# iracigt/ceres-raytracer

Measured on AMD Instinct MI355X. Metric: Mrays/sec (primary+shadow) on dragon.obj 1920x1080; 1/2/4/8-GPU scaling, higher is better.
Workload: dtype f32; 1 GPU; dragon_1080: dragon.obj 1920x1080 primary+shadow, 16 copies of the config view per step; views=config, W=1920, H=1080, row_block=1080, parallelism=one GPU, whole frames, float_framebuffer=True, streams=8

## Files before the change

### ceres-raytracer_amd/__init__.py

```python
import ctypes
import os
import sys

import numpy as np

_PKG = os.path.dirname(os.path.abspath(__file__))
LIB_PATH = os.environ.get("CERES_LIB") or os.path.join(_PKG, "libceres_hip.so")
CLI_PATH = os.path.join(_PKG, "render")

if _PKG not in sys.path:
    sys.path.insert(0, _PKG)
import configs

MODE_FULL, MODE_PRIMARY = 0, 1
MODE_ROBUST = 0x10
MODE_QBVH4 = 0x20
MODE_FMA = 0x40
ARITH_EXACT, ARITH_FMA = 0, 1


def cfg_mode(cfg, arith=ARITH_EXACT):
    return ((MODE_PRIMARY if cfg["mode"] == "primary" else MODE_FULL) | (MODE_ROBUST if cfg.get("robust") else 0)
            | (MODE_FMA if arith else 0))
SCENE_STATS = 1
SCENE_FIRST_ORDER = 2

EXPORTED_SYMBOLS = (
    "ceres_obj_load", "ceres_proc_mesh", "ceres_rotate_triangles", "ceres_bvh_build", "ceres_bvh_build_gpu",
    "ceres_bvh_build_device", "ceres_obj_load_gpu", "ceres_obj_parse_device", "ceres_rotate_triangles_device",
    "ceres_device_free", "ceres_camera_basis", "ceres_obj_load_f64", "ceres_proc_mesh_f64", "ceres_rotate_triangles_f64",
    "ceres_bvh_build_f64", "ceres_camera_basis_f64", "ceres_orbit_cameras_f64", "ceres_scene_create_f64",
    "ceres_render_f64", "ceres_render_records_f64", "ceres_obj_load_f64_arith", "ceres_proc_mesh_f64_arith",
    "ceres_rotate_triangles_f64_arith", "ceres_bvh_build_f64_arith", "ceres_camera_basis_f64_arith",
    "ceres_orbit_cameras_f64_arith",
    "ceres_free", "ceres_scene_create", "ceres_scene_create_device", "ceres_scene_destroy", "ceres_scene_info", "ceres_scene_shadow_stacks", "ceres_render_f32",
    "ceres_render_device", "ceres_render_batch_device", "ceres_render_multi_f32", "ceres_device_count", "ceres_assemble_rgb8_packed", "ceres_render_records", "ceres_tiling_local_rows",
    "ceres_scene_set_timing", "ceres_scene_read_timing", "ceres_scene_wave_log", "ceres_fetch_counters",
    "ceres_cpu_scene_create", "ceres_cpu_scene_destroy", "ceres_render_cpu_f32", "ceres_cpu_scene_create_f64",
    "ceres_render_cpu_f64",
    "ceres_orbit_cameras", "ceres_assemble_rgb8",
    "ceres_kernel_names", "ceres_last_error", "ceres_version",
    "ceres_obj_load_arith", "ceres_proc_mesh_arith", "ceres_rotate_triangles_arith", "ceres_bvh_build_arith",
    "ceres_camera_basis_arith", "ceres_orbit_cameras_arith", "ceres_content_hash",
    "ceres_bvh_build_gpu_arith", "ceres_bvh_build_device_arith", "ceres_obj_load_gpu_arith",
    "ceres_obj_parse_device_arith", "ceres_rotate_triangles_device_arith",
    "ceres_trace_rays", "ceres_trace_rays_device", "ceres_trace_rays_cpu",
    "ceres_trace_rays_f64", "ceres_trace_rays_f64_device", "ceres_trace_rays_cpu_f64",
    "ceres_shade_rays", "ceres_shade_rays_device", "ceres_shade_rays_cpu", "ceres_camera_rays",
    "ceres_shade_rays_f64", "ceres_shade_rays_f64_device", "ceres_shade_rays_cpu_f64", "ceres_camera_rays_f64",
    "ceres_scene_refit", "ceres_scene_refit_device", "ceres_scene_refit_f64", "ceres_scene_refit_f64_device",
    "ceres_cpu_scene_refit", "ceres_cpu_scene_refit_f64", "ceres_scene_read_boxes",
)

HIT_DTYPE = np.dtype([("prim", np.int32), ("t", np.float32), ("u", np.float32), ("v", np.float32)])
FLT_MAX = np.float32(np.finfo(np.float32).max)
HIT64_DTYPE = np.dtype([("prim", np.int32), ("pad", np.uint32), ("t", np.float64), ("u", np.float64), ("v", np.float64)])
DBL_MAX = np.float64(np.finfo(np.float64).max)


class CeresError(RuntimeError):
    pass


class _Stats(ctypes.Structure):
    _fields_ = [("rays", ctypes.c_uint64), ("hits", ctypes.c_uint64), ("primary_rays", ctypes.c_uint64),
                ("shadow_rays", ctypes.c_uint64), ("node_pairs", ctypes.c_uint64), ("tri_tests", ctypes.c_uint64),
                ("ms", ctypes.c_double)]


class Tiling(ctypes.Structure):
    _fields_ = [("row_block", ctypes.c_uint32), ("rank", ctypes.c_uint32), ("world", ctypes.c_uint32),
                ("bands", ctypes.c_uint32)]


_lib = None
_fp = ctypes.POINTER(ctypes.c_float)
_dp = ctypes.POINTER(ctypes.c_double)
_u32p = ctypes.POINTER(ctypes.c_uint32)
_u64p = ctypes.POINTER(ctypes.c_uint64)
_sz = ctypes.c_size_t
_vp = ctypes.c_void_p


def build(verbose=False):
    import subprocess
    r = subprocess.run(["make", "-C", os.path.join(_PKG, "csrc"), "-j4", "all"], capture_output=True, text=True)
    if verbose or r.returncode:
        sys.stdout.write(r.stdout)
        sys.stderr.write(r.stderr)
    if r.returncode:
        raise CeresError("build of libceres_hip.so failed")


def lib():
    global _lib
    if _lib is not None:
        return _lib
    if not os.path.exists(LIB_PATH):
        raise CeresError(f"{LIB_PATH} is missing: run __graft_entry__.build() (no CPU fallback exists)")
    if "torch" not in sys.modules:
        try:
            import torch
        except ImportError:
            pass
    L = ctypes.CDLL(LIB_PATH)
    L.ceres_last_error.restype = ctypes.c_char_p
    L.ceres_version.restype = ctypes.c_char_p
    L.ceres_kernel_names.restype = ctypes.c_char_p
    L.ceres_obj_load.argtypes = [ctypes.c_char_p, ctypes.POINTER(_fp), ctypes.POINTER(_fp), ctypes.POINTER(_sz)]
    L.ceres_proc_mesh.argtypes = [ctypes.c_int, ctypes.POINTER(_fp), ctypes.POINTER(_fp), ctypes.POINTER(_sz)]
    L.ceres_rotate_triangles.argtypes = [_fp, _sz, ctypes.c_int, ctypes.c_float]
    L.ceres_bvh_build.argtypes = [_fp, _sz, ctypes.POINTER(_u32p), ctypes.POINTER(_sz), ctypes.POINTER(_u64p)]
    L.ceres_bvh_build_gpu.argtypes = [_fp, _sz, ctypes.POINTER(_u32p), ctypes.POINTER(_sz), ctypes.POINTER(_u64p),
                                      ctypes.c_int]
    L.ceres_bvh_build_device.argtypes = [_vp, _sz, _vp, _vp, ctypes.POINTER(_sz), _vp]
    L.ceres_obj_load_gpu.argtypes = [ctypes.c_char_p, ctypes.POINTER(_fp), ctypes.POINTER(_fp), ctypes.POINTER(_sz),
                                     ctypes.c_int]
    L.ceres_obj_parse_device.argtypes = [_vp, _sz, ctypes.POINTER(_vp), ctypes.POINTER(_vp), ctypes.POINTER(_sz), _vp]
    L.ceres_rotate_triangles_device.argtypes = [_vp, _sz, ctypes.c_int, ctypes.c_float, _vp]
    L.ceres_device_free.argtypes = [_vp]
    L.ceres_device_free.restype = None
    L.ceres_camera_basis.argtypes = [_fp, _fp, _fp, ctypes.c_float, _sz, _sz, _fp]
    L.ceres_obj_load_f64.argtypes = [ctypes.c_char_p, ctypes.POINTER(_dp), ctypes.POINTER(_dp), ctypes.POINTER(_sz)]
    L.ceres_proc_mesh_f64.argtypes = [ctypes.c_int, ctypes.POINTER(_dp), ctypes.POINTER(_dp), ctypes.POINTER(_sz)]
    L.ceres_rotate_triangles_f64.argtypes = [_dp, _sz, ctypes.c_int, ctypes.c_double]
    L.ceres_bvh_build_f64.argtypes = [_dp, _sz, ctypes.POINTER(_u64p), ctypes.POINTER(_sz), ctypes.POINTER(_u64p)]
    L.ceres_camera_basis_f64.argtypes = [_dp, _dp, _dp, ctypes.c_double, _sz, _sz, _dp]
    L.ceres_orbit_cameras_f64.argtypes = [_dp, _dp, _dp, _dp, ctypes.c_double, _sz, _sz, _dp, ctypes.c_double,
                                          ctypes.c_uint32, ctypes.c_int, _dp, _dp, _dp]
    L.ceres_obj_load_f64_arith.argtypes = [ctypes.c_char_p, ctypes.POINTER(_dp), ctypes.POINTER(_dp), ctypes.POINTER(_sz),
                                           ctypes.c_int]
    L.ceres_proc_mesh_f64_arith.argtypes = [ctypes.c_int, ctypes.POINTER(_dp), ctypes.POINTER(_dp), ctypes.POINTER(_sz),
                                            ctypes.c_int]
    L.ceres_rotate_triangles_f64_arith.argtypes = [_dp, _sz, ctypes.c_int, ctypes.c_double, ctypes.c_int]
    L.ceres_bvh_build_f64_arith.argtypes = [_dp, _sz, ctypes.POINTER(_u64p), ctypes.POINTER(_sz), ctypes.POINTER(_u64p),
                                            ctypes.c_int]
    L.ceres_camera_basis_f64_arith.argtypes = [_dp, _dp, _dp, ctypes.c_double, _sz, _sz, _dp, ctypes.c_int]
    L.ceres_orbit_cameras_f64_arith.argtypes = [_dp, _dp, _dp, _dp, ctypes.c_double, _sz, _sz, _dp, ctypes.c_double,
                                                ctypes.c_uint32, ctypes.c_int, _dp, _dp, _dp, ctypes.c_int]
    L.ceres_scene_create_f64.argtypes = [_dp, _sz, _dp, _vp, _sz, _u64p, ctypes.c_int, ctypes.c_uint32]
    L.ceres_scene_create_f64.restype = _vp
    L.ceres_render_f64.argtypes = [_vp, _dp, _dp, ctypes.c_int, _dp, ctypes.POINTER(ctypes.c_uint8), _sz, _sz,
                                   ctypes.POINTER(_Stats)]
    L.ceres_render_records_f64.argtypes = [_vp, _dp, _dp, ctypes.c_int, _sz, _sz, ctypes.POINTER(ctypes.c_int32), _dp,
                                           ctypes.POINTER(ctypes.c_int8), ctypes.POINTER(_Stats)]
    L.ceres_orbit_cameras.argtypes = [_fp, _fp, _fp, _fp, ctypes.c_float, _sz, _sz, _fp, ctypes.c_float,
                                      ctypes.c_uint32, ctypes.c_int, _fp, _fp, _fp]
    L.ceres_free.argtypes = [_vp]
    L.ceres_free.restype = None
    L.ceres_scene_create.argtypes = [_fp, _sz, _fp, _vp, _sz, _u64p, ctypes.c_int, ctypes.c_uint32]
    L.ceres_scene_create.restype = _vp
    L.ceres_scene_create_device.argtypes = [_vp, _sz, _vp, _vp, _sz, _vp, ctypes.c_int, ctypes.c_uint32, _vp]
    L.ceres_scene_create_device.restype = _vp
    L.ceres_scene_destroy.argtypes = [_vp]
    L.ceres_scene_destroy.restype = None
    L.ceres_scene_info.argtypes = [_vp, _u32p, _u32p, ctypes.POINTER(_sz), ctypes.POINTER(_sz)]
    L.ceres_scene_shadow_stacks.argtypes = [_vp, _u32p, _u32p]
    L.ceres_render_f32.argtypes = [_vp, _fp, _fp, ctypes.c_int, _fp, ctypes.POINTER(ctypes.c_uint8), _sz, _sz,
                                   ctypes.POINTER(_Stats)]
    L.ceres_render_device.argtypes = [_vp, _fp, _fp, ctypes.c_int, _sz, _sz, ctypes.POINTER(Tiling), _vp, _vp, _vp, _vp]
    L.ceres_render_batch_device.argtypes = [_vp, ctypes.c_uint32, _fp, _fp, ctypes.c_int, _sz, _sz,
                                            ctypes.POINTER(Tiling), _vp, _vp, _vp, _vp]
    L.ceres_render_multi_f32.argtypes = [ctypes.POINTER(_vp), ctypes.c_uint32, ctypes.c_uint32, _fp, _fp, ctypes.c_int, _fp,
                                         ctypes.POINTER(ctypes.c_uint8), _sz, _sz, ctypes.POINTER(_Stats)]
    L.ceres_assemble_rgb8_packed.argtypes = [_vp, _vp, ctypes.c_uint32, _sz, _sz, ctypes.c_uint32, ctypes.c_uint32, _vp]
    L.ceres_assemble_rgb8.argtypes = [_vp, _sz, _vp, ctypes.c_uint32, _sz, _sz, ctypes.c_uint32, ctypes.c_uint32, _vp]
    L.ceres_render_records.argtypes = [_vp, _fp, _fp, ctypes.c_int, _sz, _sz, ctypes.POINTER(ctypes.c_int32), _fp,
                                       ctypes.POINTER(ctypes.c_int8), ctypes.POINTER(_Stats)]
    L.ceres_tiling_local_rows.argtypes = [_sz, ctypes.POINTER(Tiling)]
    L.ceres_tiling_local_rows.restype = _sz
    L.ceres_scene_set_timing.argtypes = [_vp, ctypes.c_int]
    L.ceres_scene_read_timing.argtypes = [_vp, ctypes.POINTER(ctypes.c_double), ctypes.POINTER(ctypes.c_double),
                                          _u64p]
    L.ceres_scene_wave_log.argtypes = [_vp, _u64p, _sz, ctypes.POINTER(_sz)]
    L.ceres_fetch_counters.argtypes = [ctypes.c_int, _u64p, ctypes.c_int]
    L.ceres_cpu_scene_create.argtypes = [_fp, _sz, _fp, _vp, _sz, _u64p]
    L.ceres_cpu_scene_create.restype = _vp
    L.ceres_cpu_scene_destroy.argtypes = [_vp]
    L.ceres_cpu_scene_destroy.restype = None
    L.ceres_render_cpu_f32.argtypes = [_vp, _fp, _fp, ctypes.c_int, _fp, ctypes.POINTER(ctypes.c_uint8), _sz, _sz,
                                       ctypes.POINTER(_Stats), ctypes.c_int]
    L.ceres_cpu_scene_create_f64.argtypes = [_dp, _sz, _dp, _vp, _sz, _u64p]
    L.ceres_cpu_scene_create_f64.restype = _vp
    L.ceres_render_cpu_f64.argtypes = [_vp, _dp, _dp, ctypes.c_int, _dp, ctypes.POINTER(ctypes.c_uint8), _sz, _sz,
                                       ctypes.POINTER(_Stats), ctypes.c_int]
    L.ceres_trace_rays.argtypes = [_vp, _vp, _sz, ctypes.c_int, _vp, _vp, ctypes.POINTER(_Stats)]
    L.ceres_trace_rays_device.argtypes = [_vp, _vp, _sz, ctypes.c_int, _vp, _vp, _vp, _vp]
    L.ceres_trace_rays_cpu.argtypes = [_vp, _vp, _sz, ctypes.c_int, _vp, _vp, ctypes.POINTER(_Stats), ctypes.c_int]
    L.ceres_trace_rays_f64.argtypes = L.ceres_trace_rays.argtypes
    L.ceres_trace_rays_f64_device.argtypes = L.ceres_trace_rays_device.argtypes
    L.ceres_trace_rays_cpu_f64.argtypes = L.ceres_trace_rays_cpu.argtypes
    L.ceres_shade_rays.argtypes = [_vp, _vp, _sz, _fp, ctypes.c_int, _vp, _vp, _vp, _vp, ctypes.POINTER(_Stats)]
    L.ceres_shade_rays_device.argtypes = [_vp, _vp, _sz, _fp, ctypes.c_int, _vp, _vp, _vp, _vp, _vp, _vp]
    L.ceres_shade_rays_cpu.argtypes = L.ceres_shade_rays.argtypes + [ctypes.c_int]
    L.ceres_camera_rays.argtypes = [_fp, _sz, _sz, ctypes.c_int, _vp]
    L.ceres_shade_rays_f64.argtypes = [_vp, _vp, _sz, _dp, ctypes.c_int, _vp, _vp, _vp, _vp, ctypes.POINTER(_Stats)]
    L.ceres_shade_rays_f64_device.argtypes = [_vp, _vp, _sz, _dp, ctypes.c_int, _vp, _vp, _vp, _vp, _vp, _vp]
    L.ceres_shade_rays_cpu_f64.argtypes = L.ceres_shade_rays_f64.argtypes + [ctypes.c_int]
    L.ceres_camera_rays_f64.argtypes = [_dp, _sz, _sz, ctypes.c_int, _vp]
    L.ceres_scene_refit.argtypes = [_vp, _fp, _sz, _fp]
    L.ceres_scene_refit_f64.argtypes = [_vp, _dp, _sz, _dp]
    L.ceres_scene_refit_device.argtypes = [_vp, _vp, _sz, _vp, _vp]
    L.ceres_scene_refit_f64_device.argtypes = [_vp, _vp, _sz, _vp, _vp]
    L.ceres_cpu_scene_refit.argtypes = [_vp, _fp, _sz, _fp]
    L.ceres_cpu_scene_refit_f64.argtypes = [_vp, _dp, _sz, _dp]
    L.ceres_scene_read_boxes.argtypes = [_vp, _vp, ctypes.POINTER(_sz), _fp, ctypes.POINTER(_sz)]
    L.ceres_content_hash.argtypes = [_vp, _sz]
    L.ceres_content_hash.restype = ctypes.c_uint64
    L.ceres_obj_load_arith.argtypes = L.ceres_obj_load.argtypes + [ctypes.c_int]
    L.ceres_proc_mesh_arith.argtypes = L.ceres_proc_mesh.argtypes + [ctypes.c_int]
    L.ceres_rotate_triangles_arith.argtypes = L.ceres_rotate_triangles.argtypes + [ctypes.c_int]
    L.ceres_bvh_build_arith.argtypes = L.ceres_bvh_build.argtypes + [ctypes.c_int]
    L.ceres_camera_basis_arith.argtypes = L.ceres_camera_basis.argtypes + [ctypes.c_int]
    L.ceres_orbit_cameras_arith.argtypes = L.ceres_orbit_cameras.argtypes + [ctypes.c_int]
    L.ceres_bvh_build_gpu_arith.argtypes = L.ceres_bvh_build_gpu.argtypes + [ctypes.c_int]
    L.ceres_bvh_build_device_arith.argtypes = L.ceres_bvh_build_device.argtypes + [ctypes.c_int]
    L.ceres_obj_load_gpu_arith.argtypes = L.ceres_obj_load_gpu.argtypes + [ctypes.c_int]
    L.ceres_obj_parse_device_arith.argtypes = L.ceres_obj_parse_device.argtypes + [ctypes.c_int]
    L.ceres_rotate_triangles_device_arith.argtypes = L.ceres_rotate_triangles_device.argtypes + [ctypes.c_int]
    _lib = L
    return L


def _check(rc):
    if rc != 0:
        raise CeresError(f"ceres error {rc}: {lib().ceres_last_error().decode()}")


def _p(a, t):
    return None if a is None else a.ctypes.data_as(ctypes.POINTER(t))


def _take(ptr, count, dtype):
    if count == 0:
        lib().ceres_free(ctypes.cast(ptr, _vp))
        return np.zeros(0, dtype)
    a = np.ctypeslib.as_array(ptr, shape=(count,)).copy().view(dtype)
    lib().ceres_free(ctypes.cast(ptr, _vp))
    return a


class Camera:

    def __init__(self, eye, dir, up, fov, dtype=np.float32, arith=ARITH_EXACT):
        self.dtype = np.dtype(dtype)
        self.eye = np.asarray(eye, self.dtype)
        self.dir = np.asarray(dir, self.dtype)
        self.up = np.asarray(up, self.dtype)
        self.fov = float(fov)
        self.arith = int(arith)

    def basis(self, W, H):
        if self.dtype == np.float64:
            out = np.zeros(9, np.float64)
            _check(lib().ceres_camera_basis_f64_arith(_p(self.eye, ctypes.c_double), _p(self.dir, ctypes.c_double),
                                                      _p(self.up, ctypes.c_double), self.fov, W, H,
                                                      _p(out, ctypes.c_double), self.arith))
            return np.concatenate([self.eye, out])
        out = np.zeros(9, np.float32)
        _check(lib().ceres_camera_basis_arith(_p(self.eye, ctypes.c_float), _p(self.dir, ctypes.c_float),
                                              _p(self.up, ctypes.c_float), self.fov, W, H, _p(out, ctypes.c_float),
                                              self.arith))
        return np.concatenate([self.eye, out]).astype(np.float32)


class Mesh:

    def __init__(self, tri, norm):
        dt = np.float64 if np.asarray(tri).dtype == np.float64 else np.float32
        self.tri = np.ascontiguousarray(tri, dt).reshape(-1, 12)
        self.norm = np.ascontiguousarray(norm, dt).reshape(-1, 9)

    @property
    def f64(self):
        return self.tri.dtype == np.float64

    def __len__(self):
        return self.tri.shape[0]


class Bvh:

    def __init__(self, nodes, prim):
        dt = np.uint64 if np.asarray(nodes).dtype == np.uint64 else np.uint32
        self.nodes = np.ascontiguousarray(nodes, dt).reshape(-1, 8)
        self.prim = np.ascontiguousarray(prim, np.uint64)


def load_obj(path, arith=ARITH_EXACT):
    t, n, cnt = _fp(), _fp(), _sz()
    _check(lib().ceres_obj_load_arith(os.fsencode(path), ctypes.byref(t), ctypes.byref(n), ctypes.byref(cnt), int(arith)))
    c = cnt.value
    return Mesh(_take(t, c * 12, np.float32).reshape(c, 12), _take(n, c * 9, np.float32).reshape(c, 9))


def load_obj_f64(path, arith=ARITH_EXACT):
    t, n, cnt = _dp(), _dp(), _sz()
    _check(lib().ceres_obj_load_f64_arith(os.fsencode(path), ctypes.byref(t), ctypes.byref(n), ctypes.byref(cnt),
                                          int(arith)))
    c = cnt.value
    return Mesh(_take(t, c * 12, np.float64).reshape(c, 12), _take(n, c * 9, np.float64).reshape(c, 9))


def proc_mesh_f64(n, arith=ARITH_EXACT):
    t, nn, cnt = _dp(), _dp(), _sz()
    _check(lib().ceres_proc_mesh_f64_arith(int(n), ctypes.byref(t), ctypes.byref(nn), ctypes.byref(cnt), int(arith)))
    c = cnt.value
    return Mesh(_take(t, c * 12, np.float64).reshape(c, 12), _take(nn, c * 9, np.float64).reshape(c, 9))


def load_obj_gpu(path, device=0, arith=ARITH_EXACT):
    t, n, cnt = _fp(), _fp(), _sz()
    _check(lib().ceres_obj_load_gpu_arith(os.fsencode(path), ctypes.byref(t), ctypes.byref(n), ctypes.byref(cnt),
                                          int(device), int(arith)))
    c = cnt.value
    return Mesh(_take(t, c * 12, np.float32).reshape(c, 12), _take(n, c * 9, np.float32).reshape(c, 9))


def parse_obj_device(d_text, length, stream=0, arith=ARITH_EXACT):
    t, n, cnt = _vp(), _vp(), _sz()
    _check(lib().ceres_obj_parse_device_arith(d_text, length, ctypes.byref(t), ctypes.byref(n), ctypes.byref(cnt),
                                              stream or None, int(arith)))
    return t.value or 0, n.value or 0, cnt.value


def rotate_triangles_device(d_tri48, n_tri, axis, degrees, stream=0, arith=ARITH_EXACT):
    ax = {"x": 0, "y": 1, "z": 2}[axis] if isinstance(axis, str) else int(axis)
    _check(lib().ceres_rotate_triangles_device_arith(d_tri48, n_tri, ax, float(degrees), stream or None, int(arith)))
# ... 242 lines not shown

    def shade(self, rays, sun, mode=0, pixels=True, rgb8=False, hits=False, status=False, threads=0):
        fn = lib().ceres_shade_rays_cpu_f64 if self.f64 else lib().ceres_shade_rays_cpu
        return _shade_host(lambda r, n, s, m, px, q, h, stt, st: fn(self._h, r, n, s, m, px, q, h, stt, st, int(threads)),
                           rays, sun, mode, pixels, rgb8, hits, status, self.f64)


class Scene:

    def __init__(self, mesh, bvh, device=0, stats=False, first_order=False, _handle=None):
        L = lib()
        if _handle is not None:
            self._h, self.device, self.n_tri = _handle
            self.f64 = False
            return
        self.f64 = mesh.f64
        flags = (SCENE_STATS if stats else 0) | (SCENE_FIRST_ORDER if first_order else 0)
        if self.f64:
            self._h = L.ceres_scene_create_f64(_p(mesh.tri, ctypes.c_double), len(mesh), _p(mesh.norm, ctypes.c_double),
                                               bvh.nodes.ctypes.data_as(_vp), bvh.nodes.shape[0],
                                               _p(bvh.prim, ctypes.c_uint64), int(device), flags)
        else:
            self._h = L.ceres_scene_create(_p(mesh.tri, ctypes.c_float), len(mesh), _p(mesh.norm, ctypes.c_float),
                                           bvh.nodes.ctypes.data_as(_vp), bvh.nodes.shape[0],
                                           _p(bvh.prim, ctypes.c_uint64), int(device), flags)
        if not self._h:
            raise CeresError("ceres_scene_create: " + L.ceres_last_error().decode())
        self.device = device
        self.n_tri = len(mesh)

    @classmethod
    def from_device(cls, d_tri48, n_tri, d_norm36, d_nodes32, n_nodes, d_prim32, device=0, stats=False, stream=0):
        L = lib()
        h = L.ceres_scene_create_device(d_tri48, n_tri, d_norm36, d_nodes32, n_nodes, d_prim32, int(device),
                                        SCENE_STATS if stats else 0, stream or None)
        if not h:
            raise CeresError("ceres_scene_create_device: " + L.ceres_last_error().decode())
        return cls(None, None, _handle=(h, device, n_tri))

    def info(self):
        d, s, n, b = ctypes.c_uint32(), ctypes.c_uint32(), _sz(), _sz()
        _check(lib().ceres_scene_info(self._h, ctypes.byref(d), ctypes.byref(s), ctypes.byref(n), ctypes.byref(b)))
        near, first = ctypes.c_uint32(), ctypes.c_uint32()
        _check(lib().ceres_scene_shadow_stacks(self._h, ctypes.byref(near), ctypes.byref(first)))
        return dict(depth=d.value, stack_entries=s.value, n_pairs=n.value, device_bytes=b.value,
                    shadow_stack_nearest=near.value, shadow_stack_first=first.value)

    def refit(self, mesh):
        if mesh.f64 != self.f64:
            raise CeresError("refit: a %s mesh for a %s scene" % (("float", "double")[mesh.f64], ("float", "double")[self.f64]))
        fn, ct = (lib().ceres_scene_refit_f64, ctypes.c_double) if self.f64 else (lib().ceres_scene_refit, ctypes.c_float)
        _check(fn(self._h, _p(mesh.tri, ct), len(mesh), _p(mesh.norm, ct)))

    def refit_device(self, d_tri, d_norm=0, stream=0, n_tri=None):
        fn = lib().ceres_scene_refit_f64_device if self.f64 else lib().ceres_scene_refit_device
        _check(fn(self._h, d_tri or None, int(self.n_tri if n_tri is None else n_tri), d_norm or None, stream or None))

    def read_boxes(self):
        n, m = _sz(), _sz()
        _check(lib().ceres_scene_read_boxes(self._h, None, ctypes.byref(n), None, ctypes.byref(m)))
        pairs = np.zeros((n.value, 12), np.float64 if self.f64 else np.float32)
        nodes4 = np.zeros((m.value, 24), np.float32) if m.value else None
        _check(lib().ceres_scene_read_boxes(self._h, pairs.ctypes.data_as(_vp), ctypes.byref(n),
                                            _p(nodes4, ctypes.c_float), ctypes.byref(m)))
        return pairs, nodes4

    def close(self):
        if getattr(self, "_h", None):
            lib().ceres_scene_destroy(self._h)
            self._h = None

    def __del__(self):
        try:
            self.close()
        except Exception:
            pass

    def render(self, basis12, sun, W, H, mode=MODE_FULL, want_pixels=True, want_rgb8=True):
        dt, ct = (np.float64, ctypes.c_double) if self.f64 else (np.float32, ctypes.c_float)
        b = np.ascontiguousarray(basis12, dt)
        s = np.ascontiguousarray(sun, dt)
        px = np.empty(3 * W * H, dt) if want_pixels else None
        rgb = np.empty(3 * W * H, np.uint8) if want_rgb8 else None
        st = _Stats()
        fn = lib().ceres_render_f64 if self.f64 else lib().ceres_render_f32
        _check(fn(self._h, _p(b, ct), _p(s, ct), int(mode), _p(px, ct), _p(rgb, ctypes.c_uint8), W, H, ctypes.byref(st)))
        return px, rgb, dict(rays=st.rays, hits=st.hits, primary_rays=st.primary_rays, shadow_rays=st.shadow_rays,
                             node_pairs=st.node_pairs, tri_tests=st.tri_tests, ms=st.ms)

    def records(self, basis12, sun, W, H, mode=MODE_FULL):
        dt, ct = (np.float64, ctypes.c_double) if self.f64 else (np.float32, ctypes.c_float)
        b = np.ascontiguousarray(basis12, dt)
        s = np.ascontiguousarray(sun, dt)
        prim = np.empty(W * H, np.int32)
        tuv = np.empty(3 * W * H, dt)
        sh = np.empty(W * H, np.int8)
        st = _Stats()
        fn = lib().ceres_render_records_f64 if self.f64 else lib().ceres_render_records
        _check(fn(self._h, _p(b, ct), _p(s, ct), int(mode), W, H, _p(prim, ctypes.c_int32), _p(tuv, ct),
                  _p(sh, ctypes.c_int8), ctypes.byref(st)))
        return prim, tuv.reshape(-1, 3), sh, dict(rays=st.rays, hits=st.hits, node_pairs=st.node_pairs,
                                                  tri_tests=st.tri_tests)

    def render_device(self, basis12, sun, W, H, mode=MODE_FULL, tiling=None, d_pixels=0, d_rgb8=0, d_counters=0,
                      stream=0):
        b = np.ascontiguousarray(basis12, np.float32)
        s = np.ascontiguousarray(sun, np.float32)
        t = ctypes.byref(tiling) if tiling is not None else None
        _check(lib().ceres_render_device(self._h, _p(b, ctypes.c_float), _p(s, ctypes.c_float), int(mode), W, H, t,
                                         d_pixels or None, d_rgb8 or None, d_counters or None, stream or None))

    def render_batch_device(self, basis12, sun3, W, H, mode=MODE_FULL, tiling=None, d_pixels=0, d_rgb8=0,
                            d_counters=0, stream=0):
        b = np.ascontiguousarray(basis12, np.float32).reshape(-1, 12)
        s = np.ascontiguousarray(sun3, np.float32).reshape(-1, 3)
        if b.shape[0] != s.shape[0]:
            raise CeresError("render_batch_device: %d cameras but %d suns" % (b.shape[0], s.shape[0]))
        t = ctypes.byref(tiling) if tiling is not None else None
        _check(lib().ceres_render_batch_device(self._h, b.shape[0], _p(b, ctypes.c_float), _p(s, ctypes.c_float),
                                               int(mode), W, H, t, d_pixels or None, d_rgb8 or None,
                                               d_counters or None, stream or None))

    def trace(self, rays, mode=0, closest=True, occluded=False):
        fn = lib().ceres_trace_rays_f64 if self.f64 else lib().ceres_trace_rays
        return _trace_host(lambda r, n, m, h, o, st: fn(self._h, r, n, m, h, o, st), rays, mode, closest, occluded, self.f64)

    def trace_device(self, d_rays32, n_rays, mode=0, d_hits16=0, d_occluded=0, d_counters=0, stream=0):
        fn = lib().ceres_trace_rays_f64_device if self.f64 else lib().ceres_trace_rays_device
        _check(fn(self._h, d_rays32 or None, int(n_rays), int(mode), d_hits16 or None, d_occluded or None,
                  d_counters or None, stream or None))

    def shade(self, rays, sun, mode=0, pixels=True, rgb8=False, hits=False, status=False):
        fn = lib().ceres_shade_rays_f64 if self.f64 else lib().ceres_shade_rays
        return _shade_host(lambda r, n, s, m, px, q, h, stt, st: fn(self._h, r, n, s, m, px, q, h, stt, st),
                           rays, sun, mode, pixels, rgb8, hits, status, self.f64)

    def shade_device(self, d_rays32, n_rays, sun, mode=0, d_pixels=0, d_rgb8=0, d_hits16=0, d_status=0, d_counters=0,
                     stream=0):
        dt, ct = (np.float64, ctypes.c_double) if self.f64 else (np.float32, ctypes.c_float)
        fn = lib().ceres_shade_rays_f64_device if self.f64 else lib().ceres_shade_rays_device
        s = np.ascontiguousarray(sun, dt).reshape(3)
        _check(fn(self._h, d_rays32 or None, int(n_rays), _p(s, ct), int(mode), d_pixels or None, d_rgb8 or None,
                  d_hits16 or None, d_status or None, d_counters or None, stream or None))

    def set_timing(self, on):
        _check(lib().ceres_scene_set_timing(self._h, 1 if on else 0))

    def wave_log(self, max_waves=1 << 16):
        out = np.zeros(8 * max_waves, np.uint64)
        n = _sz()
        _check(lib().ceres_scene_wave_log(self._h, _p(out, ctypes.c_uint64), max_waves, ctypes.byref(n)))
        return out[: 8 * n.value].reshape(-1, 8)

    def read_timing(self):
        p, q, n = ctypes.c_double(), ctypes.c_double(), ctypes.c_uint64()
        _check(lib().ceres_scene_read_timing(self._h, ctypes.byref(p), ctypes.byref(q), ctypes.byref(n)))
        return p.value, q.value, n.value


def source_sha16(repo=None):
    import glob
    import hashlib
    repo = repo or os.path.dirname(_PKG)
    inc = sorted(glob.glob(os.path.join(repo, "include", "*.h")) + glob.glob(os.path.join(repo, "include", "ceres", "*.hpp")))
    csrc = os.path.join(_PKG, "csrc")
    names = sorted(n for n in os.listdir(csrc) if n.endswith((".cpp", ".hip", ".hpp")))
    h = hashlib.sha256()
    for f in inc + [os.path.join(csrc, n) for n in names]:
        with open(f, "rb") as fh:
            h.update(fh.read())
    return h.hexdigest()[:16]


def native_provenance():
    import hashlib
    v = lib().ceres_version().decode()
    built = v.rsplit(" src ", 1)[1] if " src " in v else None
    with open(LIB_PATH, "rb") as fh:
        so_sha = hashlib.sha256(fh.read()).hexdigest()
    now = source_sha16()
    return {"lib": os.path.relpath(LIB_PATH, os.path.dirname(_PKG)), "version": v, "so_sha256": so_sha,
            "built_from_sources_sha16": built, "tree_sources_sha16": now, "built_from_this_tree": built == now}


FETCH_KINDS = ("bvh2_vector", "bvh4_vector", "bvh4_scalar", "tri_vector", "tri_scalar", "shade_vector",
               "store_vector", "order_scalar")
COUNT_LIB_PATH = os.path.join(_PKG, "variants", "libceres_hip_count.so")


def fetch_counters(device=0, reset=True):
    out = np.zeros(8, np.uint64)
    _check(lib().ceres_fetch_counters(int(device), _p(out, ctypes.c_uint64), 1 if reset else 0))
    return {k: int(v) for k, v in zip(FETCH_KINDS, out)}


def render_multi(scenes, basis12, sun, W, H, row_block=8, mode=MODE_FULL, want_pixels=True, want_rgb8=True):
    b = np.ascontiguousarray(basis12, np.float32)
    s = np.ascontiguousarray(sun, np.float32)
    px = np.empty(3 * W * H, np.float32) if want_pixels else None
    rgb = np.empty(3 * W * H, np.uint8) if want_rgb8 else None
    hs = (_vp * len(scenes))(*[sc._h for sc in scenes])
    st = _Stats()
    _check(lib().ceres_render_multi_f32(hs, len(scenes), int(row_block), _p(b, ctypes.c_float), _p(s, ctypes.c_float),
                                        int(mode), _p(px, ctypes.c_float), _p(rgb, ctypes.c_uint8), W, H,
                                        ctypes.byref(st)))
    return px, rgb, dict(rays=st.rays, hits=st.hits, primary_rays=st.primary_rays, shadow_rays=st.shadow_rays,
                         node_pairs=st.node_pairs, tri_tests=st.tri_tests, ms=st.ms)


def orbit_cameras(camera, sun, W, H, n_frames, axis=(0, 1, 0), step_deg=None, rotate_first=True, want_dirs=False):
    n = int(n_frames)
    step = np.float32(360.0) / np.float32(n) if step_deg is None else np.float32(step_deg)
    b = np.zeros((n, 12), np.float32)
    s3 = np.zeros((n, 3), np.float32)
    d3 = np.zeros((n, 3), np.float32)
    ax = np.asarray(axis, np.float32)
    sn = np.asarray(sun, np.float32)
    _check(lib().ceres_orbit_cameras_arith(_p(camera.eye, ctypes.c_float), _p(camera.dir, ctypes.c_float),
                                           _p(camera.up, ctypes.c_float), _p(sn, ctypes.c_float), camera.fov, W, H,
                                           _p(ax, ctypes.c_float), float(step), n, 1 if rotate_first else 0,
                                           _p(b, ctypes.c_float), _p(s3, ctypes.c_float), _p(d3, ctypes.c_float),
                                           camera.arith))
    return (b, s3, d3) if want_dirs else (b, s3)


def bench_views(camera, sun, W, H, F, basis0=None):
    F = int(F)
    b12 = np.zeros((F, 12), np.float32)
    s3 = np.zeros((F, 3), np.float32)
    steps = np.asarray([configs.orbit_step(f, F) for f in range(F)], np.float32)
    b12[0] = camera.basis(W, H) if basis0 is None else np.asarray(basis0, np.float32)
    s3[0] = np.asarray(sun, np.float32)
    for f in range(1, F):
        b, s = orbit_cameras(camera, sun, W, H, 2, axis=configs.BENCH_AXIS, step_deg=float(steps[f]),
                             rotate_first=False)
        b12[f], s3[f] = b[1], s[1]
    return b12, s3, steps


def pose(cfg, frame=0, arith=ARITH_EXACT):
    cam = Camera(cfg["eye"], cfg["dir"], cfg["up"], cfg["fov"], arith=arith)
    axis, step = (cfg["orbit"][0], cfg["orbit"][1]) if cfg.get("orbit") else configs.BENCH_ORBIT
    n = (cfg["orbit"][2] if cfg.get("orbit") else 0) + int(frame)
    if n == 0:
        return cam, np.asarray(cfg["sun"], np.float32)
    b, s3, d3 = orbit_cameras(cam, cfg["sun"], cfg["W"], cfg["H"], n + 1, axis=axis, step_deg=step,
                              rotate_first=False, want_dirs=True)
    return Camera(b[n, :3], d3[n], cfg["up"], cfg["fov"], arith=arith), s3[n].copy()


def pose_f64(cfg, arith=ARITH_EXACT):
    cam = Camera(cfg["eye"], cfg["dir"], cfg["up"], cfg["fov"], dtype=np.float64, arith=arith)
    sun = np.asarray(cfg["sun"], np.float64)
    if not cfg.get("orbit"):
        return cam, sun
    (axis, step, n) = cfg["orbit"]
    b = np.zeros((n + 1, 12), np.float64)
    s3 = np.zeros((n + 1, 3), np.float64)
    d3 = np.zeros((n + 1, 3), np.float64)
    ax = np.asarray(axis, np.float64)
    _check(lib().ceres_orbit_cameras_f64_arith(_p(cam.eye, ctypes.c_double), _p(cam.dir, ctypes.c_double),
                                               _p(cam.up, ctypes.c_double), _p(sun, ctypes.c_double), cam.fov, cfg["W"],
                                               cfg["H"], _p(ax, ctypes.c_double), float(step), n + 1, 0,
                                               _p(b, ctypes.c_double), _p(s3, ctypes.c_double), _p(d3, ctypes.c_double),
                                               int(arith)))
    return Camera(b[n, :3], d3[n], cfg["up"], cfg["fov"], dtype=np.float64, arith=arith), s3[n].copy()


def assemble_rgb8(d_gathered, rank_stride, d_out, frames, W, H, row_block, world, stream=0):
    _check(lib().ceres_assemble_rgb8(d_gathered, rank_stride, d_out, int(frames), W, H, int(row_block), int(world),
                                     stream or None))


def assemble_rgb8_packed(d_gathered, d_out, frames, W, H, row_block, world, stream=0):
    _check(lib().ceres_assemble_rgb8_packed(d_gathered, d_out, int(frames), W, H, int(row_block), int(world),
                                            stream or None))


def local_rows(H, tiling):
    return lib().ceres_tiling_local_rows(H, ctypes.byref(tiling))


def row_map(H, row_block, world):
    out = []
    nb = (H + row_block - 1) // row_block
    for r in range(world):
        rows = []
        for b in range(r, nb, world):
            rows.extend(range(b * row_block, min(H, (b + 1) * row_block)))
        out.append(np.asarray(rows, np.int64))
    return out


def prepare(cfg, f64=False, arith=ARITH_EXACT):
    if f64:
        mesh = proc_mesh_f64(cfg["proc"], arith) if cfg.get("proc") else load_obj_f64(configs.obj_path(cfg), arith)
        if len(mesh) == 0:
            raise CeresError("The given scene is empty or cannot be loaded")
        if cfg.get("rotate"):
            rotate_triangles(mesh, cfg["rotate"][0], cfg["rotate"][1], arith)
        return mesh, build_bvh(mesh, arith), pose_f64(cfg, arith)[0]
    mesh = proc_mesh(cfg["proc"], arith) if cfg.get("proc") else load_obj(configs.obj_path(cfg), arith)
    if len(mesh) == 0:
        raise CeresError("The given scene is empty or cannot be loaded")
    if cfg.get("rotate"):
        rotate_triangles(mesh, cfg["rotate"][0], cfg["rotate"][1], arith)
    bvh = build_bvh(mesh, arith)
    cam, _ = pose(cfg, arith=arith)
    return mesh, bvh, cam


def render(camera, sun, scene, W, H, mode=MODE_FULL):
    px, _, st = scene.render(camera.basis(W, H), sun, W, H, mode=mode, want_rgb8=False)
    return px, st["rays"], st["hits"]


def ppm(W, H, rgb8):
    return b"P6 %d %d 255\n" % (W, H) + np.asarray(rgb8, np.uint8).tobytes()
```

### ceres-raytracer_amd/csrc/ceres_types.hpp

```cpp
#pragma once
#include <cstddef>
#include <cstdint>
#include <vector>

namespace ceres {

struct Tri48 {
    float p0[3], e1[3], e2[3], n[3];
};
static_assert(sizeof(Tri48) == 48, "Tri48");

struct RefNode {
    float bounds[6];
    uint32_t primitive_count;
    uint32_t first_child_or_primitive;
};
static_assert(sizeof(RefNode) == 32, "RefNode");

struct alignas(16) SiblingPair {
    float lb[6];
    float rb[6];
    uint32_t lcount, lfirst;
    uint32_t rcount, rfirst;
};
static_assert(sizeof(SiblingPair) == 64, "SiblingPair");

struct RefNode64 {
    double bounds[6];
    uint64_t primitive_count;
    uint64_t first_child_or_primitive;
};
static_assert(sizeof(RefNode64) == 64, "RefNode64");
struct Tri96 { double p0[3], e1[3], e2[3], n[3]; };
static_assert(sizeof(Tri96) == 96, "Tri96");
struct alignas(16) SiblingPair64 {
    double lb[6], rb[6];
    uint32_t lcount, lfirst, rcount, rfirst;
};
static_assert(sizeof(SiblingPair64) == 112, "SiblingPair64");

constexpr uint32_t kNode4Empty = 0xffffffffu;
constexpr uint32_t kNode4CountBits = 5;
constexpr uint32_t kNode4MaxCount = (1u << kNode4CountBits) - 1;
constexpr uint32_t kNode4MaxFirst = (1u << (32 - kNode4CountBits)) - 2;
struct alignas(128) Node4 {
    float lo_x[4], hi_x[4], lo_y[4], hi_y[4], lo_z[4], hi_z[4];
    uint32_t child[4];
    uint32_t nleaf;
    uint32_t unused[3];
};
static_assert(sizeof(Node4) == 128, "Node4");
#if defined(__HIPCC__)
__host__ __device__
#endif
inline uint32_t node4_child(uint32_t count, uint32_t first) { return first << kNode4CountBits | count; }

constexpr uint32_t kNode4NoSource = 0xffffffffu;

#if defined(__HIPCC__)
__host__ __device__
#endif
inline void node4_leaves_first(Node4& r, uint32_t* src = nullptr) {
    Node4 t;
    uint32_t k = 0, nl = 0, ts[4] = {0, 0, 0, 0};
    for (int pass = 0; pass < 3; ++pass)
        for (int c = 0; c < 4; ++c) {
            const uint32_t w = r.child[c];
            const int group = w == kNode4Empty ? 2 : (w & kNode4MaxCount) ? 0 : 1;
            if (group != pass) continue;
            t.lo_x[k] = r.lo_x[c]; t.hi_x[k] = r.hi_x[c];
            t.lo_y[k] = r.lo_y[c]; t.hi_y[k] = r.hi_y[c];
            t.lo_z[k] = r.lo_z[c]; t.hi_z[k] = r.hi_z[c];
            t.child[k] = w;
            if (src) ts[k] = src[c];
            nl += group == 0;
            ++k;
        }
    t.nleaf = nl;
    t.unused[0] = t.unused[1] = t.unused[2] = 0;
    r = t;
    if (src) for (int c = 0; c < 4; ++c) src[c] = ts[c];
}

struct alignas(64) QNode4 {
    float ox, oy, oz, sx;
    float sy, sz;
    uint32_t qlx, qhx;
    uint32_t qly, qhy, qlz, qhz;
    uint32_t child[4];
};
static_assert(sizeof(QNode4) == 64, "QNode4");

constexpr int kShards = 32;
struct alignas(128) Shard {
    uint32_t queued;
    uint32_t error;
    unsigned long long hits;
    unsigned long long pairs;
    unsigned long long tests;
    uint32_t pad[24];
};
static_assert(sizeof(Shard) == 128, "Shard");

constexpr int kMaxFrames = 64;
constexpr int kFramesPerLaunch = 56;
struct FrameCam {
    float eye[3], dir[3], iu[3], iv[3], sun[3];
};

constexpr uint32_t kTileXBits = 13, kTileYBits = 13;
constexpr uint32_t pack_tile(uint32_t f, uint32_t y, uint32_t x) { return (f << (kTileXBits + kTileYBits)) | (y << kTileXBits) | x; }

struct CullRect { uint16_t i0, i1, j0, j1; };

struct KParams {
    FrameCam cam[kFramesPerLaunch];
    CullRect cull_rect[kFramesPerLaunch];
    uint32_t frames;
    uint32_t W, H;
    uint32_t row_block, rank, world, local_rows;
    uint32_t bands;
    uint32_t band_magic;
    uint32_t row_blocks_per_frame;
    uint32_t stack_entries;
    uint32_t root_leaf_count, root_leaf_first;
    float root_box[6];
    uint32_t root_box_ok;
    uint32_t cull;
    uint32_t shadow_stack_entries;
    uint32_t steal_first;
    uint32_t packets;
    uint32_t tiles_x;
    uint32_t lds_entries;
    uint32_t tile_packed;
    const uint32_t* tile_order;
    const SiblingPair* pairs;
    const Node4* nodes4;
    const QNode4* qnodes4;
    const Tri48* tris;
    const uint32_t* orig;
    const float* norms;
    float* pixels;
    uint8_t* rgb8;
    Shard* shards;
    int32_t* rec_prim;
    float* rec_tuv;
    int8_t* rec_shadow;
    unsigned long long* wave_log;
    uint32_t fill_stride, fill_magic;
};
static_assert(sizeof(KParams) <= 4096, "KParams must fit the 4 KB kernel-argument limit");

struct DeviceLayout {
    float root_box[6] = {0, 0, 0, 0, 0, 0};
    SiblingPair* pairs = nullptr;
    Node4* nodes4 = nullptr;
    Tri48* tris = nullptr;
    uint32_t* orig = nullptr;
    size_t n_pairs = 0, n_nodes4 = 0;
    uint32_t depth = 0, stack4 = 0, root_leaf_count = 0, root_leaf_first = 0;
    uint32_t* src4 = nullptr;
};
#ifdef __HIPCC__
int relayout_device(const Tri48* d_tris, uint32_t n_tri, const RefNode* d_nodes, uint32_t n_nodes, const uint32_t* d_prim,
                    hipStream_t stream, DeviceLayout& out);
#endif

int relayout_bvh(const RefNode* nodes, size_t n_nodes, const uint64_t* prim, size_t n_tri, const Tri48* tris,
                 std::vector<SiblingPair>& pairs, std::vector<Tri48>& leaf_tris, std::vector<uint32_t>& orig,
                 uint32_t& depth, uint32_t& root_leaf_count, uint32_t& root_leaf_first);
int build_shadow_bvh4(const std::vector<SiblingPair>& pairs, std::vector<Node4>& out, uint32_t& stack_bound,
                      uint32_t& not_collapsed, std::vector<uint32_t>* src4 = nullptr);
int order_shadow_bvh4(std::vector<Node4>& nodes, uint32_t& first_bound, std::vector<uint32_t>* src4 = nullptr);
int relayout_bvh64(const RefNode64* nodes, size_t n_nodes, const uint64_t* prim, size_t n_tri, const Tri96* tris,
                   std::vector<SiblingPair64>& pairs, std::vector<Tri96>& leaf_tris, std::vector<uint32_t>& orig,
                   uint32_t& depth, uint32_t& root_leaf_count, uint32_t& root_leaf_first);

}
```

### ceres-raytracer_amd/csrc/render_hip.hip

```cpp
#include <hip/hip_runtime.h>

#include <algorithm>
#include <chrono>
#include <cfloat>
#include <cmath>
#include <cstdint>
#include <cstdlib>
#include <cstring>
#include <new>
#include <string>
#include <type_traits>
#include <vector>

#include "ceres_render.h"
#include "ceres_types.hpp"
#include "host_common.hpp"
#include "pow24.hpp"

#pragma clang fp contract(off)

#ifndef CERES_COUNTING
#define CERES_COUNTING 0
#endif
#ifndef CERES_TILES_PER_WAVE
#define CERES_TILES_PER_WAVE 4
#endif
#ifndef CERES_TPW_BY_SIZE
#define CERES_TPW_BY_SIZE 1
#endif
#ifndef CERES_FRAME_MAJOR_PIXELS
#define CERES_FRAME_MAJOR_PIXELS (1u << 20)
#endif
#ifndef CERES_SPLIT_UNIFORM
#define CERES_SPLIT_UNIFORM 1
#endif
#ifndef CERES_ROOT_TEST
#define CERES_ROOT_TEST 1
#endif
#ifndef CERES_OCTANT_SLAB
#define CERES_OCTANT_SLAB 3
#endif
#ifndef CERES_SHADOW_PACKET
#define CERES_SHADOW_PACKET 1
#endif
#ifndef CERES_TRUST_STACK_BOUND
#define CERES_TRUST_STACK_BOUND 1
#endif
#ifndef CERES_PAIR_STORES
#define CERES_PAIR_STORES 1
#endif
#ifndef CERES_STACK_GUARD
#define CERES_STACK_GUARD CERES_COUNTING
#endif
#ifndef CERES_ASSEMBLE_NT
#define CERES_ASSEMBLE_NT 0
#endif
#ifndef CERES_LOCAL_ORDER
#define CERES_LOCAL_ORDER 1
#endif
#ifndef CERES_LOCAL_CHUNK_BATCH
#define CERES_LOCAL_CHUNK_BATCH 128
#endif
#ifndef CERES_XCD_GROUP_TILES
#define CERES_XCD_GROUP_TILES 16
#endif
#ifndef CERES_LOCAL_CHUNK_SOLO
#define CERES_LOCAL_CHUNK_SOLO 16
#endif
#ifndef CERES_RCP_UNIFORM
#define CERES_RCP_UNIFORM 2
#endif
#ifndef CERES_RCP_IFTHEN
#define CERES_RCP_IFTHEN 1
#endif
#ifndef CERES_PK_PACKET
#define CERES_PK_PACKET 1
#endif
#ifndef CERES_LOAD_ALWAYS
#define CERES_LOAD_ALWAYS 1
#endif
#ifndef CERES_CULL
#define CERES_CULL 1
#endif
#ifndef CERES_TRI_SELECT
#define CERES_TRI_SELECT 1
#endif

namespace ceres {

char* error_buffer() {
    static thread_local char buf[kErrorBufferSize] = "";
    return buf;
}

namespace dev {

constexpr int kBlock = 256;

struct F3 { float x, y, z; };
__device__ __forceinline__ F3 operator+(F3 a, F3 b) { return {a.x + b.x, a.y + b.y, a.z + b.z}; }
__device__ __forceinline__ F3 operator-(F3 a, F3 b) { return {a.x - b.x, a.y - b.y, a.z - b.z}; }
__device__ __forceinline__ F3 operator*(F3 a, float s) { return {a.x * s, a.y * s, a.z * s}; }
__device__ __forceinline__ float dot(F3 a, F3 b) { float s = a.x * b.x; s += a.y * b.y; s += a.z * b.z; return s; }
__device__ __forceinline__ F3 cross(F3 a, F3 b) { return {a.y * b.z - a.z * b.y, a.z * b.x - a.x * b.z, a.x * b.y - a.y * b.x}; }
template <bool kU = false>
__device__ __forceinline__ float rcp_exact(float x) {
    const uint32_t m = __float_as_uint(x) & 0x7fffffffu;
    if (kU) {
        const bool slow = m - 0x00800000u >= 0x7e000000u - 0x00800000u;
        if (__builtin_expect(__ballot(slow) != 0, 0)) {
            const float q = 1.0f / x;
            const float r0 = __builtin_amdgcn_rcpf(x);
            return slow ? q : __builtin_fmaf(__builtin_fmaf(-x, r0, 1.0f), r0, r0);
        }
        const float r0 = __builtin_amdgcn_rcpf(x);
        return __builtin_fmaf(__builtin_fmaf(-x, r0, 1.0f), r0, r0);
    }
    if constexpr (CERES_RCP_IFTHEN) {
        const float r0 = __builtin_amdgcn_rcpf(x);
        float r = __builtin_fmaf(__builtin_fmaf(-x, r0, 1.0f), r0, r0);
        if (__builtin_expect(m - 0x00800000u >= 0x7e000000u - 0x00800000u, 0)) r = 1.0f / x;
        return r;
    }
    if (__builtin_expect(m - 0x00800000u >= 0x7e000000u - 0x00800000u, 0)) return 1.0f / x;
    const float r0 = __builtin_amdgcn_rcpf(x);
    return __builtin_fmaf(__builtin_fmaf(-x, r0, 1.0f), r0, r0);
}

__device__ __forceinline__ float rcp_fast(float x) {
    const float r0 = __builtin_amdgcn_rcpf(x);
    return __builtin_fmaf(__builtin_fmaf(-x, r0, 1.0f), r0, r0);
}
__device__ __forceinline__ F3 normalize(F3 v) { float inv = 1.0f / sqrtf(dot(v, v)); return v * inv; }
__device__ __forceinline__ F3 f3(const float* p) { return {p[0], p[1], p[2]}; }

template <bool kG> __device__ __forceinline__ float dotA(F3 a, F3 b) {
    if constexpr (kG) return __builtin_fmaf(a.z, b.z, __builtin_fmaf(a.x, b.x, a.y * b.y));
    else return dot(a, b);
}
template <bool kG> __device__ __forceinline__ float dotB(F3 a, F3 b) {
    if constexpr (kG) return __builtin_fmaf(a.z, b.z, __builtin_fmaf(a.y, b.y, a.x * b.x));
    else return dot(a, b);
}
template <bool kG> __device__ __forceinline__ F3 crossG(F3 a, F3 b) {
    if constexpr (kG)
        return {__builtin_fmaf(a.y, b.z, -(a.z * b.y)), __builtin_fmaf(a.z, b.x, -(a.x * b.z)),
                __builtin_fmaf(a.x, b.y, -(a.y * b.x))};
    else return cross(a, b);
}
template <bool kG> __device__ __forceinline__ F3 normalizeG(F3 v) { float inv = 1.0f / sqrtf(dotA<kG>(v, v)); return v * inv; }

__device__ __forceinline__ bool uniform_id(uint32_t id, uint32_t& r) {
    r = __builtin_amdgcn_readfirstlane(id);
    return __ballot(id != r) == 0;
}
enum FetchKind : int {
    kFBvh2V = 0,
    kFBvh4V,
    kFBvh4S,
    kFTriV,
    kFTriS,
    kFShadeV,
    kFStoreV,
    kFOrderS,
    kFKinds
};
#if CERES_COUNTING
constexpr int kFetchShards = 16;
__device__ unsigned long long g_fetch[kFetchShards][kFKinds];
__device__ __forceinline__ void count_fetch(int k, uint32_t bytes, bool per_lane) {
    const uint64_t m = __ballot(1);
    if ((threadIdx.x & 63u) == uint32_t(__builtin_ctzll(m)))
        atomicAdd(&g_fetch[blockIdx.x % kFetchShards][k], (unsigned long long)(per_lane ? __popcll(m) : 1) * bytes);
}
#define CERES_COUNT_V(k, b) ::ceres::dev::count_fetch((k), (b), true)
#define CERES_COUNT_S(k, b) ::ceres::dev::count_fetch((k), (b), false)
#else
#define CERES_COUNT_V(k, b) ((void)0)
#define CERES_COUNT_S(k, b) ((void)0)
#endif

typedef float F4v __attribute__((ext_vector_type(4)));
typedef uint32_t U4v __attribute__((ext_vector_type(4)));
__device__ __forceinline__ float4 sload_f4(const void* p, int i) {
    const F4v v = ((const __attribute__((address_space(4))) F4v*)(p))[i];
    return make_float4(v.x, v.y, v.z, v.w);
}
__device__ __forceinline__ uint32_t sload_u32(const void* p) {
    return *((const __attribute__((address_space(4))) uint32_t*)(p));
}
__device__ __forceinline__ uint4 sload_u4(const void* p, int i) {
    const U4v v = ((const __attribute__((address_space(4))) U4v*)(p))[i];
    return make_uint4(v.x, v.y, v.z, v.w);
}

struct TriV { F3 p0, e1, e2, n; };
__device__ __forceinline__ TriV load_tri(const Tri48* t) {
    const float4* q = reinterpret_cast<const float4*>(t);
    const float4 a = q[0], b = q[1], c = q[2];
    return {{a.x, a.y, a.z}, {a.w, b.x, b.y}, {b.z, b.w, c.x}, {c.y, c.z, c.w}};
}
__device__ __forceinline__ TriV load_tri_s(const Tri48* t) {
    const float4 a = sload_f4(t, 0), b = sload_f4(t, 1), c = sload_f4(t, 2);
    return {{a.x, a.y, a.z}, {a.w, b.x, b.y}, {b.z, b.w, c.x}, {c.y, c.z, c.w}};
}
__device__ __forceinline__ TriV load_tri_u(const Tri48* tris, uint32_t idx) {
    uint32_t r;
    if (uniform_id(idx, r)) { CERES_COUNT_S(kFTriS, 48); return load_tri_s(tris + r); }
    CERES_COUNT_V(kFTriV, 48);
    return load_tri(tris + idx);
}

struct Stk24 {
    uint16_t* lo;
    uint8_t* hi;
    struct Ref {
        uint16_t* lo; uint8_t* hi;
        __device__ __forceinline__ operator uint32_t() const { return uint32_t(*lo) | (uint32_t(*hi) << 16); }
        __device__ __forceinline__ Ref& operator=(uint32_t v) { *lo = uint16_t(v); *hi = uint8_t(v >> 16); return *this; }
    };
    __device__ __forceinline__ Ref operator[](uint32_t i) const { return {lo + i, hi + i}; }
};

template <typename StkT> __device__ __forceinline__ constexpr uint32_t stack_guard() {
    return std::is_same<StkT, uint16_t*>::value ? 0xffffu : std::is_same<StkT, Stk24>::value ? 0xffffffu : 0xffffffffu;
}

struct Hit { uint32_t slot; float t, u, v; };
constexpr uint32_t kNoSlot = 0xffffffffu;

struct CamRay {
    constexpr float tmin() const { return 0.0f; }
    constexpr float tmax() const { return FLT_MAX; }
    static constexpr bool kNanFail = false;
    static constexpr bool kUnitDir = true;
// ... 853 lines not shown
        }
        const unsigned long long idle = __ballot(!active);
        const unsigned long long donors = __ballot(active && cnt > 0);
        if (idle && donors) {
            const uint32_t n_idle = __popcll(idle), n_don = __popcll(donors);
            if (active && cnt > 0) {
                const uint32_t r = __popcll(donors & lt_mask);
                if (r < n_idle) {
                    L.mail[wbase + r] = stk[bot * kS];
                    L.from[wbase + r] = lane;
                    bot = bot + 1 == cap ? 0 : bot + 1;
                    --cnt;
                }
            }
            __builtin_amdgcn_wave_barrier();
            uint32_t mail = 0, donor = 0;
            const uint32_t r = __popcll(idle & lt_mask);
            const bool thief = !active && r < n_don;
            if (thief) { mail = L.mail[wbase + r]; donor = L.from[wbase + r]; }
            const float ox = __shfl(w.o.x, donor, 64), oy = __shfl(w.o.y, donor, 64), oz = __shfl(w.o.z, donor, 64);
            const float dx = __shfl(w.d.x, donor, 64), dy = __shfl(w.d.y, donor, 64), dz = __shfl(w.d.z, donor, 64);
            const float jx = __shfl(w.ix, donor, 64), jy = __shfl(w.iy, donor, 64), jz = __shfl(w.iz, donor, 64);
            const float tx = __shfl(w.sx, donor, 64), ty = __shfl(w.sy, donor, 64), tz = __shfl(w.sz, donor, 64);
            const uint32_t down = __shfl(owner, donor, 64);
            if (thief) {
                w.o = F3{ox, oy, oz}; w.d = F3{dx, dy, dz};
                w.ix = jx; w.iy = jy; w.iz = jz; w.sx = tx; w.sy = ty; w.sz = tz;
                owner = down;
                cur = mail;
                top = bot = cnt = 0;
                active = true;
            }
            __builtin_amdgcn_wave_barrier();
        }
    }
    __builtin_amdgcn_wave_barrier();
}

template <bool kRobust = false, bool kG = false>
__device__ __forceinline__ RayWork make_shadow_ray(F3 o, F3 sun) {
    RayWork w;
    w.o = o;
    w.d = normalizeG<kG>(sun - o);
    const Slab<kRobust> sl = make_slab<kRobust>(o, w.d);
    w.ix = sl.ix; w.iy = sl.iy; w.iz = sl.iz; w.sx = sl.sx; w.sy = sl.sy; w.sz = sl.sz;
    return w;
}

template <typename StkT, bool kRobust, bool kQ, bool kG>
__device__ __forceinline__ bool shadow_packet(const KParams& P, bool hit, const RayWork& w, uint32_t lane, bool& blocked) {
    if constexpr (!kRobust && !kQ && CERES_SHADOW_PACKET && std::is_same<StkT, uint16_t*>::value) {
        const uint64_t act = __ballot(hit);
        if (!act) { blocked = false; return true; }
        const uint32_t oct = (__float_as_uint(w.ix) >> 31) | (__float_as_uint(w.iy) >> 31) << 1 |
                             (__float_as_uint(w.iz) >> 31) << 2;
        const int first = __builtin_ctzll(act);
        const uint32_t oct0 = uint32_t(__builtin_amdgcn_readlane(int(oct), first));
        const bool finite = isfinite(w.ix) && isfinite(w.iy) && isfinite(w.iz) && isfinite(w.sx) && isfinite(w.sy) &&
                            isfinite(w.sz);
        if (!P.packets || P.shadow_stack_entries > 64 || P.root_leaf_count || __ballot(hit && (oct != oct0 || !finite)))
            return false;
        auto bc = [&](float x) { return hit ? x : __int_as_float(__builtin_amdgcn_readlane(__float_as_int(x), first)); };
        const F3 o{bc(w.o.x), bc(w.o.y), bc(w.o.z)}, d{bc(w.d.x), bc(w.d.y), bc(w.d.z)};
        const Slab<false> sl{bc(w.ix), bc(w.iy), bc(w.iz), bc(w.sx), bc(w.sy), bc(w.sz), o};
        uint64_t occ = 0;
        switch (oct0) {
            case 0: occ = packet_any4<0, kG>(P, sl, o, d, act, lane); break;
            case 1: occ = packet_any4<1, kG>(P, sl, o, d, act, lane); break;
            case 2: occ = packet_any4<2, kG>(P, sl, o, d, act, lane); break;
            case 3: occ = packet_any4<3, kG>(P, sl, o, d, act, lane); break;
            case 4: occ = packet_any4<4, kG>(P, sl, o, d, act, lane); break;
            case 5: occ = packet_any4<5, kG>(P, sl, o, d, act, lane); break;
            case 6: occ = packet_any4<6, kG>(P, sl, o, d, act, lane); break;
            default: occ = packet_any4<7, kG>(P, sl, o, d, act, lane); break;
        }
        blocked = (occ >> lane) & 1u;
        return true;
    }
    return false;
}

template <bool kG, bool kBands = false>
__device__ __forceinline__ void shade_pixel(const KParams& P, uint32_t f, uint32_t lr, uint32_t i, uint32_t pix,
                                            bool blocked, F3 sun_line, uint32_t slot, float hu, float hv,
                                            uint32_t& occluded, float c[3]) {
    if (P.rec_shadow) P.rec_shadow[pix] = blocked ? 1 : 0;
    c[0] = c[1] = c[2] = 0.f;
    if (blocked) {
        ++occluded;
    } else {
        const F3 view = primary_dir<kG>(P, f, i, global_row<kBands>(P, f, lr));
        CERES_COUNT_V(kFShadeV, 40);
        shade<kG>(sun_line, P.norms + 9 * size_t(P.orig[slot]), view, hu, hv, c);
    }
}

constexpr int kFusedB = 64;
constexpr size_t kLdsPerCu = 160 * 1024;
template <bool kStats, typename StkT, int kMinW, bool kRobust, bool kSteal, bool kQ, bool kG, int kTPWo = 0, bool kBands = false>
__global__ __launch_bounds__(kFusedB) __attribute__((amdgpu_waves_per_eu(kMinW))) void ceres_fused(const KParams P) {
    constexpr int kB = kFusedB;
    constexpr bool kPacketsCompiled = !kStats && !kSteal && !kRobust && !kQ && CERES_SHADOW_PACKET && std::is_same<StkT, uint16_t*>::value;
    extern __shared__ __attribute__((aligned(16))) uint32_t lds[];
    __shared__ StealLdsT<kB> L;
    const uint32_t lane = threadIdx.x, tid = lane;
    constexpr uint32_t kTPWp = (kStats || kSteal) ? 1 : kTPWo ? uint32_t(kTPWo) : uint32_t(CERES_TILES_PER_WAVE);
    constexpr bool kPair = CERES_PAIR_STORES && !kStats && !kSteal && kTPWp >= 2 && std::is_same<StkT, uint16_t*>::value;
    __shared__ typename std::conditional<kPair, PairStash, NoStash>::type S;
    auto tile_pixel = [&](uint32_t t, uint32_t& f_, uint32_t& lr_, uint32_t& i_) {
        uint32_t by_, bx_;
        if (P.tile_packed) {
            bx_ = t & ((1u << kTileXBits) - 1u);
            by_ = (t >> kTileXBits) & ((1u << kTileYBits) - 1u);
            f_ = t >> (kTileXBits + kTileYBits);
        } else {
            const uint32_t per_frame_ = P.tiles_x * P.row_blocks_per_frame;
            f_ = t / per_frame_;
            const uint32_t rem = t - f_ * per_frame_;
            by_ = rem / P.tiles_x; bx_ = rem - by_ * P.tiles_x;
        }
        const uint32_t lx = (lane & 1) | ((lane >> 1) & 2) | ((lane >> 2) & 4), ly = ((lane >> 1) & 1) | ((lane >> 2) & 2) | ((lane >> 3) & 4);
        i_ = bx_ * 8u + lx;
        lr_ = by_ * 8u + ly;
        return i_ < P.W && lr_ < P.local_rows && (!kBands || global_row<true>(P, f_, lr_) < P.H);
    };
    bool stashed = false;
    auto flush = [&](uint32_t t_prev) {
        if constexpr (kPair) {
            uint32_t pf, plr, pi;
            if (tile_pixel(t_prev, pf, plr, pi)) store_pixel(P, pf, plr, pi, S.c[0][lane], S.c[1][lane], S.c[2][lane]);
        }
        stashed = false;
    };
    auto emit = [&](uint32_t q, bool last, uint32_t t_prev, bool act, uint32_t f_, uint32_t lr_, uint32_t i_, float c0, float c1,
                    float c2) {
        if constexpr (kPair) {
            if (!(q & 1u) && !last) {
                S.c[0][lane] = c0; S.c[1][lane] = c1; S.c[2][lane] = c2;
                stashed = true;
                return;
            }
            if (stashed) flush(t_prev);
        }
        if (act) store_pixel(P, f_, lr_, i_, c0, c1, c2);
    };
    StkT stk;
    if constexpr (std::is_same<StkT, Stk24>::value)
        stk = Stk24{reinterpret_cast<uint16_t*>(lds) + tid,
                    reinterpret_cast<uint8_t*>(lds) + size_t(P.lds_entries) * kB * 2 + tid};
    else
        stk = reinterpret_cast<StkT>(lds) + tid;
    constexpr uint32_t kTile = 8;
    constexpr uint32_t kTPW = (kStats || kSteal) ? 1 : kTPWo ? uint32_t(kTPWo) : uint32_t(CERES_TILES_PER_WAVE);
    const uint32_t per_frame = P.tiles_x * P.row_blocks_per_frame;
    const uint32_t n_tiles = per_frame * P.frames;
    uint32_t group = blockIdx.x;
    if constexpr (!kStats) {
        const uint32_t tile_groups = (n_tiles + kTPW - 1) / kTPW;
        if (P.fill_stride) {
            const uint32_t oct = blockIdx.x >> 3, x = blockIdx.x & 7u, nfo = (gridDim.x >> 3) - (tile_groups + 7u) / 8u;
            const uint32_t q = __umulhi(oct, P.fill_magic), r = oct - q * P.fill_stride;
            if (r == P.fill_stride - 1 && q < nfo) {
                fill_culled_rows<kBands>(P, q * 8u + x, lane);
                return;
            }
            group = (oct - (q < nfo ? q : nfo)) * 8u + x;
            if (group >= tile_groups) return;
        } else if (blockIdx.x >= tile_groups) {
            fill_culled_rows<kBands>(P, blockIdx.x - tile_groups, lane);
            return;
        }
    }
    uint32_t n_shadow = 0, occluded = 0, n_pairs = 0, n_tests = 0;
    bool overflow = false;
    static_assert(kTPW == 1 || kTPW == 2 || kTPW == 4 || kTPW == 8, "CERES_TILES_PER_WAVE must be 1, 2, 4 or 8");
    uint4 tiles4 = make_uint4(0, 0, 0, 0), tiles4b = make_uint4(0, 0, 0, 0);
    if constexpr (kTPW == 8) {
        tiles4 = sload_u4(P.tile_order + 8 * size_t(group), 0);
        tiles4b = sload_u4(P.tile_order + 8 * size_t(group), 1);
    } else if constexpr (kTPW == 4) {
        tiles4 = sload_u4(P.tile_order + 4 * size_t(group), 0);
    } else if constexpr (kTPW == 2) {
        tiles4.x = sload_u32(P.tile_order + 2 * size_t(group));
        tiles4.y = sload_u32(P.tile_order + 2 * size_t(group) + 1);
    } else {
        tiles4.x = sload_u32(P.tile_order + group);
    }
    CERES_COUNT_S(kFOrderS, 4 * kTPW);
    const uint32_t n_here = kTPW == 1 || n_tiles - group * kTPW >= kTPW ? kTPW : n_tiles - group * kTPW;
    for (uint32_t q = 0; q < n_here; ++q) {
    const uint4 tq = q < 4 ? tiles4 : tiles4b;
    const uint32_t qq = q & 3;
    const uint32_t t = kTPW == 1 ? tiles4.x : qq == 0 ? tq.x : qq == 1 ? tq.y : qq == 2 ? tq.z : tq.w;
    const uint32_t qp = (q - 1) & 3;
    const uint4 tp = q - 1 < 4 ? tiles4 : tiles4b;
    const uint32_t t_prev = qp == 0 ? tp.x : qp == 1 ? tp.y : qp == 2 ? tp.z : tp.w;
    uint32_t f, lr, i;
    bool active = tile_pixel(t, f, lr, i);
    uint32_t px = (f * P.local_rows + lr) * P.W + i;
    auto redecode = [&]() {
        if constexpr (CERES_LEAN_WRITES) {
            uint32_t tr = t;
            asm volatile("" : "+s"(tr));
            active = tile_pixel(tr, f, lr, i);
            px = (f * P.local_rows + lr) * P.W + i;
        }
    };
    bool hit = false;
    Hit h{0, 0.f, 0.f, 0.f};
    RayWork w{};
    uint64_t t_start = 0;
    if (kStats && P.wave_log) t_start = __builtin_amdgcn_s_memrealtime();
    const bool last_q = q + 1 == n_here;
    if (!kStats && P.cull && tile_misses_root(P, f, i >> 3, tile_rows_hit<kBands>(P, f, lr))) {
        if (stashed) flush(t_prev);
        continue;
    }
    if (active) {
        const F3 view = primary_dir<kG>(P, f, i, global_row<kBands>(P, f, lr));
        constexpr int kOctMode = (!kSteal || (CERES_OCTANT_SLAB & 4)) ? -1 : -2;
        hit = guarded_trace<kStats, kB, StkT, kRobust, kOctMode, kG>(P, f3(P.cam[f].eye), view, stk, h, n_pairs,
                                                                   n_tests, overflow);
        if (P.rec_prim) {
            redecode();
            P.rec_prim[px] = hit ? int32_t(P.orig[h.slot]) : -1;
            P.rec_tuv[3 * size_t(px)] = hit ? h.t : 0.f;
            P.rec_tuv[3 * size_t(px) + 1] = hit ? h.u : 0.f;
            P.rec_tuv[3 * size_t(px) + 2] = hit ? h.v : 0.f;
            P.rec_shadow[px] = -1;
        }
        if (hit) {
            CERES_COUNT_V(kFShadeV, 48);
            const TriV tr = load_tri(P.tris + h.slot);
            const F3 normal = normalizeG<kG>(tr.n);
            w = make_shadow_ray<kRobust, kG>(hit_point<kG>(tr, normal, h.u, h.v), f3(P.cam[f].sun));
        }
    }
    const uint32_t n_shadow_t = __popcll(__ballot(hit));
    n_shadow += n_shadow_t;
    uint64_t t_primary = 0;
    uint32_t prim_pairs = n_pairs, shadow_iters = 0;
    if (kStats && P.wave_log) t_primary = __builtin_amdgcn_s_memrealtime();
    bool pk_blocked = false;
    const bool pk = !kStats && !kSteal && shadow_packet<StkT, kRobust, kQ, kG>(P, hit, w, lane, pk_blocked);
    if (pk)
        L.blocked[tid] = pk_blocked ? 1u : 0u;
    else if constexpr (kSteal)
        steal_traverse<kStats, kB, StkT, kRobust, kQ, kG>(P, hit, w, stk, L, tid, lane, n_pairs, n_tests, overflow, &shadow_iters);
    else
        L.blocked[tid] = hit && trace_any4<kStats, kB, StkT, kRobust, kQ, kPacketsCompiled ? -2 : -1, kG>(
                                    P, w.o, w.d, stk, n_pairs, n_tests, overflow) ? 1u : 0u;
    redecode();
    float col[3] = {0.f, 0.f, 0.f};
    if (hit) shade_pixel<kG, kBands>(P, f, lr, i, px, L.blocked[tid] != 0, w.d, h.slot, h.u, h.v, occluded, col);
    emit(q, last_q, t_prev, active, f, lr, i, col[0], col[1], col[2]);
    if (kStats && P.wave_log) {
        const uint64_t t_end = __builtin_amdgcn_s_memrealtime();
        uint32_t mx = prim_pairs;
        for (int off = 32; off > 0; off >>= 1) mx = max(mx, uint32_t(__shfl_xor(int(mx), off, 64)));
        const uint32_t sp = wave_sum(prim_pairs), ss = wave_sum(n_pairs - prim_pairs);
        if (lane == 0) {
            unsigned long long* wl = P.wave_log + 8 * size_t(blockIdx.x);
            wl[0] = t_start; wl[1] = t_primary; wl[2] = t_end; wl[3] = mx; wl[4] = shadow_iters;
            wl[5] = n_shadow_t; wl[6] = sp; wl[7] = ss;
        }
    }
    }
    const uint32_t wo = wave_sum(occluded);
    const uint32_t shard = blockIdx.x % kShards;
    if (lane == 0 && n_shadow) {
        atomicAdd(&P.shards[shard].queued, n_shadow);
        atomicAdd(&P.shards[shard].hits, (unsigned long long)(n_shadow + wo));
    }
    if (kStats) {
        const uint32_t wp = wave_sum(n_pairs), wt = wave_sum(n_tests);
        if (lane == 0) {
            atomicAdd(&P.shards[shard].pairs, (unsigned long long)wp);
            atomicAdd(&P.shards[shard].tests, (unsigned long long)wt);
        }
    }
    if (overflow) atomicOr(&P.shards[shard].error, 1u);
}

__global__ __launch_bounds__(256) void ceres_compact_lit(const float* __restrict__ px, uint32_t n_pix,
                                                         uint4* __restrict__ out, uint32_t* __restrict__ n,
                                                         uint32_t cap) {
    const uint32_t p = blockIdx.x * 256 + threadIdx.x, lane = threadIdx.x & 63;
    uint32_t r = 0, g = 0, b = 0;
    if (p < n_pix) {
        const float* q = px + 3 * size_t(p);
        r = __float_as_uint(q[0]); g = __float_as_uint(q[1]); b = __float_as_uint(q[2]);
    }
    const bool lit = (r | g | b) != 0;
    const uint64_t m = __ballot(lit);
    if (!m) return;
    uint32_t base = 0;
    if (lane == 0) base = atomicAdd(n, uint32_t(__popcll(m)));
    base = uint32_t(__shfl(int(base), 0, 64));
    const uint32_t k = base + uint32_t(__popcll(m & ((1ull << lane) - 1ull)));
    if (lit && k < cap) out[k] = make_uint4(p, r, g, b);
}

__global__ void ceres_finalize(Shard* shards, uint64_t primary_rays, uint64_t* out) {
    if (threadIdx.x != 0) return;
    unsigned long long q = 0, h = 0, p = 0, t = 0;
    uint32_t err = 0;
    for (int s = 0; s < kShards; ++s) { q += shards[s].queued; h += shards[s].hits; p += shards[s].pairs; t += shards[s].tests; err |= shards[s].error; }
    for (int s = 0; s < kShards; ++s) { shards[s].queued = 0; shards[s].hits = 0; shards[s].pairs = 0; shards[s].tests = 0; shards[s].error = 0; }
    out[0] = primary_rays + q; out[1] = h; out[2] = primary_rays; out[3] = q;
    out[4] = p; out[5] = t; out[6] = err; out[7] = 0;
}

struct RayParams {
    const float4* rays;
    uint4* hits;
    uint8_t* occluded;
    unsigned long long* counters;
    const SiblingPair* pairs;
    const Node4* nodes4;
    const Tri48* tris;
    const uint32_t* orig;
    uint32_t n_rays;
    uint32_t stack_entries, shadow_stack_entries, lds_entries;
    uint32_t root_leaf_count, root_leaf_first;
    uint32_t root_box_ok;
    float root_box[6];
};

template <bool kStats, typename StkT, bool kRobust, bool kG>
__global__ __launch_bounds__(kFusedB) void ceres_trace_rays_k(const RayParams P) {
    constexpr int kB = kFusedB;
    constexpr int kOctMode = kStats ? -2 : -1;
    extern __shared__ __attribute__((aligned(16))) uint32_t lds[];
    const uint32_t lane = threadIdx.x;
    StkT stk;
    if constexpr (std::is_same<StkT, Stk24>::value)
        stk = Stk24{reinterpret_cast<uint16_t*>(lds) + lane,
                    reinterpret_cast<uint8_t*>(lds) + size_t(P.lds_entries) * kB * 2 + lane};
    else
        stk = reinterpret_cast<StkT>(lds) + lane;
    const uint32_t r = blockIdx.x * uint32_t(kB) + lane;
    bool hit = false, occ = false, overflow = false;
    uint32_t n_pairs = 0, n_tests = 0;
    if (r < P.n_rays) {
        const float4 a = P.rays[2 * size_t(r)], b = P.rays[2 * size_t(r) + 1];
        const F3 o{a.x, a.y, a.z}, d{a.w, b.x, b.y};
        const CallerRay rk{b.z, b.w};
        if (P.hits) {
            Hit h{kNoSlot, 0.f, 0.f, 0.f};
            hit = trace<false, kStats, kB, StkT, kRobust, kOctMode, kG>(P, o, d, stk, h, n_pairs, n_tests, overflow, rk);
            uint4 rec = make_uint4(0xffffffffu, 0u, 0u, 0u);
            if (hit) rec = make_uint4(P.orig[h.slot], __float_as_uint(h.t), __float_as_uint(h.u), __float_as_uint(h.v));
            P.hits[r] = rec;
        }
        if (P.occluded) {
            occ = trace_any4<false, kB, StkT, kRobust, false, kOctMode, kG>(P, o, d, stk, n_pairs, n_tests, overflow, rk);
            P.occluded[r] = occ ? 1 : 0;
        }
    }
    if (P.counters) {
        const uint32_t nh = __popcll(__ballot(P.hits ? hit : occ));
        if (lane == 0 && nh) atomicAdd(&P.counters[1], (unsigned long long)nh);
        if (kStats) {
            const uint32_t wp = wave_sum(n_pairs), wt = wave_sum(n_tests);
            if (lane == 0) {
                atomicAdd(&P.counters[4], (unsigned long long)wp);
                atomicAdd(&P.counters[5], (unsigned long long)wt);
            }
        }
        if (blockIdx.x == 0 && lane == 0) {
            atomicAdd(&P.counters[0], (unsigned long long)P.n_rays);
            atomicAdd(&P.counters[2], (unsigned long long)P.n_rays);
        }
        if (overflow) atomicOr(&P.counters[6], 1ull);
    }
}

struct ShadeParams {
    const float4* rays;
    float* pixels;
    uint8_t* rgb8;
    uint4* hits;
    uint8_t* status;
    unsigned long long* counters;
    const SiblingPair* pairs;
    const Node4* nodes4;
    const Tri48* tris;
    const uint32_t* orig;
    const float* norms;
    uint32_t n_rays;
    uint32_t stack_entries, shadow_stack_entries, lds_entries;
    uint32_t root_leaf_count, root_leaf_first;
    uint32_t root_box_ok;
    float root_box[6];
    float sun[3];
};

template <typename StkT, bool kRobust, bool kG>
__global__ __launch_bounds__(kFusedB) void ceres_shade_rays_k(const ShadeParams P) {
    constexpr int kB = kFusedB;
    extern __shared__ __attribute__((aligned(16))) uint32_t lds[];
    const uint32_t lane = threadIdx.x;
    StkT stk;
    if constexpr (std::is_same<StkT, Stk24>::value)
        stk = Stk24{reinterpret_cast<uint16_t*>(lds) + lane,
                    reinterpret_cast<uint8_t*>(lds) + size_t(P.lds_entries) * kB * 2 + lane};
    else
        stk = reinterpret_cast<StkT>(lds) + lane;
    const uint32_t r = blockIdx.x * uint32_t(kB) + lane;
    bool hit = false, blocked = false, overflow = false;
    uint32_t n_pairs = 0, n_tests = 0;
    if (r < P.n_rays) {
        Hit h{kNoSlot, 0.f, 0.f, 0.f};
        {
            const float4 a = P.rays[2 * size_t(r)], b = P.rays[2 * size_t(r) + 1];
            const CallerRay rk{b.z, b.w};
            hit = trace<false, false, kB, StkT, kRobust, -1, kG>(P, F3{a.x, a.y, a.z}, F3{a.w, b.x, b.y}, stk, h, n_pairs, n_tests,
                                                                 overflow, rk);
        }
        if (P.hits) {
            uint4 rec = make_uint4(0xffffffffu, 0u, 0u, 0u);
            if (hit) rec = make_uint4(P.orig[h.slot], __float_as_uint(h.t), __float_as_uint(h.u), __float_as_uint(h.v));
            P.hits[r] = rec;
        }
        float col[3] = {0.f, 0.f, 0.f};
        if (hit) {
            CERES_COUNT_V(kFShadeV, 48);
            const TriV tr = load_tri(P.tris + h.slot);
            const F3 normal = normalizeG<kG>(tr.n);
            const RayWork w = make_shadow_ray<kRobust, kG>(hit_point<kG>(tr, normal, h.u, h.v), f3(P.sun));
            blocked = trace_any4<false, kB, StkT, kRobust, false, -1, kG>(P, w.o, w.d, stk, n_pairs, n_tests, overflow);
            if (!blocked) {
                const float4 a = P.rays[2 * size_t(r)], b = P.rays[2 * size_t(r) + 1];
                CERES_COUNT_V(kFShadeV, 40);
                shade<kG>(w.d, P.norms + 9 * size_t(P.orig[h.slot]), F3{a.w, b.x, b.y}, h.u, h.v, col);
            }
        }
        CERES_COUNT_V(kFStoreV, (P.pixels ? 12u : 0u) + (P.rgb8 ? 3u : 0u));
        if (P.pixels) {
            float* q = P.pixels + 3 * size_t(r);
            q[0] = col[0]; q[1] = col[1]; q[2] = col[2];
        }
        if (P.rgb8) {
            uint8_t* q = P.rgb8 + 3 * size_t(r);
            q[0] = quantize(col[0]); q[1] = quantize(col[1]); q[2] = quantize(col[2]);
        }
        if (P.status) P.status[r] = hit ? (blocked ? 2 : 1) : 0;
    }
    if (P.counters) {
        const uint32_t nh = __popcll(__ballot(hit)), nb = __popcll(__ballot(blocked));
        if (lane == 0 && nh) {
            atomicAdd(&P.counters[0], (unsigned long long)nh);
            atomicAdd(&P.counters[1], (unsigned long long)(nh + nb));
            atomicAdd(&P.counters[3], (unsigned long long)nh);
        }
        if (blockIdx.x == 0 && lane == 0) {
            atomicAdd(&P.counters[0], (unsigned long long)P.n_rays);
            atomicAdd(&P.counters[2], (unsigned long long)P.n_rays);
        }
        if (overflow) atomicOr(&P.counters[6], 1ull);
    }
}

__device__ __forceinline__ uint32_t rank_rows(uint32_t H, uint32_t rb, uint32_t r, uint32_t world) {
    const uint32_t nb = (H + rb - 1) / rb;
    if (r >= nb) return 0;
    const uint32_t mine = (nb - 1 - r) / world + 1;
    const bool has_last = (nb - 1) % world == r;
    return mine * rb - (has_last ? nb * rb - H : 0);
}

template <bool kVec, bool kPacked = false>
__global__ __launch_bounds__(256) void ceres_assemble(const uint8_t* __restrict__ src, size_t rank_stride,
                                                      uint8_t* __restrict__ dst, uint32_t frames, uint32_t H,
                                                      uint32_t row_bytes, uint32_t rb, uint32_t world) {
    const uint32_t units = kVec ? row_bytes / 16 : row_bytes;
    for (uint32_t oy = blockIdx.y; oy < frames * H; oy += gridDim.y) {
        const uint32_t f = oy / H, y = oy - f * H;
        const uint32_t j = H - 1 - y;
        const uint32_t b = j / rb, r = b % world;
        const uint32_t k = (b / world) * rb + j % rb;
        const uint32_t n = rank_rows(H, rb, r, world);
        size_t base = size_t(r) * rank_stride;
        if (kPacked) {
            base = 0;
            for (uint32_t p = 0; p < r; ++p) base += size_t(frames) * rank_rows(H, rb, p, world) * row_bytes;
        }
        const uint8_t* s = src + base + (size_t(f) * n + (n - 1 - k)) * row_bytes;
        uint8_t* d = dst + size_t(oy) * row_bytes;
        for (uint32_t u = blockIdx.x * blockDim.x + threadIdx.x; u < units; u += gridDim.x * blockDim.x) {
            if (kVec) {
#if CERES_ASSEMBLE_NT
                const U4v x = __builtin_nontemporal_load(reinterpret_cast<const U4v*>(s) + u);
                __builtin_nontemporal_store(x, reinterpret_cast<U4v*>(d) + u);
#else
                reinterpret_cast<uint4*>(d)[u] = reinterpret_cast<const uint4*>(s)[u];
#endif
            }
            else d[u] = s[u];
        }
    }
}

}
}

using namespace ceres;

#include "scene_internal.hpp"

namespace {

#define HIP_TRY(expr)                                                                         \
    do {                                                                                      \
        hipError_t e_ = (expr);                                                               \
        if (e_ != hipSuccess) return set_error(CERES_EHIP, "%s: %s", #expr, hipGetErrorString(e_)); \
    } while (0)

template <typename T>
void dfree(T*& p) { if (p) { (void)hipFree(p); p = nullptr; } }

}

void ceres::scene_release(ceres_scene* s) {
    if (!s) return;
    (void)hipSetDevice(s->device);
    dfree(s->d_pairs64); dfree(s->d_tris64); dfree(s->d_norms64);
    dfree(s->d_src4); dfree(s->d_refit_levels); dfree(s->d_refit_root);
    if (s->d_refit_stage) { (void)hipFree(s->d_refit_stage); s->d_refit_stage = nullptr; }
    for (auto& o : s->orders) dfree(o.d);
    for (auto& d : s->retired) dfree(d);
    s->orders.clear(); s->retired.clear(); s->retired_bytes = 0;
    dfree(s->d_pairs); dfree(s->d_nodes4); dfree(s->d_qnodes4); dfree(s->d_tris); dfree(s->d_orig); dfree(s->d_norms);
    dfree(s->d_shards); dfree(s->d_counters); dfree(s->d_wave_log); dfree(s->d_pixels); dfree(s->d_rgb8);
    for (auto e : s->ev_pool) (void)hipEventDestroy(e);
    for (auto e : s->ev_used) (void)hipEventDestroy(e);
    s->ev_pool.clear(); s->ev_used.clear();
    for (auto e : s->band_events) (void)hipEventDestroy(e);
    s->band_events.clear();
    dfree(s->d_band_counters);
    dfree(s->d_lit); dfree(s->d_lit_count);
    if (s->h_lit_pinned) (void)hipHostFree(s->h_lit_pinned);
    s->h_lit_pinned = nullptr;
    if (s->h_small) (void)hipHostFree(s->h_small);
    s->h_small = nullptr;
    if (s->ev_count) (void)hipEventDestroy(s->ev_count);
    s->ev_count = nullptr;
    if (s->copy_stream) (void)hipStreamDestroy(s->copy_stream);
    s->copy_stream = nullptr;
    if (s->stream) (void)hipStreamDestroy(s->stream);
    s->stream = nullptr;
}

namespace {

size_t local_rows_of(size_t H, uint32_t rb, uint32_t rank, uint32_t world);
size_t local_rows_of(size_t H, const ceres_tiling& t) {
    if (t.bands && t.world > 1) return t.row_block;
    return local_rows_of(H, t.row_block, t.rank, t.world);
}
size_t local_rows_of(size_t H, uint32_t rb, uint32_t rank, uint32_t world) {
    const size_t nblocks = (H + rb - 1) / rb;
    size_t rows = 0;
    for (size_t b = rank; b < nblocks; b += world) rows += std::min<size_t>(rb, H - b * rb);
    return rows;
}

int ensure_workspace(ceres_scene* s, size_t px, bool want_px, bool want_rgb) {
    if ((want_px || want_rgb) && px > s->px_cap) {
        dfree(s->d_pixels); dfree(s->d_rgb8);
        HIP_TRY(hipMalloc(&s->d_pixels, px * 3 * sizeof(float)));
        HIP_TRY(hipMalloc(&s->d_rgb8, px * 3));
        s->px_cap = px;
    }
    return CERES_OK;
}

int upload_tile_order(ceres_scene* s, size_t W, size_t H, const ceres_tiling& t, uint32_t frames, uint32_t tile,
                      std::vector<uint32_t>& order, hipStream_t stream, const uint32_t** out, bool packed,
                      uint32_t bx, uint32_t by) {
    const size_t n = order.size();
    if (packed) {
        const uint32_t per_frame = bx * by;
        for (auto& id : order) {
            const uint32_t f = id / per_frame, rem = id - f * per_frame, y = rem / bx;
            id = pack_tile(f, y, rem - y * bx);
        }
    }
    ceres_scene::TileOrder o;
    if (s->orders.size() >= ceres::kMaxTileOrders) {
        auto lru = std::min_element(s->orders.begin(), s->orders.end(),
                                    [](const auto& a, const auto& b) { return a.used < b.used; });
        s->retired.push_back(lru->d);
        s->retired_bytes += (lru->cap * sizeof(uint32_t) + kAllocGranule - 1) / kAllocGranule * kAllocGranule;
        s->orders.erase(lru);
        if (s->retired_bytes > ceres::kRetiredBytes || s->retired.size() >= ceres::kMaxRetired) {
            HIP_TRY(hipDeviceSynchronize());
            for (auto& d : s->retired) dfree(d);
            s->retired.clear();
            s->retired_bytes = 0;
        }
    }
    o.W = W; o.H = H; o.row_block = t.row_block; o.rank = t.rank; o.world = t.world; o.frames = frames; o.tile = tile;
    o.bands = t.bands;
    o.packed = packed;
    const size_t padded = (n + 7) / 8 * 8;
    if (!o.d) {
        HIP_TRY(hipMalloc(&o.d, padded * sizeof(uint32_t)));
        o.cap = padded;
    }
    if ((padded > n && hipMemsetAsync(o.d + n, 0, (padded - n) * sizeof(uint32_t), stream) != hipSuccess) ||
        hipMemcpyAsync(o.d, order.data(), n * sizeof(uint32_t), hipMemcpyHostToDevice, stream) != hipSuccess ||
        hipStreamSynchronize(stream) != hipSuccess) {
        dfree(o.d);
        return set_error(CERES_EHIP, "tile order upload failed");
    }
    o.used = ++s->order_clock;
    s->orders.push_back(o);
    *out = o.d;
    return CERES_OK;
}

static void xcd_group_rows(std::vector<uint32_t>& order, uint32_t bx, uint32_t per_frame, uint32_t tpw) {
    std::vector<uint32_t> q[8];
    for (auto& v : q) v.reserve(order.size() / 8 + 1);
    for (const uint32_t id : order) {
        const uint32_t f = id / per_frame, rem = id - f * per_frame, y = rem / bx, x = rem - y * bx;
        uint64_t h = (uint64_t(f) << 42) ^ (uint64_t(y) << 21) ^ uint64_t(x / CERES_XCD_GROUP_TILES);
        h *= 0x9e3779b97f4a7c15ull;
        h ^= h >> 29;
        h *= 0xbf58476d1ce4e5b9ull;
        q[(h >> 32) & 7].push_back(id);
    }
    size_t head[8] = {0, 0, 0, 0, 0, 0, 0, 0};
    for (size_t p = 0; p < order.size(); ++p) {
        uint32_t x = uint32_t((p / tpw) % 8);
        if (head[x] == q[x].size()) {
            size_t best = 0;
            for (uint32_t k = 0; k < 8; ++k)
                if (q[k].size() - head[k] > best) { best = q[k].size() - head[k]; x = k; }
        }
        order[p] = q[x][head[x]++];
    }
}

int ensure_tile_order(ceres_scene* s, size_t W, size_t H, const ceres_tiling& t, size_t rows, uint32_t frames,
                      uint32_t bx, uint32_t by, uint32_t tile, hipStream_t stream, const uint32_t** out, bool packed,
                      uint32_t tpw) {
    const uint32_t tile_key = tile | tpw << 16;
    for (auto& o : s->orders)
        if (o.W == W && o.H == H && o.row_block == t.row_block && o.rank == t.rank && o.world == t.world && o.bands == t.bands &&
            o.frames == frames && o.tile == tile_key && o.packed == packed) {
            o.used = ++s->order_clock;
            *out = o.d;
            return CERES_OK;
        }
    const size_t n = size_t(bx) * by * frames;
    const double cx = 0.5 * double(W), cy = 0.5 * double(H);
    std::vector<std::pair<double, uint32_t>> k(n);
    const uint64_t fm_pixels = CERES_FRAME_MAJOR_PIXELS;
    const bool frame_major = fm_pixels != 0 && uint64_t(W) * rows >= fm_pixels;
    for (uint32_t f = 0; f < frames; ++f)
        for (uint32_t y = 0; y < by; ++y) {
            const size_t lr = std::min<size_t>(size_t(y) * tile + tile / 2, rows - 1);
            const size_t j = (t.bands && t.world > 1) ? ((t.rank + f) % t.world) * t.row_block + lr
                                                      : ((lr / t.row_block) * t.world + t.rank) * t.row_block + lr % t.row_block;
            for (uint32_t x = 0; x < bx; ++x) {
                const double dx = double(x) * tile + tile / 2 - cx, dy = double(j) - cy;
                const uint32_t id = (f * by + y) * bx + x;
                k[id] = {dx * dx + dy * dy, id};
            }
        }
    const uint32_t per_frame = bx * by;
    std::stable_sort(k.begin(), k.end(), [frame_major, per_frame](const auto& a, const auto& b) {
        if (frame_major && a.second / per_frame != b.second / per_frame) return a.second < b.second;
        return a.first < b.first;
    });
    std::vector<uint32_t> order(n);
    for (size_t q = 0; q < n; ++q) order[q] = k[q].second;
    const size_t scene_bytes = s->n_pairs * sizeof(SiblingPair) + s->n_nodes4 * sizeof(Node4) +
                               s->n_tri * (sizeof(Tri48) + 4 + 36);
    const size_t lchunk = !CERES_LOCAL_ORDER || !frame_major ? 0
                          : frames > 1 ? size_t(CERES_LOCAL_CHUNK_BATCH)
                          : scene_bytes >= kDramSceneBytes ? size_t(CERES_LOCAL_CHUNK_SOLO) : 0;
    if (lchunk) {
        auto morton = [](uint32_t x, uint32_t y) {
            uint64_t m = 0;
            for (int b = 0; b < 16; ++b) m |= (uint64_t((x >> b) & 1) << (2 * b)) | (uint64_t((y >> b) & 1) << (2 * b + 1));
            return m;
        };
        std::vector<std::pair<uint64_t, uint32_t>> mk(n);
        for (uint32_t id = 0; id < n; ++id) {
            const uint32_t f = id / per_frame, rem = id - f * per_frame, y = rem / bx, x = rem - y * bx;
            mk[id] = {(uint64_t(f) << 40) | morton(x, y), id};
        }
        std::sort(mk.begin(), mk.end());
        const size_t c = std::max<size_t>(tpw, lchunk / tpw * tpw), cw = c / tpw, grp = 8 * c;
        const size_t full = n / grp * grp;
        for (size_t p = 0; p < n; ++p) {
            size_t src = p;
            if (p < full) {
                const size_t w = p / tpw, i = p % tpw, g = w / (8 * cw), wl = w % (8 * cw);
                src = g * grp + (wl % 8) * c + (wl / 8) * tpw + i;
            }
            order[p] = mk[src].second;
        }
        return upload_tile_order(s, W, H, t, frames, tile_key, order, stream, out, packed, bx, by);
    }
    uint64_t st = 0x9e3779b97f4a7c15ull;
    for (size_t b0 = 0; b0 < n; b0 += dev::kTileShuffleWindow) {
        const size_t len = std::min<size_t>(dev::kTileShuffleWindow, n - b0);
        for (size_t q = len - 1; q > 0; --q) {
            st = st * 6364136223846793005ull + 1442695040888963407ull;
            std::swap(order[b0 + q], order[b0 + size_t((st >> 33) % (q + 1))]);
        }
    }
    if (CERES_XCD_GROUP_TILES && frames > 1) xcd_group_rows(order, bx, per_frame, tpw);
    return upload_tile_order(s, W, H, t, frames, tile_key, order, stream, out, packed, bx, by);
}

int quantize_nodes4(const std::vector<Node4>& in, std::vector<QNode4>& out) {
    out.assign(in.size(), QNode4{});
    for (size_t k = 0; k < in.size(); ++k) {
        const Node4& n = in[k];
        QNode4& q = out[k];
        const float* lo[3] = {n.lo_x, n.lo_y, n.lo_z};
        const float* hi[3] = {n.hi_x, n.hi_y, n.hi_z};
        float org[3], scl[3];
        uint32_t ql[3] = {0, 0, 0}, qh[3] = {0, 0, 0};
        for (int a = 0; a < 3; ++a) {
            float mn = INFINITY, mx = -INFINITY;
            for (int c = 0; c < 4; ++c)
                if (n.child[c] != kNode4Empty) { mn = std::min(mn, lo[a][c]); mx = std::max(mx, hi[a][c]); }
            if (mn > mx) { mn = 0.f; mx = 0.f; }
            if (!std::isfinite(mn) || !std::isfinite(mx))
                return set_error(CERES_EUNSUPPORTED, "CERES_MODE_QBVH4: non-finite BVH bounds");
            const double ext = double(mx) - double(mn);
            int e = ext > 0 ? int(std::ceil(std::log2(ext / 250.0))) : -126;
            e = std::max(e, -126);
            float sc = std::ldexp(1.0f, e);
            org[a] = mn;
            for (int c = 0; c < 4; ++c) {
                uint32_t bl = 255, bh = 0;
                if (n.child[c] != kNode4Empty) {
                    double fl = std::floor((double(lo[a][c]) - double(mn)) / double(sc));
                    double fh = std::ceil((double(hi[a][c]) - double(mn)) / double(sc));
                    int il = int(std::max(0.0, std::min(255.0, fl))), ih = int(std::max(0.0, std::min(255.0, fh)));
                    while (il > 0 && std::fma(float(il), sc, mn) > lo[a][c]) --il;
                    while (ih < 255 && std::fma(float(ih), sc, mn) < hi[a][c]) ++ih;
                    if (std::fma(float(il), sc, mn) > lo[a][c] || std::fma(float(ih), sc, mn) < hi[a][c])
                        return set_error(CERES_EUNSUPPORTED, "CERES_MODE_QBVH4: bound not representable");
                    bl = uint32_t(il); bh = uint32_t(ih);
                }
                ql[a] |= bl << (8 * c);
                qh[a] |= bh << (8 * c);
            }
            scl[a] = sc;
        }
        q.ox = org[0]; q.oy = org[1]; q.oz = org[2];
        q.sx = scl[0]; q.sy = scl[1]; q.sz = scl[2];
        q.qlx = ql[0]; q.qhx = qh[0]; q.qly = ql[1]; q.qhy = qh[1]; q.qlz = ql[2]; q.qhz = qh[2];
        for (int c = 0; c < 4; ++c) q.child[c] = n.child[c];
    }
    return CERES_OK;
}

int build_qnodes4(ceres_scene* s) {
    if (!s->n_nodes4 || !s->d_nodes4) return CERES_OK;
    std::vector<Node4> n4(s->n_nodes4);
    HIP_TRY(hipMemcpy(n4.data(), s->d_nodes4, n4.size() * sizeof(Node4), hipMemcpyDeviceToHost));
    std::vector<QNode4> q;
    if (int rc = quantize_nodes4(n4, q)) return rc;
    HIP_TRY(hipMalloc(&s->d_qnodes4, q.size() * sizeof(QNode4)));
    HIP_TRY(hipMemcpy(s->d_qnodes4, q.data(), q.size() * sizeof(QNode4), hipMemcpyHostToDevice));
    return CERES_OK;
}

void set_root_box(ceres_scene* s, const float root[6], const SiblingPair& p0) {
    for (int k = 0; k < 6; ++k) s->root_box[k] = root[k];
    auto inside = [&](const float* c) {
        return c[0] >= root[0] && c[1] <= root[1] && c[2] >= root[2] && c[3] <= root[3] && c[4] >= root[4] && c[5] <= root[5];
    };
    s->root_box_ok = (!s->root_leaf_count && inside(p0.lb) && inside(p0.rb)) ? 1u : 0u;
}

static CullRect cull_rect(const FrameCam& c, const float root[6], uint32_t W, uint32_t H) {
    const CullRect keep{0u, 0xffffu, 0u, 0xffffu};
    if (W > 0xffffu || H > 0xffffu) return keep;
    double e[3], iu[3], iv[3], d[3];
    for (int k = 0; k < 3; ++k) { e[k] = c.eye[k]; iu[k] = c.iu[k]; iv[k] = c.iv[k]; d[k] = c.dir[k]; }
    double sc = 0;
    for (int k = 0; k < 3; ++k) sc = std::max(sc, std::fabs(e[k]));
    for (int k = 0; k < 6; ++k) sc = std::max(sc, std::fabs(double(root[k])));
    const double pad = 1e-4 * sc;
    auto cr = [](const double* a, const double* b, double* o) {
        o[0] = a[1] * b[2] - a[2] * b[1]; o[1] = a[2] * b[0] - a[0] * b[2]; o[2] = a[0] * b[1] - a[1] * b[0]; };
    double c0[3], c1[3], c2[3];
    cr(iv, d, c0); cr(d, iu, c1); cr(iu, iv, c2);
    const double det = iu[0] * c0[0] + iu[1] * c0[1] + iu[2] * c0[2];
    double u0 = HUGE_VAL, u1 = -HUGE_VAL, v0 = HUGE_VAL, v1 = -HUGE_VAL;
    for (int k = 0; k < 8; ++k) {
        const double X[3] = {(k & 1) ? root[1] + pad : root[0] - pad, (k & 2) ? root[3] + pad : root[2] - pad,
                             (k & 4) ? root[5] + pad : root[4] - pad};
        const double r[3] = {X[0] - e[0], X[1] - e[1], X[2] - e[2]};
        const double pw = r[0] * c0[0] + r[1] * c0[1] + r[2] * c0[2], qw = r[0] * c1[0] + r[1] * c1[1] + r[2] * c1[2];
        const double ww = r[0] * c2[0] + r[1] * c2[1] + r[2] * c2[2];
        if (!(ww / det > 0.01 * std::sqrt(r[0] * r[0] + r[1] * r[1] + r[2] * r[2]))) return keep;
        u0 = std::min(u0, pw / ww); u1 = std::max(u1, pw / ww); v0 = std::min(v0, qw / ww); v1 = std::max(v1, qw / ww);
    }
    const double m = 2e-3 * (1 + std::max(std::max(std::fabs(u0), std::fabs(u1)), std::max(std::fabs(v0), std::fabs(v1))));
    auto lo = [](double x, uint32_t n) { return x <= 0 ? 0u : x >= n ? n : uint32_t(std::floor(x)); };
    const double a0 = (u0 - m + 1) * W / 2 - 0.5 - 1, a1 = (u1 + m + 1) * W / 2 - 0.5 + 1;
    const double b0 = (v0 - m + 1) * H / 2 - 0.5 - 1, b1 = (v1 + m + 1) * H / 2 - 0.5 + 1;
    if (!(a0 == a0 && a1 == a1 && b0 == b0 && b1 == b1)) return keep;
    if (a1 < 0 || b1 < 0) return CullRect{1u, 0u, 1u, 0u};
    return CullRect{uint16_t(lo(a0, W)), uint16_t(std::min<double>(std::ceil(a1), 0xffff)),
                    uint16_t(lo(b0, H)), uint16_t(std::min<double>(std::ceil(b1), 0xffff))};
}

static bool launch_culls_a_tile(const KParams& P) {
    const uint32_t tiles_x = (P.W + 7u) / 8u;
    for (uint32_t f = 0; f < P.frames; ++f) {
        const CullRect& r = P.cull_rect[f];
        const bool all_cols = dev::cull_cols_hit(r, P.W, 0) && dev::cull_cols_hit(r, P.W, tiles_x - 1);
        for (uint32_t lr0 = 0; lr0 < P.local_rows; lr0 += 8) {
            bool exists = false, hit = false;
            for (uint32_t lr = lr0; lr < lr0 + 8 && lr < P.local_rows; ++lr) {
                const uint32_t j = P.world == 1 ? lr
                                   : P.bands    ? ((P.rank + f) % P.world) * P.row_block + lr
                                                : ((lr / P.row_block) * P.world + P.rank) * P.row_block + lr % P.row_block;
                if (P.bands && P.world > 1 && j >= P.H) continue;
                exists = true;
                hit = hit || (j >= r.j0 && j <= r.j1);
            }
            if (exists && !(hit && all_cols)) return true;
        }
    }
    return false;
}

static int stack_width(size_t n_pairs, size_t n_nodes4) {
    const size_t nmax = std::max(n_pairs, n_nodes4);
    return CERES_STACK16 && nmax < (1u << 16) ? 2 : CERES_STACK24 && nmax < (1u << 24) ? 3 : 4;
}
static uint32_t batch_tiles_per_wave(size_t frame_pixels, int stw, bool qbvh) {
    if (!CERES_TPW_BY_SIZE || stw != 2 || qbvh) return CERES_TILES_PER_WAVE;
    return frame_pixels >= (size_t(1) << 20) && frame_pixels < (size_t(1) << 22) ? 2u : uint32_t(CERES_TILES_PER_WAVE);
}

static size_t fused_lds_bytes(uint32_t entries, int stw) {
    return size_t(entries) * dev::kFusedB * stw + sizeof(dev::StealLdsT<dev::kFusedB>);
}
static bool lds_limits_waves(uint32_t entries, int stw) { return fused_lds_bytes(entries, stw) > dev::kLdsPerCu / 28; }

static int check_fused_lds(const ceres_scene* s, const KParams& P, int stw, size_t dyn_bytes) {
    const size_t need = size_t(P.lds_entries) * dev::kFusedB * size_t(stw);
    const size_t total = dyn_bytes + sizeof(dev::StealLdsT<dev::kFusedB>);
    if (stw != 2 && stw != 3 && stw != 4)
        return set_error(CERES_EINVAL, "render: bad LDS stack entry width %d", stw);
    if (P.lds_entries < P.stack_entries + 1 || P.lds_entries < P.shadow_stack_entries || dyn_bytes < need)
        return set_error(CERES_EINVAL, "render: LDS stack of %u slots (%zu B) cannot hold the BVH2 stack (%u + 1) and the BVH4 "
                         "stack (%u)", P.lds_entries, dyn_bytes, P.stack_entries, P.shadow_stack_entries);
    if (total > s->max_lds_per_block)
        return set_error(CERES_EINVAL, "render: fused kernel needs %zu B of LDS per workgroup (%zu available)", total,
                         s->max_lds_per_block);
    return CERES_OK;
}

int launch_chunk(ceres_scene* s, uint32_t frames, const float* basis12, const float* sun, int mode, size_t W, size_t H,
                 const ceres_tiling* tiling, float* d_pixels, uint8_t* d_rgb8, uint64_t* d_counters, hipStream_t stream,
                 int32_t* d_rec_prim, float* d_rec_tuv, int8_t* d_rec_shadow, bool first, bool last,
                 uint64_t batch_primary) {
    if (!s || !basis12 || !sun) return set_error(CERES_EINVAL, "render: null argument");
    if (s->f64) return set_error(CERES_EINVAL, "scene is double precision: use ceres_render_f64");
    if (frames == 0 || frames > uint32_t(kFramesPerLaunch))
        return set_error(CERES_EINVAL, "render: %u frames per launch (1..%d)", frames, kFramesPerLaunch);
    const bool robust = (mode & CERES_MODE_ROBUST) != 0;
    const bool qbvh = (mode & CERES_MODE_QBVH4) != 0;
    const bool gfma = (mode & CERES_MODE_FMA) != 0;
    mode &= ~(CERES_MODE_ROBUST | CERES_MODE_QBVH4 | CERES_MODE_FMA);
    if (mode != CERES_MODE_FULL && mode != CERES_MODE_PRIMARY) return set_error(CERES_EINVAL, "render: bad mode %d", mode);
    if (W == 0 || H == 0 || W > 65535u * 16u || H > 0xffffffu) return set_error(CERES_EINVAL, "render: bad size %zux%zu", W, H);
    ceres_tiling t{uint32_t(H), 0, 1};
    if (tiling) t = *tiling;
    if (t.world == 0 || t.rank >= t.world || t.row_block == 0) return set_error(CERES_EINVAL, "render: bad tiling");
    if (t.world == 1) t.bands = 0;
    if (t.bands && (t.bands != 1 || t.world > 65535u || size_t(t.row_block) * t.world < H))
        return set_error(CERES_EINVAL, "render: bands of %u rows x %u ranks do not cover %zu rows", t.row_block, t.world, H);
    const size_t rows = local_rows_of(H, t);
    if (size_t(frames) * W * rows > 0xffffffffull) return set_error(CERES_EINVAL, "render: more than 2^32 pixels per batch");
    const uint32_t bx = uint32_t((W + 15) / 16), by = uint32_t((rows + 15) / 16);
    if (size_t(by) * frames > 65535u) return set_error(CERES_EINVAL, "render: frames x row blocks exceeds the grid limit");
    if ((d_rec_prim != nullptr) != (d_rec_tuv != nullptr) || (d_rec_prim != nullptr) != (d_rec_shadow != nullptr))
        return set_error(CERES_EINVAL, "render: hit records need all three arrays");
    if (qbvh && (robust || (s->flags & CERES_SCENE_STATS)))
        return set_error(CERES_EUNSUPPORTED, "render: CERES_MODE_QBVH4 takes neither CERES_MODE_ROBUST nor a stats scene");
    if (t.bands && (mode != CERES_MODE_FULL || robust || qbvh || (s->flags & CERES_SCENE_STATS) || d_rec_prim))
        return set_error(CERES_EUNSUPPORTED, "render: ceres_tiling.bands takes the full mode of a non-stats scene "
                                             "(not ROBUST, QBVH4, PRIMARY or hit records)");
    HIP_TRY(hipSetDevice(s->device));
    if (qbvh && mode == CERES_MODE_FULL && !s->d_qnodes4)
        if (int rc = build_qnodes4(s)) return rc;

    KParams P{};
    for (uint32_t f = 0; f < frames; ++f) {
        FrameCam& c = P.cam[f];
        std::memcpy(c.eye, basis12 + 12 * f, 12); std::memcpy(c.dir, basis12 + 12 * f + 3, 12);
        std::memcpy(c.iu, basis12 + 12 * f + 6, 12); std::memcpy(c.iv, basis12 + 12 * f + 9, 12);
        std::memcpy(c.sun, sun + 3 * f, 12);
    }
    P.frames = frames;
    P.W = uint32_t(W); P.H = uint32_t(H);
    P.row_block = t.row_block; P.rank = t.rank; P.world = t.world; P.local_rows = uint32_t(rows);
    P.bands = t.bands;
    P.band_magic = t.bands ? uint32_t(((uint64_t(1) << 32) + t.world - 1) / t.world) : 0u;
    P.row_blocks_per_frame = by;
    P.stack_entries = s->stack_entries;
    P.shadow_stack_entries = s->shadow_stack_entries;
    P.packets = (s->n_pairs * sizeof(SiblingPair) + s->n_nodes4 * sizeof(Node4) + s->n_tri * sizeof(Tri48)) <
                kDramSceneBytes ? 1u : 0u;
    P.root_leaf_count = s->root_leaf_count; P.root_leaf_first = s->root_leaf_first;
    for (int k = 0; k < 6; ++k) P.root_box[k] = s->root_box[k];
    P.root_box_ok = CERES_ROOT_TEST ? s->root_box_ok : 0u;
    P.cull = (CERES_CULL && P.root_box_ok && !(s->flags & CERES_SCENE_STATS) && !d_rec_prim && W <= 0xffffu && H <= 0xffffu) ? 1u : 0u;
    uint32_t fill_tasks = 0;
    if (P.cull) {
        for (uint32_t f = 0; f < frames; ++f) P.cull_rect[f] = cull_rect(P.cam[f], P.root_box, P.W, P.H);
        if (rows && launch_culls_a_tile(P)) fill_tasks = frames * uint32_t((rows + 7) / 8);
        else P.cull = 0u;
    }
    P.pairs = s->d_pairs; P.nodes4 = s->d_nodes4; P.tris = s->d_tris; P.orig = s->d_orig; P.norms = s->d_norms;
    P.qnodes4 = s->d_qnodes4;
    P.pixels = d_pixels; P.rgb8 = d_rgb8; P.shards = s->d_shards;
    P.rec_prim = d_rec_prim; P.rec_tuv = d_rec_tuv; P.rec_shadow = d_rec_shadow;

    const bool stats = (s->flags & CERES_SCENE_STATS) != 0;
    const bool full = mode == CERES_MODE_FULL;
    hipEvent_t e0 = nullptr, e1 = nullptr;
    if (s->timing && rows) {
        while (s->ev_pool.size() < 2) { hipEvent_t e; HIP_TRY(hipEventCreate(&e)); s->ev_pool.push_back(e); }
        e0 = s->ev_pool.back(); s->ev_pool.pop_back();
        e1 = s->ev_pool.back(); s->ev_pool.pop_back();
        s->ev_used.push_back(e0); s->ev_used.push_back(e1);
    }
    constexpr uint32_t ftile = 8;
    const uint32_t fbx = uint32_t((W + ftile - 1) / ftile), fby = uint32_t((rows + ftile - 1) / ftile);
    const uint32_t* tile_order = nullptr;
    const bool packed = frames <= (1u << (32 - kTileXBits - kTileYBits)) &&
                        fbx <= (1u << kTileXBits) && fby <= (1u << kTileYBits);
    const uint32_t tpw = (!stats && (frames > 1 || t.bands)) ? batch_tiles_per_wave(size_t(W) * rows, stack_width(s->n_pairs, s->n_nodes4), qbvh)
                                                : 1u;
    if (full && rows)
        if (int rc = ensure_tile_order(s, W, H, t, rows, frames, fbx, fby, ftile, stream, &tile_order, packed, tpw)) return rc;
    const bool need_clean = d_counters || !full;
    if (first && need_clean && s->shards_dirty) HIP_TRY(hipMemsetAsync(s->d_shards, 0, sizeof(Shard) * kShards, stream));
    s->shards_dirty = true;
    if (rows) {
        if (e0) HIP_TRY(hipEventRecord(e0, stream));
        if (full) {
            const int stw = stack_width(s->n_pairs, s->n_nodes4);
            const bool st16 = stw == 2;
            const bool steal = frames == 1 && !t.bands;
            P.steal_first = steal && !stats && ((s->flags & CERES_SCENE_FIRST_ORDER) ||
                                                lds_limits_waves(std::max(s->stack_entries + 1, s->shadow_stack_entries), stw))
                                ? 1u : 0u;
            P.shadow_stack_entries = (!steal || P.steal_first) ? s->shadow_stack_first : s->shadow_stack_entries;
            P.lds_entries = uint32_t(std::max(s->stack_entries + 1, P.shadow_stack_entries));
            const size_t flds = size_t(P.lds_entries) * dev::kFusedB * stw;
            if (int rc = check_fused_lds(s, P, stw, flds)) return rc;
            if (!stats)
                if (const char* g = std::getenv("CERES_DEBUG_GUARD_SLOT")) {
                    const long k = std::strtol(g, nullptr, 10);
                    if (k > 0 && uint32_t(k) < P.stack_entries) P.stack_entries = uint32_t(k);
                }
            P.tile_order = tile_order;
            P.tile_packed = packed ? 1u : 0u;
            P.tiles_x = fbx;
            P.row_blocks_per_frame = fby;
            const uint32_t n_tiles = fbx * fby * frames;
            const uint32_t tile_groups = (n_tiles + tpw - 1) / tpw;
            dim3 fgrid(tile_groups + fill_tasks), fblock(dev::kFusedB);
            if (CERES_FILL_SPREAD > (steal ? 1 : 0) && fill_tasks) {
                const uint64_t nto = (tile_groups + 7) / 8, nfo = (fill_tasks + 7) / 8, stride = (nto + nfo) / nfo;
                if (stride >= 2 && (nto + nfo) * stride < (uint64_t(1) << 32)) {
                    fgrid.x = uint32_t((nto + nfo) * 8);
                    P.fill_stride = uint32_t(stride);
                    P.fill_magic = uint32_t(((uint64_t(1) << 32) + stride - 1) / stride);
                }
            }
            if (stats) {
                const size_t waves = size_t(fbx) * fby * frames;
                if (s->wave_log_waves < waves) {
                    dfree(s->d_wave_log);
                    HIP_TRY(hipMalloc(&s->d_wave_log, waves * 64));
                    s->wave_log_waves = waves;
                }
                HIP_TRY(hipMemsetAsync(s->d_wave_log, 0, waves * 64, stream));
                P.wave_log = s->d_wave_log;
                s->last_grid_waves = waves;
            }
            constexpr int w32 = CERES_FUSED_MINW32;
            auto fused = [&](auto rt, auto st, auto gt) {
                constexpr bool R = decltype(rt)::value, T = decltype(st)::value, G = decltype(gt)::value;
                constexpr int w16 = T ? CERES_FUSED_MINW16_SOLO : CERES_FUSED_MINW16;
                if constexpr (!R) {
                    if (qbvh) {
                        if (st16) hipLaunchKernelGGL((dev::ceres_fused<false, uint16_t*, w16, false, T, true, G>), fgrid, fblock, flds, stream, P);
                        else if (stw == 3) hipLaunchKernelGGL((dev::ceres_fused<false, dev::Stk24, w32, false, T, true, G>), fgrid, fblock, flds, stream, P);
                        else hipLaunchKernelGGL((dev::ceres_fused<false, uint32_t*, w32, false, T, true, G>), fgrid, fblock, flds, stream, P);
                        return;
                    }
                }
                if (stats && st16) hipLaunchKernelGGL((dev::ceres_fused<true, uint16_t*, 1, R, T, false, G>), fgrid, fblock, flds, stream, P);
                else if (stats && stw == 3) hipLaunchKernelGGL((dev::ceres_fused<true, dev::Stk24, w32, R, T, false, G>), fgrid, fblock, flds, stream, P);
                else if (stats) hipLaunchKernelGGL((dev::ceres_fused<true, uint32_t*, w32, R, T, false, G>), fgrid, fblock, flds, stream, P);
                else if (st16) {
                    if constexpr (!T) {
                        if (tpw == 2) { hipLaunchKernelGGL((dev::ceres_fused<false, uint16_t*, w16, R, T, false, G, 2>), fgrid, fblock, flds, stream, P); return; }
                    }
                    constexpr int w16b = T ? CERES_FUSED_MINW16_SOLO : CERES_FUSED_MINW16_TPW4;
                    hipLaunchKernelGGL((dev::ceres_fused<false, uint16_t*, w16b, R, T, false, G>), fgrid, fblock, flds, stream, P);
                }
                else if (stw == 3) hipLaunchKernelGGL((dev::ceres_fused<false, dev::Stk24, w32, R, T, false, G>), fgrid, fblock, flds, stream, P);
                else hipLaunchKernelGGL((dev::ceres_fused<false, uint32_t*, w32, R, T, false, G>), fgrid, fblock, flds, stream, P);
            };
            auto fused_g = [&](auto rt, auto st) {
                if (gfma) fused(rt, st, std::true_type{});
                else fused(rt, st, std::false_type{});
            };
            auto fused_s = [&](auto rt) {
                if (steal) fused_g(rt, std::true_type{});
                else fused_g(rt, std::false_type{});
            };
            auto fused_bands = [&](auto gt) {
                constexpr bool G = decltype(gt)::value;
                if (st16) {
                    if (tpw == 2) hipLaunchKernelGGL((dev::ceres_fused<false, uint16_t*, CERES_FUSED_MINW16, false, false, false, G, 2, true>), fgrid, fblock, flds, stream, P);
                    else hipLaunchKernelGGL((dev::ceres_fused<false, uint16_t*, CERES_FUSED_MINW16_TPW4, false, false, false, G, 0, true>), fgrid, fblock, flds, stream, P);
                } else if (stw == 3) hipLaunchKernelGGL((dev::ceres_fused<false, dev::Stk24, w32, false, false, false, G, 0, true>), fgrid, fblock, flds, stream, P);
                else hipLaunchKernelGGL((dev::ceres_fused<false, uint32_t*, w32, false, false, false, G, 0, true>), fgrid, fblock, flds, stream, P);
            };
            if (t.bands) {
                if (gfma) fused_bands(std::true_type{});
                else fused_bands(std::false_type{});
            } else if (robust) fused_s(std::true_type{});
            else fused_s(std::false_type{});
        } else {
            const size_t lds = size_t(s->stack_entries + 1) * dev::kBlock * 4;
            if (lds > s->max_lds_per_block)
                return set_error(CERES_EINVAL, "render: primary-only traversal stack needs %zu B of LDS per workgroup (%zu available)",
                                 lds, s->max_lds_per_block);
            uint32_t fill_y = (((fill_tasks + dev::kBlock / 64 - 1) / (dev::kBlock / 64)) + bx - 1) / bx;
            if (size_t(by) * frames + fill_y > 65535u) { P.cull = 0u; fill_y = 0; }
            const dim3 grid(bx, by * frames + fill_y), block(dev::kBlock);
            auto primary = [&](auto rt, auto gt) {
                constexpr bool R = decltype(rt)::value, G = decltype(gt)::value;
                if (stats) hipLaunchKernelGGL((dev::ceres_primary<true, R, G>), grid, block, lds, stream, P);
                else hipLaunchKernelGGL((dev::ceres_primary<false, R, G>), grid, block, lds, stream, P);
            };
            auto primary_g = [&](auto rt) {
                if (gfma) primary(rt, std::true_type{});
                else primary(rt, std::false_type{});
            };
            if (robust) primary_g(std::true_type{});
            else primary_g(std::false_type{});
        }
        HIP_TRY(hipGetLastError());
        if (e1) HIP_TRY(hipEventRecord(e1, stream));
    }
    if (d_counters && last) {
        hipLaunchKernelGGL(dev::ceres_finalize, dim3(1), dim3(64), 0, stream, s->d_shards,
                           batch_primary, d_counters);
        HIP_TRY(hipGetLastError());
        s->shards_dirty = false;
    }
    return CERES_OK;
}

int launch(ceres_scene* s, uint32_t frames, const float* basis12, const float* sun, int mode, size_t W, size_t H,
           const ceres_tiling* tiling, float* d_pixels, uint8_t* d_rgb8, uint64_t* d_counters, hipStream_t stream,
           int32_t* d_rec_prim = nullptr, float* d_rec_tuv = nullptr, int8_t* d_rec_shadow = nullptr) {
    if (frames == 0 || frames > uint32_t(kMaxFrames))
        return set_error(CERES_EINVAL, "render: %u frames per batch (1..%d)", frames, kMaxFrames);
    if (!basis12 || !sun) return set_error(CERES_EINVAL, "render: null argument");
    ceres_tiling t{uint32_t(H), 0, 1};
    if (tiling) t = *tiling;
    if (t.world == 0 || t.rank >= t.world || t.row_block == 0) return set_error(CERES_EINVAL, "render: bad tiling");
    uint64_t primary = uint64_t(frames) * W * local_rows_of(H, t);
    if (t.bands && t.world > 1) {
        primary = 0;
        for (uint32_t f = 0; f < frames; ++f) {
            const size_t b = (t.rank + f) % t.world, top = b * size_t(t.row_block);
            primary += uint64_t(W) * (top < H ? std::min<size_t>(t.row_block, H - top) : 0);
        }
    }
    if (frames <= uint32_t(kFramesPerLaunch))
        return launch_chunk(s, frames, basis12, sun, mode, W, H, tiling, d_pixels, d_rgb8, d_counters, stream, d_rec_prim,
                            d_rec_tuv, d_rec_shadow, true, true, primary);
    const size_t fp = W * local_rows_of(H, t);
    const uint32_t n_launch = (frames + kFramesPerLaunch - 1) / kFramesPerLaunch;
    for (uint32_t c = 0, f0 = 0; c < n_launch; ++c) {
        const uint32_t n = frames / n_launch + (c < frames % n_launch ? 1u : 0u);
        const size_t o = size_t(f0) * fp;
        ceres_tiling tc = t;
        if (t.bands) tc.rank = (t.rank + f0) % t.world;
        if (int rc = launch_chunk(s, n, basis12 + 12 * size_t(f0), sun + 3 * size_t(f0), mode, W, H, &tc,
                                  d_pixels ? d_pixels + 3 * o : nullptr, d_rgb8 ? d_rgb8 + 3 * o : nullptr, d_counters,
                                  stream, d_rec_prim ? d_rec_prim + o : nullptr, d_rec_tuv ? d_rec_tuv + 3 * o : nullptr,
                                  d_rec_shadow ? d_rec_shadow + o : nullptr, f0 == 0, f0 + n >= frames, primary))
            return rc;
        f0 += n;
    }
    return CERES_OK;
}

void fill_stats(ceres_stats* st, const uint64_t c[8], double ms) {
    if (!st) return;
    st->rays = c[0]; st->hits = c[1]; st->primary_rays = c[2]; st->shadow_rays = c[3];
    st->node_pairs = c[4]; st->tri_tests = c[5]; st->ms = ms;
}

}

namespace ceres {
int scene_after_refit(ceres_scene* s, const float root[6], const SiblingPair& p0) {
    set_root_box(s, root, p0);
    dfree(s->d_qnodes4);
    return CERES_OK;
}
int frame_tile_order(ceres_scene* s, size_t W, size_t H, uint32_t tile, hipStream_t stream, const uint32_t** out) {
    const ceres_tiling t{uint32_t(H), 0, 1};
    return ensure_tile_order(s, W, H, t, H, 1, uint32_t((W + tile - 1) / tile), uint32_t((H + tile - 1) / tile), tile,
                             stream, out, false, 1u);
}
}

extern "C" {

const char* ceres_last_error(void) { return error_buffer(); }
extern const char ceres_src_sha[];
const char* ceres_version(void) {
    static const std::string v = std::string("ceres-mi355x 0.4 (gfx950) src ") + ceres_src_sha;
    return v.c_str();
}
int ceres_device_count(void) {
    int n = 0;
    if (hipGetDeviceCount(&n) != hipSuccess) return set_error(CERES_EHIP, "hipGetDeviceCount failed");
    return n;
}
const char* ceres_kernel_names(void) {
    return "ceres_fused,ceres_primary,ceres_finalize,ceres_assemble,ceres_trace_rays_k,ceres_trace_rays64_k,ceres_shade_rays_k,ceres_shade_rays64_k";
}

size_t ceres_tiling_local_rows(size_t height, const ceres_tiling* t) {
    if (!t) return height;
    if (t->world == 0 || t->row_block == 0 || t->rank >= t->world) return 0;
    return local_rows_of(height, *t);
}

ceres_scene* ceres_scene_create(const float* tri48, size_t n_tri, const float* norm36, const void* nodes32,
                                size_t n_nodes, const uint64_t* prim64, int device, uint32_t flags) {
    if (!tri48 || !norm36 || !nodes32 || !prim64 || n_tri == 0 || n_nodes == 0) {
        set_error(CERES_EINVAL, "ceres_scene_create: empty scene or null argument");
        return nullptr;
    }
    if (n_tri > 0xffffffffull || n_nodes > 0xffffffffull) { set_error(CERES_EUNSUPPORTED, "scene too large"); return nullptr; }
    std::vector<SiblingPair> pairs;
    std::vector<Tri48> leaf_tris;
    std::vector<uint32_t> orig;
    uint32_t depth = 0, rlc = 0, rlf = 0;
    if (relayout_bvh(static_cast<const RefNode*>(nodes32), n_nodes, prim64, n_tri, reinterpret_cast<const Tri48*>(tri48),
                     pairs, leaf_tris, orig, depth, rlc, rlf))
        return nullptr;
    std::vector<Node4> nodes4;
    std::vector<uint32_t> src4;
    uint32_t stack4 = 0, not_collapsed = 0;
    if (!rlc && build_shadow_bvh4(pairs, nodes4, stack4, not_collapsed, &src4)) return nullptr;

    uint32_t stack4_first = stack4;
    if (!rlc && ((flags & CERES_SCENE_FIRST_ORDER) ||
                 lds_limits_waves(std::max(depth + 1, stack4), stack_width(pairs.size(), nodes4.size()))) &&
        order_shadow_bvh4(nodes4, stack4_first, &src4))
        return nullptr;
    if (nodes4.empty()) nodes4.emplace_back();
    src4.resize(nodes4.size() * 4, kNode4NoSource);
    auto* s = new (std::nothrow) ceres_scene;
    if (!s) { set_error(CERES_ENOMEM, "out of host memory"); return nullptr; }
    s->n_nodes4 = nodes4.size();
    s->shadow_stack_entries = std::max<uint32_t>(1, stack4);
    s->shadow_stack_first = std::max<uint32_t>(1, std::min(stack4, stack4_first));
    s->device = device; s->flags = flags; s->n_tri = n_tri; s->n_pairs = pairs.size();
    s->depth = depth; s->root_leaf_count = rlc; s->root_leaf_first = rlf;
    s->stack_entries = std::max<uint32_t>(1, depth);
    set_root_box(s, static_cast<const RefNode*>(nodes32)[0].bounds, pairs[0]);
    auto fail = [&]() -> ceres_scene* { scene_release(s); delete s; return nullptr; };
    int ndev = 0;
    if (hipGetDeviceCount(&ndev) != hipSuccess || ndev == 0) { set_error(CERES_EHIP, "no HIP device available"); return fail(); }
    if (device < 0 || device >= ndev) { set_error(CERES_EINVAL, "device %d out of range (%d devices)", device, ndev); return fail(); }
    auto body = [&]() -> int {
        HIP_TRY(hipSetDevice(device));
        hipDeviceProp_t prop;
        HIP_TRY(hipGetDeviceProperties(&prop, device));
        if (std::strncmp(prop.gcnArchName, "gfx950", 6) != 0)
            return set_error(CERES_EHIP, "device %d is %s, this build targets gfx950 only", device, prop.gcnArchName);
        s->num_cus = prop.multiProcessorCount;
        s->max_lds_per_block = prop.sharedMemPerBlock;
        HIP_TRY(hipStreamCreateWithFlags(&s->stream, hipStreamNonBlocking));
        HIP_TRY(hipMalloc(&s->d_pairs, pairs.size() * sizeof(SiblingPair)));
        HIP_TRY(hipMalloc(&s->d_nodes4, nodes4.size() * sizeof(Node4)));
        HIP_TRY(hipMemcpy(s->d_nodes4, nodes4.data(), nodes4.size() * sizeof(Node4), hipMemcpyHostToDevice));
        HIP_TRY(hipMalloc(&s->d_src4, src4.size() * sizeof(uint32_t)));
        HIP_TRY(hipMemcpy(s->d_src4, src4.data(), src4.size() * sizeof(uint32_t), hipMemcpyHostToDevice));
        HIP_TRY(hipMalloc(&s->d_tris, n_tri * sizeof(Tri48)));
        HIP_TRY(hipMalloc(&s->d_orig, n_tri * sizeof(uint32_t)));
        HIP_TRY(hipMalloc(&s->d_norms, n_tri * 36));
        HIP_TRY(hipMalloc(&s->d_shards, sizeof(Shard) * kShards));
        HIP_TRY(hipMalloc(&s->d_counters, 8 * sizeof(uint64_t)));
        HIP_TRY(hipMemcpy(s->d_pairs, pairs.data(), pairs.size() * sizeof(SiblingPair), hipMemcpyHostToDevice));
        HIP_TRY(hipMemcpy(s->d_tris, leaf_tris.data(), n_tri * sizeof(Tri48), hipMemcpyHostToDevice));
        HIP_TRY(hipMemcpy(s->d_orig, orig.data(), n_tri * sizeof(uint32_t), hipMemcpyHostToDevice));
        HIP_TRY(hipMemcpy(s->d_norms, norm36, n_tri * 36, hipMemcpyHostToDevice));
        return CERES_OK;
    };
    if (body()) return fail();
    return s;
}

ceres_scene* ceres_scene_create_device(const float* d_tri48, size_t n_tri, const float* d_norm36, const uint32_t* d_nodes32,
                                       size_t n_nodes, const uint32_t* d_prim32, int device, uint32_t flags, void* stream) {
    if (!d_tri48 || !d_norm36 || !d_nodes32 || !d_prim32 || n_tri == 0 || n_nodes == 0) {
        set_error(CERES_EINVAL, "ceres_scene_create_device: empty scene or null argument");
        return nullptr;
    }
    if (n_tri > 0xffffffffull || n_nodes > 0xffffffffull) { set_error(CERES_EUNSUPPORTED, "scene too large"); return nullptr; }
    auto* s = new (std::nothrow) ceres_scene;
    if (!s) { set_error(CERES_ENOMEM, "out of host memory"); return nullptr; }
    DeviceLayout L;
    auto fail = [&]() -> ceres_scene* {
        if (L.pairs) (void)hipFree(L.pairs);
        if (L.nodes4) (void)hipFree(L.nodes4);
        if (L.tris) (void)hipFree(L.tris);
        if (L.orig) (void)hipFree(L.orig);
        if (L.src4) (void)hipFree(L.src4);
        scene_release(s); delete s; return nullptr;
    };
    int ndev = 0;
    if (hipGetDeviceCount(&ndev) != hipSuccess || ndev == 0) { set_error(CERES_EHIP, "no HIP device available"); return fail(); }
    if (device < 0 || device >= ndev) { set_error(CERES_EINVAL, "device %d out of range (%d devices)", device, ndev); return fail(); }
    s->device = device; s->flags = flags; s->n_tri = n_tri;
    auto body = [&]() -> int {
        HIP_TRY(hipSetDevice(device));
        hipDeviceProp_t prop;
        HIP_TRY(hipGetDeviceProperties(&prop, device));
        if (std::strncmp(prop.gcnArchName, "gfx950", 6) != 0)
            return set_error(CERES_EHIP, "device %d is %s, this build targets gfx950 only", device, prop.gcnArchName);
        s->num_cus = prop.multiProcessorCount;
        s->max_lds_per_block = prop.sharedMemPerBlock;
        HIP_TRY(hipStreamCreateWithFlags(&s->stream, hipStreamNonBlocking));
        hipStream_t st = stream ? static_cast<hipStream_t>(stream) : s->stream;
        if (int rc = relayout_device(reinterpret_cast<const Tri48*>(d_tri48), uint32_t(n_tri),
                                     reinterpret_cast<const RefNode*>(d_nodes32), uint32_t(n_nodes), d_prim32, st, L))
            return rc;
        s->d_pairs = L.pairs; s->d_nodes4 = L.nodes4; s->d_tris = L.tris; s->d_orig = L.orig;
        s->d_src4 = L.src4;
        s->n_pairs = L.n_pairs; s->n_nodes4 = L.n_nodes4;
        s->depth = L.depth; s->root_leaf_count = L.root_leaf_count; s->root_leaf_first = L.root_leaf_first;
        s->stack_entries = std::max<uint32_t>(1, L.depth);
        s->shadow_stack_entries = std::max<uint32_t>(1, L.stack4);
        s->shadow_stack_first = s->shadow_stack_entries;
        if (!L.root_leaf_count) {
            SiblingPair p0;
            HIP_TRY(hipMemcpyAsync(&p0, L.pairs, sizeof p0, hipMemcpyDeviceToHost, st));
            HIP_TRY(hipStreamSynchronize(st));
            set_root_box(s, L.root_box, p0);
        }
        L = DeviceLayout{};
        HIP_TRY(hipMalloc(&s->d_norms, n_tri * 36));
        HIP_TRY(hipMemcpyAsync(s->d_norms, d_norm36, n_tri * 36, hipMemcpyDeviceToDevice, st));
        HIP_TRY(hipMalloc(&s->d_shards, sizeof(Shard) * kShards));
        HIP_TRY(hipMalloc(&s->d_counters, 8 * sizeof(uint64_t)));
        HIP_TRY(hipStreamSynchronize(st));
        return CERES_OK;
    };
    if (body()) return fail();
    return s;
}

void ceres_scene_destroy(ceres_scene* s) {
    if (!s) return;
    scene_release(s);
    delete s;
}

int ceres_scene_info(const ceres_scene* s, uint32_t* depth, uint32_t* stack_entries, size_t* n_pairs, size_t* device_bytes) {
    if (!s) return set_error(CERES_EINVAL, "null scene");
    if (depth) *depth = s->depth;
    if (stack_entries) *stack_entries = s->stack_entries;
    if (n_pairs) *n_pairs = s->n_pairs;
    if (device_bytes)
        *device_bytes = s->n_pairs * sizeof(SiblingPair) + s->n_nodes4 * sizeof(Node4) + s->n_tri * (sizeof(Tri48) + 4 + 36);
    return CERES_OK;
}

int ceres_scene_shadow_stacks(const ceres_scene* s, uint32_t* nearest_first, uint32_t* first_passing) {
// ... 397 lines not shown
        return CERES_OK;
    }
    HIP_TRY(hipSetDevice(s->device));
    void* dr = nullptr; void* dh = nullptr; uint8_t* dc = nullptr;
    hipEvent_t e0 = nullptr, e1 = nullptr;
    auto cleanup = [&] {
        dfree(dr); dfree(dh); dfree(dc);
        if (e0) (void)hipEventDestroy(e0);
        if (e1) (void)hipEventDestroy(e1);
    };
    if (hipMalloc(&dr, n_rays * 32) != hipSuccess || (hits16 && hipMalloc(&dh, n_rays * 16) != hipSuccess) ||
        (occluded && hipMalloc(&dc, n_rays) != hipSuccess)) {
        cleanup();
        return set_error(CERES_ENOMEM, "ceres_trace_rays: device allocation failed");
    }
    float ms = 0.f;
    int rc = CERES_OK;
    if (hipEventCreate(&e0) != hipSuccess || hipEventCreate(&e1) != hipSuccess ||
        hipMemcpyAsync(dr, rays32, n_rays * 32, hipMemcpyHostToDevice, s->stream) != hipSuccess ||
        hipEventRecord(e0, s->stream) != hipSuccess)
        rc = set_error(CERES_EHIP, "ceres_trace_rays: upload failed");
    if (!rc) rc = ceres_trace_rays_device(s, dr, n_rays, mode, dh, dc, s->d_counters, s->stream);
    if (!rc && (hipEventRecord(e1, s->stream) != hipSuccess ||
                hipMemcpyAsync(c, s->d_counters, sizeof c, hipMemcpyDeviceToHost, s->stream) != hipSuccess ||
                (hits16 && hipMemcpyAsync(hits16, dh, n_rays * 16, hipMemcpyDeviceToHost, s->stream) != hipSuccess) ||
                (occluded && hipMemcpyAsync(occluded, dc, n_rays, hipMemcpyDeviceToHost, s->stream) != hipSuccess) ||
                hipStreamSynchronize(s->stream) != hipSuccess || hipEventElapsedTime(&ms, e0, e1) != hipSuccess))
        rc = set_error(CERES_EHIP, "ceres_trace_rays: copy back failed");
    cleanup();
    if (rc) return rc;
    fill_stats(stats, c, double(ms));
    if (c[6]) return set_error(CERES_ESTACK, "traversal stack overflow");
    return CERES_OK;
}

static int check_shade_args(const ceres_scene* s, const void* rays, size_t n_rays, const float* sun, int mode, bool any_output) {
    if (!s) return set_error(CERES_EINVAL, "ceres_shade_rays: null scene");
    if (s->f64) return set_error(CERES_EUNSUPPORTED, "ceres_shade_rays: the scene is double precision (use ceres_shade_rays_f64)");
    if (mode & ~(CERES_MODE_FMA | CERES_MODE_ROBUST))
        return set_error(CERES_EINVAL, "ceres_shade_rays: bad mode %d (0, CERES_MODE_FMA, CERES_MODE_ROBUST or both)", mode);
    if (!any_output) return set_error(CERES_EINVAL, "ceres_shade_rays: none of pixels, rgb8, hits and status asked for");
    if (n_rays >= (size_t(1) << 31)) return set_error(CERES_EUNSUPPORTED, "ceres_shade_rays: %zu rays (below 2^31 per call)", n_rays);
    if (n_rays == 0) return 1;
    if (!rays || !sun) return set_error(CERES_EINVAL, "ceres_shade_rays: null rays or sun");
    return 0;
}

int ceres_shade_rays_device(ceres_scene* s, const void* d_rays32, size_t n_rays, const float sun[3], int mode, float* d_pixels,
                            uint8_t* d_rgb8, void* d_hits16, uint8_t* d_status, uint64_t* d_counters, void* stream_) {
    if (const int chk = check_shade_args(s, d_rays32, n_rays, sun, mode, d_pixels || d_rgb8 || d_hits16 || d_status))
        return chk < 0 ? chk : CERES_OK;
    if ((reinterpret_cast<uintptr_t>(d_rays32) | reinterpret_cast<uintptr_t>(d_hits16)) & 15u)
        return set_error(CERES_EINVAL, "ceres_shade_rays: rays and hits must be 16-byte aligned");
    if (reinterpret_cast<uintptr_t>(d_pixels) & 3u) return set_error(CERES_EINVAL, "ceres_shade_rays: pixels must be 4-byte aligned");
    hipStream_t stream = static_cast<hipStream_t>(stream_);
    HIP_TRY(hipSetDevice(s->device));
    dev::ShadeParams P{};
    P.rays = static_cast<const float4*>(d_rays32);
    P.pixels = d_pixels; P.rgb8 = d_rgb8;
    P.hits = static_cast<uint4*>(d_hits16);
    P.status = d_status;
    P.counters = reinterpret_cast<unsigned long long*>(d_counters);
    P.pairs = s->d_pairs; P.nodes4 = s->d_nodes4; P.tris = s->d_tris; P.orig = s->d_orig; P.norms = s->d_norms;
    P.n_rays = uint32_t(n_rays);
    P.stack_entries = s->stack_entries;
    P.shadow_stack_entries = s->shadow_stack_entries;
    P.lds_entries = std::max(s->stack_entries + 1, s->shadow_stack_entries);
    P.root_leaf_count = s->root_leaf_count; P.root_leaf_first = s->root_leaf_first;
    for (int k = 0; k < 6; ++k) P.root_box[k] = s->root_box[k];
    P.root_box_ok = s->root_box_ok;
    for (int k = 0; k < 3; ++k) P.sun[k] = sun[k];
    const int stw = stack_width(s->n_pairs, s->n_nodes4);
    const size_t lds = size_t(P.lds_entries) * dev::kFusedB * size_t(stw);
    if (P.lds_entries < P.stack_entries + 1 || P.lds_entries < P.shadow_stack_entries)
        return set_error(CERES_EINVAL, "ceres_shade_rays: LDS stack of %u slots cannot hold the BVH2 stack (%u + 1) and the BVH4 "
                         "stack (%u)", P.lds_entries, P.stack_entries, P.shadow_stack_entries);
    if (lds > s->max_lds_per_block)
        return set_error(CERES_EINVAL, "ceres_shade_rays: traversal stacks need %zu B of LDS per workgroup (%zu available)", lds,
                         s->max_lds_per_block);
    if (d_counters) HIP_TRY(hipMemsetAsync(d_counters, 0, 8 * sizeof(uint64_t), stream));
    const dim3 grid(uint32_t((n_rays + dev::kFusedB - 1) / dev::kFusedB)), block(dev::kFusedB);
    const bool robust = (mode & CERES_MODE_ROBUST) != 0, gfma = (mode & CERES_MODE_FMA) != 0;
    auto go = [&](auto rt, auto gt) {
        constexpr bool R = decltype(rt)::value, G = decltype(gt)::value;
        if (stw == 2) hipLaunchKernelGGL((dev::ceres_shade_rays_k<uint16_t*, R, G>), grid, block, lds, stream, P);
        else if (stw == 3) hipLaunchKernelGGL((dev::ceres_shade_rays_k<dev::Stk24, R, G>), grid, block, lds, stream, P);
        else hipLaunchKernelGGL((dev::ceres_shade_rays_k<uint32_t*, R, G>), grid, block, lds, stream, P);
    };
    auto go_g = [&](auto rt) {
        if (gfma) go(rt, std::true_type{});
        else go(rt, std::false_type{});
    };
    if (robust) go_g(std::true_type{});
    else go_g(std::false_type{});
    HIP_TRY(hipGetLastError());
    return CERES_OK;
}

int ceres_shade_rays(ceres_scene* s, const void* rays32, size_t n_rays, const float sun[3], int mode, float* pixels,
                     uint8_t* rgb8, void* hits16, uint8_t* status, ceres_stats* stats) {
    uint64_t c[8] = {0};
    if (const int chk = check_shade_args(s, rays32, n_rays, sun, mode, pixels || rgb8 || hits16 || status)) {
        if (chk < 0) return chk;
        fill_stats(stats, c, 0.0);
        return CERES_OK;
    }
    HIP_TRY(hipSetDevice(s->device));
    void* dr = nullptr; void* dh = nullptr; float* dp = nullptr; uint8_t* dq = nullptr; uint8_t* ds = nullptr;
    hipEvent_t e0 = nullptr, e1 = nullptr;
    auto cleanup = [&] {
        dfree(dr); dfree(dh); dfree(dp); dfree(dq); dfree(ds);
        if (e0) (void)hipEventDestroy(e0);
        if (e1) (void)hipEventDestroy(e1);
    };
    if (hipMalloc(&dr, n_rays * 32) != hipSuccess || (hits16 && hipMalloc(&dh, n_rays * 16) != hipSuccess) ||
        (pixels && hipMalloc(&dp, n_rays * 12) != hipSuccess) || (rgb8 && hipMalloc(&dq, n_rays * 3) != hipSuccess) ||
        (status && hipMalloc(&ds, n_rays) != hipSuccess)) {
        cleanup();
        return set_error(CERES_ENOMEM, "ceres_shade_rays: device allocation failed");
    }
    float ms = 0.f;
    int rc = CERES_OK;
    if (hipEventCreate(&e0) != hipSuccess || hipEventCreate(&e1) != hipSuccess ||
        hipMemcpyAsync(dr, rays32, n_rays * 32, hipMemcpyHostToDevice, s->stream) != hipSuccess ||
        hipEventRecord(e0, s->stream) != hipSuccess)
        rc = set_error(CERES_EHIP, "ceres_shade_rays: upload failed");
    if (!rc) rc = ceres_shade_rays_device(s, dr, n_rays, sun, mode, dp, dq, dh, ds, s->d_counters, s->stream);
    if (!rc && (hipEventRecord(e1, s->stream) != hipSuccess ||
                hipMemcpyAsync(c, s->d_counters, sizeof c, hipMemcpyDeviceToHost, s->stream) != hipSuccess ||
                (pixels && hipMemcpyAsync(pixels, dp, n_rays * 12, hipMemcpyDeviceToHost, s->stream) != hipSuccess) ||
                (rgb8 && hipMemcpyAsync(rgb8, dq, n_rays * 3, hipMemcpyDeviceToHost, s->stream) != hipSuccess) ||
                (hits16 && hipMemcpyAsync(hits16, dh, n_rays * 16, hipMemcpyDeviceToHost, s->stream) != hipSuccess) ||
                (status && hipMemcpyAsync(status, ds, n_rays, hipMemcpyDeviceToHost, s->stream) != hipSuccess) ||
                hipStreamSynchronize(s->stream) != hipSuccess || hipEventElapsedTime(&ms, e0, e1) != hipSuccess))
        rc = set_error(CERES_EHIP, "ceres_shade_rays: copy back failed");
    cleanup();
    if (rc) return rc;
    fill_stats(stats, c, double(ms));
    if (c[6]) return set_error(CERES_ESTACK, "traversal stack overflow");
    return CERES_OK;
}

int ceres_scene_wave_log(ceres_scene* s, uint64_t* out, size_t max_waves, size_t* n_waves) {
    if (!s || !out || !n_waves) return set_error(CERES_EINVAL, "ceres_scene_wave_log: null argument");
    if (!s->d_wave_log) return set_error(CERES_EINVAL, "wave log needs a CERES_SCENE_STATS scene and a full-mode render");
    HIP_TRY(hipSetDevice(s->device));
    HIP_TRY(hipDeviceSynchronize());
    const size_t n = std::min(max_waves, s->last_grid_waves);
    HIP_TRY(hipMemcpy(out, s->d_wave_log, n * 64, hipMemcpyDeviceToHost));
    *n_waves = n;
    return CERES_OK;
}

int ceres_fetch_counters(int device, uint64_t out[8], int reset) {
    if (!out) return set_error(CERES_EINVAL, "ceres_fetch_counters: null argument");
#if CERES_COUNTING
    static_assert(dev::kFKinds == 8, "ceres_fetch_counters reports 8 kinds");
    HIP_TRY(hipSetDevice(device));
    HIP_TRY(hipDeviceSynchronize());
    unsigned long long h[dev::kFetchShards][dev::kFKinds];
    HIP_TRY(hipMemcpyFromSymbol(h, HIP_SYMBOL(dev::g_fetch), sizeof h));
    for (int k = 0; k < dev::kFKinds; ++k) {
        out[k] = 0;
        for (int q = 0; q < dev::kFetchShards; ++q) out[k] += h[q][k];
    }
    if (reset) {
        std::memset(h, 0, sizeof h);
        HIP_TRY(hipMemcpyToSymbol(HIP_SYMBOL(dev::g_fetch), h, sizeof h));
    }
    return CERES_OK;
#else
    (void)device; (void)reset;
    std::memset(out, 0, 8 * sizeof(uint64_t));
    return set_error(CERES_EUNSUPPORTED, "ceres_fetch_counters: only the counting build (make count) tallies fetches");
#endif
}

int ceres_scene_set_timing(ceres_scene* s, int enable) {
    if (!s) return set_error(CERES_EINVAL, "null scene");
    s->timing = enable != 0;
    return CERES_OK;
}

int ceres_scene_read_timing(ceres_scene* s, double* kernel_ms, double* shadow_ms, uint64_t* renders) {
    if (!s) return set_error(CERES_EINVAL, "null scene");
    HIP_TRY(hipSetDevice(s->device));
    double p = 0;
    const size_t n = s->ev_used.size() / 2;
    for (size_t k = 0; k < n; ++k) {
        hipEvent_t e0 = s->ev_used[2 * k], e1 = s->ev_used[2 * k + 1];
        HIP_TRY(hipEventSynchronize(e1));
        float a = 0.f;
        HIP_TRY(hipEventElapsedTime(&a, e0, e1));
        p += a;
    }
    for (auto e : s->ev_used) s->ev_pool.push_back(e);
    s->ev_used.clear();
    if (kernel_ms) *kernel_ms = p;
    if (shadow_ms) *shadow_ms = 0.0;
    if (renders) *renders = n;
    return CERES_OK;
}

}
```

### ceres-raytracer_amd/csrc/scene_internal.hpp

```cpp
#pragma once
#include <hip/hip_runtime.h>

#include <cstdint>
#include <utility>
#include <vector>

#include "ceres_types.hpp"

using ceres::SiblingPair; using ceres::SiblingPair64; using ceres::Node4; using ceres::Tri48; using ceres::Tri96;
using ceres::Shard;

struct ceres_scene {
    int device = 0;
    uint32_t flags = 0;
    size_t n_tri = 0, n_pairs = 0;
    uint32_t depth = 0, stack_entries = 1, root_leaf_count = 0, root_leaf_first = 0;
    float root_box[6] = {0, 0, 0, 0, 0, 0};
    uint32_t root_box_ok = 0;
    uint32_t shadow_stack_entries = 1;
    uint32_t shadow_stack_first = 1;
    size_t n_nodes4 = 0;
    SiblingPair* d_pairs = nullptr;
    Node4* d_nodes4 = nullptr;
    ceres::QNode4* d_qnodes4 = nullptr;
    struct TileOrder {
        size_t W = 0, H = 0;
        uint32_t row_block = 0, rank = 0, world = 0, frames = 0, tile = 0, bands = 0;
        bool packed = false;
        uint32_t* d = nullptr;
        size_t cap = 0;
        uint64_t used = 0;
    };
    std::vector<TileOrder> orders;
    std::vector<uint32_t*> retired;
    size_t retired_bytes = 0;
    uint64_t order_clock = 0;
    Tri48* d_tris = nullptr;
    uint32_t* d_orig = nullptr;
    float* d_norms = nullptr;
    Shard* d_shards = nullptr;
    bool shards_dirty = true;
    uint64_t* d_counters = nullptr;
    float* d_pixels = nullptr;
    uint8_t* d_rgb8 = nullptr;
    size_t px_cap = 0;
    hipStream_t stream = nullptr;
    hipStream_t copy_stream = nullptr;
    uint64_t* d_band_counters = nullptr;
    std::vector<hipEvent_t> band_events;
    uint4* d_lit = nullptr;
    uint32_t* d_lit_count = nullptr;
    size_t lit_cap = 0;
    uint32_t* h_small = nullptr;
    std::vector<uint4> h_lit;
    uint4* h_lit_pinned = nullptr;
    bool lit_zc = false;
    double last_lit_frac = 0.0;
    uint32_t dense_calls = 0;
    hipEvent_t ev_count = nullptr;
    int num_cus = 256;
    size_t max_lds_per_block = 64 * 1024;
    unsigned long long* d_wave_log = nullptr;
    size_t wave_log_waves = 0, last_grid_waves = 0;
    bool timing = false;
    std::vector<hipEvent_t> ev_pool;
    std::vector<hipEvent_t> ev_used;
    bool f64 = false;
    SiblingPair64* d_pairs64 = nullptr;
    Tri96* d_tris64 = nullptr;
    double* d_norms64 = nullptr;
    uint32_t* d_src4 = nullptr;
    uint32_t* d_refit_levels = nullptr;
    std::vector<uint32_t> refit_level_off;
    float* d_refit_root = nullptr;
    void* d_refit_stage = nullptr;
};

namespace ceres {
void host_fill_zero(float* dst, size_t n);
void host_scatter_lit(float* dst, const uint32_t* lit4, size_t n);
void scene_release(ceres_scene* s);
int scene_after_refit(ceres_scene* s, const float root[6], const SiblingPair& p0);
int frame_tile_order(ceres_scene* s, size_t W, size_t H, uint32_t tile, hipStream_t stream, const uint32_t** out);
constexpr size_t kMaxTileOrders = 16;
constexpr size_t kDramSceneBytes = size_t(64) << 20;
#ifndef CERES_RETIRED_BYTES
#define CERES_RETIRED_BYTES (64u << 20)
#endif
constexpr size_t kRetiredBytes = CERES_RETIRED_BYTES;
constexpr size_t kMaxRetired = 64;
constexpr size_t kAllocGranule = 4096;
}
```

### include/ceres_render.h

```cpp
#ifndef CERES_RENDER_H
#define CERES_RENDER_H

#include <stddef.h>
#include <stdint.h>

#ifdef __cplusplus
extern "C" {
#endif

typedef enum {
    CERES_OK = 0,
    CERES_EINVAL = -1,
    CERES_EIO = -2,
    CERES_ENOMEM = -3,
    CERES_EHIP = -4,
    CERES_ESTACK = -5,
    CERES_EUNSUPPORTED = -6
} ceres_status;

typedef enum {
    CERES_MODE_FULL = 0,
    CERES_MODE_PRIMARY = 1,
    CERES_MODE_ROBUST = 0x10,
    CERES_MODE_QBVH4 = 0x20,
// ... 11 lines not shown
    uint64_t primary_rays, shadow_rays;
    uint64_t node_pairs;
    uint64_t tri_tests;
    double   ms;
} ceres_stats;

typedef struct {
    uint32_t row_block, rank, world;
    uint32_t bands;
} ceres_tiling;


int ceres_obj_load(const char* path, float** tri48, float** norm36, size_t* n_tri);
int ceres_proc_mesh(int n, float** tri48, float** norm36, size_t* n_tri);
int ceres_rotate_triangles(float* tri48, size_t n_tri, int axis, float degrees);
int ceres_bvh_build(const float* tri48, size_t n_tri, uint32_t** nodes32, size_t* n_nodes, uint64_t** prim64);
int ceres_bvh_build_gpu(const float* tri48, size_t n_tri, uint32_t** nodes32, size_t* n_nodes, uint64_t** prim64,
                        int device);
int ceres_bvh_build_device(const float* d_tri48, size_t n_tri, uint32_t* d_nodes32, uint32_t* d_prim32,
                           size_t* n_nodes, void* stream);
int ceres_obj_load_gpu(const char* path, float** tri48, float** norm36, size_t* n_tri, int device);
int ceres_obj_parse_device(const char* d_text, size_t len, float** d_tri48, float** d_norm36, size_t* n_tri,
                           void* stream);
int ceres_rotate_triangles_device(float* d_tri48, size_t n_tri, int axis, float degrees, void* stream);
void ceres_device_free(void* d_ptr);
int ceres_bvh_build_gpu_arith(const float* tri48, size_t n_tri, uint32_t** nodes32, size_t* n_nodes, uint64_t** prim64,
                              int device, int arith);
int ceres_bvh_build_device_arith(const float* d_tri48, size_t n_tri, uint32_t* d_nodes32, uint32_t* d_prim32,
                                 size_t* n_nodes, void* stream, int arith);
int ceres_obj_load_gpu_arith(const char* path, float** tri48, float** norm36, size_t* n_tri, int device, int arith);
int ceres_obj_parse_device_arith(const char* d_text, size_t len, float** d_tri48, float** d_norm36, size_t* n_tri,
                                 void* stream, int arith);
int ceres_rotate_triangles_device_arith(float* d_tri48, size_t n_tri, int axis, float degrees, void* stream, int arith);
int ceres_camera_basis(const float eye[3], const float dir[3], const float up[3], float fov_deg,
                       size_t width, size_t height, float out9[9]);
int ceres_orbit_cameras(const float eye[3], const float dir[3], const float up[3], const float sun[3],
                        float fov_deg, size_t width, size_t height, const float axis[3], float step_deg,
                        uint32_t n_frames, int rotate_first, float* basis12, float* sun3, float* dir3);
void ceres_free(void* p);
int ceres_obj_load_arith(const char* path, float** tri48, float** norm36, size_t* n_tri, int arith);
int ceres_proc_mesh_arith(int n, float** tri48, float** norm36, size_t* n_tri, int arith);
int ceres_rotate_triangles_arith(float* tri48, size_t n_tri, int axis, float degrees, int arith);
int ceres_bvh_build_arith(const float* tri48, size_t n_tri, uint32_t** nodes32, size_t* n_nodes, uint64_t** prim64,
                          int arith);
int ceres_camera_basis_arith(const float eye[3], const float dir[3], const float up[3], float fov_deg,
                             size_t width, size_t height, float out9[9], int arith);
int ceres_orbit_cameras_arith(const float eye[3], const float dir[3], const float up[3], const float sun[3],
                              float fov_deg, size_t width, size_t height, const float axis[3], float step_deg,
                              uint32_t n_frames, int rotate_first, float* basis12, float* sun3, float* dir3, int arith);

int ceres_obj_load_f64(const char* path, double** tri96, double** norm72, size_t* n_tri);
int ceres_proc_mesh_f64(int n, double** tri96, double** norm72, size_t* n_tri);
int ceres_rotate_triangles_f64(double* tri96, size_t n_tri, int axis, double degrees);
int ceres_bvh_build_f64(const double* tri96, size_t n_tri, uint64_t** nodes64, size_t* n_nodes, uint64_t** prim64);
int ceres_camera_basis_f64(const double eye[3], const double dir[3], const double up[3], double fov_deg,
                           size_t width, size_t height, double out9[9]);
int ceres_orbit_cameras_f64(const double eye[3], const double dir[3], const double up[3], const double sun[3],
                            double fov_deg, size_t width, size_t height, const double axis[3], double step_deg,
                            uint32_t n_frames, int rotate_first, double* basis12, double* sun3, double* dir3);
int ceres_obj_load_f64_arith(const char* path, double** tri96, double** norm72, size_t* n_tri, int arith);
int ceres_proc_mesh_f64_arith(int n, double** tri96, double** norm72, size_t* n_tri, int arith);
int ceres_rotate_triangles_f64_arith(double* tri96, size_t n_tri, int axis, double degrees, int arith);
int ceres_bvh_build_f64_arith(const double* tri96, size_t n_tri, uint64_t** nodes64, size_t* n_nodes,
                              uint64_t** prim64, int arith);
int ceres_camera_basis_f64_arith(const double eye[3], const double dir[3], const double up[3], double fov_deg,
                                 size_t width, size_t height, double out9[9], int arith);
int ceres_orbit_cameras_f64_arith(const double eye[3], const double dir[3], const double up[3], const double sun[3],
                                  double fov_deg, size_t width, size_t height, const double axis[3], double step_deg,
                                  uint32_t n_frames, int rotate_first, double* basis12, double* sun3, double* dir3,
                                  int arith);


#define CERES_SCENE_STATS 1u
#define CERES_SCENE_FIRST_ORDER 2u

ceres_scene* ceres_scene_create(const float* tri48, size_t n_tri, const float* norm36,
                                const void* nodes32, size_t n_nodes, const uint64_t* prim64,
                                int device, uint32_t flags);
ceres_scene* ceres_scene_create_device(const float* d_tri48, size_t n_tri, const float* d_norm36,
                                       const uint32_t* d_nodes32, size_t n_nodes, const uint32_t* d_prim32,
                                       int device, uint32_t flags, void* stream);
ceres_scene* ceres_scene_create_f64(const double* tri96, size_t n_tri, const double* norm72, const void* nodes64,
                                    size_t n_nodes, const uint64_t* prim64, int device, uint32_t flags);
void ceres_scene_destroy(ceres_scene* scene);
int ceres_scene_info(const ceres_scene* scene, uint32_t* depth, uint32_t* stack_entries,
                     size_t* n_pairs, size_t* device_bytes);
int ceres_scene_shadow_stacks(const ceres_scene* scene, uint32_t* nearest_first, uint32_t* first_passing);

int ceres_scene_refit(ceres_scene* scene, const float* tri48, size_t n_tri, const float* norm36);
int ceres_scene_refit_device(ceres_scene* scene, const float* d_tri48, size_t n_tri, const float* d_norm36, void* stream);
int ceres_scene_refit_f64(ceres_scene* scene, const double* tri96, size_t n_tri, const double* norm72);
int ceres_scene_refit_f64_device(ceres_scene* scene, const double* d_tri96, size_t n_tri, const double* d_norm72,
                                 void* stream);
int ceres_scene_read_boxes(ceres_scene* scene, void* pair_boxes, size_t* n_pairs, float* node4_boxes, size_t* n_nodes4);


int ceres_render_f32(ceres_scene* scene, const float basis12[12], const float sun[3], int mode,
                     float* pixels, uint8_t* rgb8, size_t width, size_t height, ceres_stats* stats);

int ceres_render_device(ceres_scene* scene, const float basis12[12], const float sun[3], int mode,
                        size_t width, size_t height, const ceres_tiling* tiling,
                        float* d_pixels, uint8_t* d_rgb8, uint64_t* d_counters, void* stream);
int ceres_render_batch_device(ceres_scene* scene, uint32_t frames, const float* basis12,
                              const float* sun3, int mode, size_t width, size_t height,
                              const ceres_tiling* tiling, float* d_pixels, uint8_t* d_rgb8,
                              uint64_t* d_counters, void* stream);
int ceres_assemble_rgb8(const uint8_t* d_gathered, size_t rank_stride_bytes, uint8_t* d_out, uint32_t frames,
                        size_t width, size_t height, uint32_t row_block, uint32_t world, void* stream);
int ceres_device_count(void);
int ceres_render_multi_f32(ceres_scene* const* scenes, uint32_t world, uint32_t row_block,
                           const float basis12[12], const float sun[3], int mode, float* pixels,
                           uint8_t* rgb8, size_t width, size_t height, ceres_stats* stats);
int ceres_assemble_rgb8_packed(const uint8_t* d_gathered, uint8_t* d_out, uint32_t frames, size_t width,
                               size_t height, uint32_t row_block, uint32_t world, void* stream);
int ceres_render_records(ceres_scene* scene, const float basis12[12], const float sun[3], int mode,
                         size_t width, size_t height, int32_t* prim, float* tuv, int8_t* shadow,
                         ceres_stats* stats);
size_t ceres_tiling_local_rows(size_t height, const ceres_tiling* tiling);
int ceres_render_f64(ceres_scene* scene, const double basis12[12], const double sun[3], int mode,
                     double* pixels, uint8_t* rgb8, size_t width, size_t height, ceres_stats* stats);
int ceres_render_records_f64(ceres_scene* scene, const double basis12[12], const double sun[3], int mode,
                             size_t width, size_t height, int32_t* prim, double* tuv, int8_t* shadow,
                             ceres_stats* stats);

int ceres_trace_rays_device(ceres_scene* scene, const void* d_rays32, size_t n_rays, int mode, void* d_hits16,
                            uint8_t* d_occluded, uint64_t* d_counters, void* stream);
int ceres_trace_rays(ceres_scene* scene, const void* rays32, size_t n_rays, int mode, void* hits16, uint8_t* occluded,
                     ceres_stats* stats);

int ceres_trace_rays_f64_device(ceres_scene* scene, const void* d_rays64, size_t n_rays, int mode, void* d_hits32,
                                uint8_t* d_occluded, uint64_t* d_counters, void* stream);
int ceres_trace_rays_f64(ceres_scene* scene, const void* rays64, size_t n_rays, int mode, void* hits32, uint8_t* occluded,
                         ceres_stats* stats);

int ceres_shade_rays_device(ceres_scene* scene, const void* d_rays32, size_t n_rays, const float sun[3], int mode,
                            float* d_pixels, uint8_t* d_rgb8, void* d_hits16, uint8_t* d_status, uint64_t* d_counters,
                            void* stream);
int ceres_shade_rays(ceres_scene* scene, const void* rays32, size_t n_rays, const float sun[3], int mode, float* pixels,
                     uint8_t* rgb8, void* hits16, uint8_t* status, ceres_stats* stats);
int ceres_camera_rays(const float basis12[12], size_t width, size_t height, int arith, void* rays32);

int ceres_shade_rays_f64_device(ceres_scene* scene, const void* d_rays64, size_t n_rays, const double sun[3], int mode,
                                double* d_pixels, uint8_t* d_rgb8, void* d_hits32, uint8_t* d_status, uint64_t* d_counters,
                                void* stream);
int ceres_shade_rays_f64(ceres_scene* scene, const void* rays64, size_t n_rays, const double sun[3], int mode, double* pixels,
                         uint8_t* rgb8, void* hits32, uint8_t* status, ceres_stats* stats);
int ceres_camera_rays_f64(const double basis12[12], size_t width, size_t height, int arith, void* rays64);

int ceres_scene_set_timing(ceres_scene* scene, int enable);
int ceres_scene_read_timing(ceres_scene* scene, double* kernel_ms, double* shadow_ms, uint64_t* renders);

int ceres_scene_wave_log(ceres_scene* scene, uint64_t* out, size_t max_waves, size_t* n_waves);

int ceres_fetch_counters(int device, uint64_t out[8], int reset);

typedef struct ceres_cpu_scene ceres_cpu_scene;
ceres_cpu_scene* ceres_cpu_scene_create(const float* tri48, size_t n_tri, const float* norm36, const void* nodes32,
                                        size_t n_nodes, const uint64_t* prim64);
void ceres_cpu_scene_destroy(ceres_cpu_scene* scene);
int ceres_render_cpu_f32(const ceres_cpu_scene* scene, const float basis12[12], const float sun[3], int mode,
                         float* pixels, uint8_t* rgb8, size_t width, size_t height, ceres_stats* stats, int threads);
ceres_cpu_scene* ceres_cpu_scene_create_f64(const double* tri96, size_t n_tri, const double* norm72, const void* nodes64,
                                            size_t n_nodes, const uint64_t* prim64);
int ceres_render_cpu_f64(const ceres_cpu_scene* scene, const double basis12[12], const double sun[3], int mode,
                         double* pixels, uint8_t* rgb8, size_t width, size_t height, ceres_stats* stats, int threads);
int ceres_cpu_scene_refit(ceres_cpu_scene* scene, const float* tri48, size_t n_tri, const float* norm36);
int ceres_cpu_scene_refit_f64(ceres_cpu_scene* scene, const double* tri96, size_t n_tri, const double* norm72);
int ceres_trace_rays_cpu(const ceres_cpu_scene* scene, const void* rays32, size_t n_rays, int mode, void* hits16,
                         uint8_t* occluded, ceres_stats* stats, int threads);
int ceres_trace_rays_cpu_f64(const ceres_cpu_scene* scene, const void* rays64, size_t n_rays, int mode, void* hits32,
                             uint8_t* occluded, ceres_stats* stats, int threads);

int ceres_shade_rays_cpu(const ceres_cpu_scene* scene, const void* rays32, size_t n_rays, const float sun[3], int mode,
                         float* pixels, uint8_t* rgb8, void* hits16, uint8_t* status, ceres_stats* stats, int threads);
int ceres_shade_rays_cpu_f64(const ceres_cpu_scene* scene, const void* rays64, size_t n_rays, const double sun[3], int mode,
                             double* pixels, uint8_t* rgb8, void* hits32, uint8_t* status, ceres_stats* stats, int threads);

uint64_t ceres_content_hash(const void* p, size_t bytes);

const char* ceres_kernel_names(void);

const char* ceres_last_error(void);
const char* ceres_version(void);

#ifdef __cplusplus
}
#endif

#endif
```

Baseline: 50000 Mrays/s.

## Compact tile order on device to drop culled tile groups before fused launch

```diff
diff --git a/ceres-raytracer_amd/__init__.py b/ceres-raytracer_amd/__init__.py
--- a/ceres-raytracer_amd/__init__.py
+++ b/ceres-raytracer_amd/__init__.py
@@ -36,6 +36,7 @@
     "ceres_free", "ceres_scene_create", "ceres_scene_create_device", "ceres_scene_destroy", "ceres_scene_info", "ceres_scene_shadow_stacks", "ceres_render_f32",
     "ceres_render_device", "ceres_render_batch_device", "ceres_render_multi_f32", "ceres_device_count", "ceres_assemble_rgb8_packed", "ceres_render_records", "ceres_tiling_local_rows",
     "ceres_scene_set_timing", "ceres_scene_read_timing", "ceres_scene_wave_log", "ceres_fetch_counters",
+    "ceres_debug_compact_order", "ceres_debug_kept_tiles",
     "ceres_cpu_scene_create", "ceres_cpu_scene_destroy", "ceres_render_cpu_f32", "ceres_cpu_scene_create_f64",
     "ceres_render_cpu_f64",
     "ceres_orbit_cameras", "ceres_assemble_rgb8",
@@ -174,6 +175,10 @@
                                           _u64p]
     L.ceres_scene_wave_log.argtypes = [_vp, _u64p, _sz, ctypes.POINTER(_sz)]
     L.ceres_fetch_counters.argtypes = [ctypes.c_int, _u64p, ctypes.c_int]
+    if hasattr(L, "ceres_debug_compact_order"):
+        L.ceres_debug_compact_order.argtypes = [_vp, _u32p, _u32p, _u32p, _sz]
+        L.ceres_debug_kept_tiles.argtypes = [_sz, _sz, ctypes.c_uint32, ctypes.c_uint32, ctypes.POINTER(ctypes.c_uint16), _u32p,
+                                             _u32p, _sz]
     L.ceres_cpu_scene_create.argtypes = [_fp, _sz, _fp, _vp, _sz, _u64p]
     L.ceres_cpu_scene_create.restype = _vp
     L.ceres_cpu_scene_destroy.argtypes = [_vp]
@@ -722,6 +727,18 @@
         _check(lib().ceres_scene_wave_log(self._h, _p(out, ctypes.c_uint64), max_waves, ctypes.byref(n)))
         return out[: 8 * n.value].reshape(-1, 8)
 
+    def compact_order(self):
+        info = np.zeros(8, np.uint32)
+        _check(lib().ceres_debug_compact_order(self._h, _p(info, ctypes.c_uint32), None, None, 0))
+        if not info[0]:
+            return None
+        cap = int(info[6]) + 16
+        order, source = np.zeros(cap, np.uint32), np.zeros(cap, np.uint32)
+        _check(lib().ceres_debug_compact_order(self._h, _p(info, ctypes.c_uint32), _p(order, ctypes.c_uint32),
+                                               _p(source, ctypes.c_uint32), cap))
+        return {"host_tiles": int(info[1]), "device_tiles": int(info[2]), "groups": int(info[3]), "tpw": int(info[4]),
+                "deal": int(info[5]), "order": order[:(int(info[2]) + 7) // 8 * 8], "source": source[:int(info[6])]}
+
     def read_timing(self):
         p, q, n = ctypes.c_double(), ctypes.c_double(), ctypes.c_uint64()
         _check(lib().ceres_scene_read_timing(self._h, ctypes.byref(p), ctypes.byref(q), ctypes.byref(n)))
@@ -851,6 +868,18 @@
     return lib().ceres_tiling_local_rows(H, ctypes.byref(tiling))
 
 
+def kept_tiles(W, H, frames, tpw, rects):
+    r = np.ascontiguousarray(rects, np.uint16).reshape(frames, 4)
+    info = np.zeros(4, np.uint32)
+    n = ((W + 7) // 8) * ((H + 7) // 8) * frames
+    src = np.zeros(n, np.uint32)
+    _check(lib().ceres_debug_kept_tiles(W, H, frames, tpw, _p(r, ctypes.c_uint16), _p(info, ctypes.c_uint32),
+                                        _p(src, ctypes.c_uint32), n))
+    assert int(info[1]) == n
+    how = "boxes" if info[3] & 4 else "walk" if info[3] & 2 else None
+    return {"tiles": int(info[0]), "deal": int(info[2]), "packed": bool(info[3] & 1), "count": how, "source": src}
+
+
 def row_map(H, row_block, world):
     out = []
     nb = (H + row_block - 1) // row_block
diff --git a/ceres-raytracer_amd/csrc/ceres_types.hpp b/ceres-raytracer_amd/csrc/ceres_types.hpp
--- a/ceres-raytracer_amd/csrc/ceres_types.hpp
+++ b/ceres-raytracer_amd/csrc/ceres_types.hpp
@@ -148,7 +148,17 @@
     int8_t* rec_shadow;
     unsigned long long* wave_log;
     uint32_t fill_stride, fill_magic;
+    uint32_t n_tiles;
 };
+
+struct CompactArgs {
+    uint32_t* buf;
+    uint32_t tpw;
+    uint32_t deal;
+    uint32_t want_tiles;
+    uint32_t off_result, off_counts, off_rows;
+};
+static_assert(sizeof(KParams) + sizeof(CompactArgs) <= 4096, "KParams + CompactArgs must fit the 4 KB kernel-argument limit");
 static_assert(sizeof(KParams) <= 4096, "KParams must fit the 4 KB kernel-argument limit");
 
 struct DeviceLayout {
diff --git a/ceres-raytracer_amd/csrc/render_hip.hip b/ceres-raytracer_amd/csrc/render_hip.hip
--- a/ceres-raytracer_amd/csrc/render_hip.hip
+++ b/ceres-raytracer_amd/csrc/render_hip.hip
@@ -81,6 +81,9 @@
 #endif
 #ifndef CERES_CULL
 #define CERES_CULL 1
+#endif
+#ifndef CERES_COMPACT
+#define CERES_COMPACT 1
 #endif
 #ifndef CERES_TRI_SELECT
 #define CERES_TRI_SELECT 1
@@ -1240,8 +1243,7 @@
         stk = reinterpret_cast<StkT>(lds) + tid;
     constexpr uint32_t kTile = 8;
     constexpr uint32_t kTPW = (kStats || kSteal) ? 1 : kTPWo ? uint32_t(kTPWo) : uint32_t(CERES_TILES_PER_WAVE);
-    const uint32_t per_frame = P.tiles_x * P.row_blocks_per_frame;
-    const uint32_t n_tiles = per_frame * P.frames;
+    const uint32_t n_tiles = P.n_tiles;
     uint32_t group = blockIdx.x;
     if constexpr (!kStats) {
         const uint32_t tile_groups = (n_tiles + kTPW - 1) / kTPW;
@@ -1370,6 +1372,116 @@
     if (overflow) atomicOr(&P.shards[shard].error, 1u);
 }
 
+__device__ __forceinline__ void order_tile(const KParams& P, uint32_t t, uint32_t& f, uint32_t& by, uint32_t& bx) {
+    if (P.tile_packed) {
+        bx = t & ((1u << kTileXBits) - 1u);
+        by = (t >> kTileXBits) & ((1u << kTileYBits) - 1u);
+        f = t >> (kTileXBits + kTileYBits);
+    } else {
+        const uint32_t per_frame = P.tiles_x * P.row_blocks_per_frame;
+        f = t / per_frame;
+        const uint32_t rem = t - f * per_frame;
+        by = rem / P.tiles_x; bx = rem - by * P.tiles_x;
+    }
+}
+
+__global__ __launch_bounds__(256) void ceres_cull_rows(const KParams P, const CompactArgs A) {
+    const uint32_t lane = threadIdx.x & 63u, task = blockIdx.x * 4u + (threadIdx.x >> 6);
+    const uint32_t tile_rows = P.row_blocks_per_frame;
+    const uint32_t f = task / tile_rows, by = task - f * tile_rows;
+    if (f >= P.frames) return;
+    const bool hit = tile_rows_hit(P, f, by * 8u + (lane & 7u));
+    if (lane == 0) A.buf[A.off_rows + task] = hit ? 1u : 0u;
+}
+
+__device__ __forceinline__ bool group_kept(const KParams& P, const CompactArgs& A, uint32_t g) {
+    bool keep = false;
+    for (uint32_t i = 0; i < A.tpw; ++i) {
+        const uint32_t p = g * A.tpw + i;
+        if (p >= P.n_tiles) break;
+        uint32_t f, by, bx;
+        order_tile(P, P.tile_order[p], f, by, bx);
+        if (f >= P.frames || by >= P.row_blocks_per_frame) continue;
+        keep = keep || !tile_misses_root(P, f, bx, A.buf[A.off_rows + f * P.row_blocks_per_frame + by] != 0u);
+    }
+    return keep;
+}
+
+constexpr uint32_t kCompactBlock = 1024;
+
+__device__ __forceinline__ uint32_t block_sum_256(uint32_t x, uint32_t* sh) {
+    x = wave_sum(x);
+    __syncthreads();
+    if ((threadIdx.x & 63u) == 0) sh[threadIdx.x >> 6] = x;
+    __syncthreads();
+    return sh[0] + sh[1] + sh[2] + sh[3];
+}
+
+__global__ __launch_bounds__(256) void ceres_order_count(const KParams P, const CompactArgs A) {
+    __shared__ uint32_t sh[4];
+    const uint32_t groups = (P.n_tiles + A.tpw - 1u) / A.tpw, g0 = blockIdx.x * kCompactBlock + threadIdx.x * 4u;
+    uint32_t c = 0;
+    for (uint32_t k = 0; k < 4u; ++k)
+        if (g0 + k < groups && group_kept(P, A, g0 + k)) ++c;
+    c = block_sum_256(c, sh);
+    if (threadIdx.x == 0) A.buf[A.off_counts + blockIdx.x] = c;
+}
+
+__global__ __launch_bounds__(256) void ceres_order_compact(const KParams P, const CompactArgs A) {
+    __shared__ uint32_t sh[4];
+    __shared__ uint32_t wsum[4];
+    const uint32_t groups = (P.n_tiles + A.tpw - 1u) / A.tpw, g0 = blockIdx.x * kCompactBlock + threadIdx.x * 4u;
+    uint32_t before = 0, total = 0;
+    for (uint32_t b = threadIdx.x; b < gridDim.x; b += 256u) {
+        const uint32_t c = A.buf[A.off_counts + b];
+        total += c;
+        if (b < blockIdx.x) before += c;
+    }
+    before = block_sum_256(before, sh);
+    total = block_sum_256(total, sh);
+    const uint32_t rem = P.n_tiles % A.tpw;
+    const uint32_t short_last = rem && group_kept(P, A, groups - 1u) ? A.tpw - rem : 0u;
+    const uint32_t kept_tiles = total * A.tpw - short_last;
+    const uint32_t run = 8u * A.deal, dealt = A.deal ? kept_tiles / (run * A.tpw) * run : 0u;
+    bool keep[4];
+    uint32_t mine = 0;
+    for (uint32_t k = 0; k < 4u; ++k) {
+        keep[k] = g0 + k < groups && group_kept(P, A, g0 + k);
+        mine += keep[k] ? 1u : 0u;
+    }
+    const uint32_t lane = threadIdx.x & 63u, wave = threadIdx.x >> 6;
+    uint32_t x = mine;
+    for (uint32_t off = 1; off < 64u; off <<= 1) {
+        const uint32_t y = __shfl_up(x, off, 64);
+        if (lane >= off) x += y;
+    }
+    if (lane == 63u) wsum[wave] = x;
+    __syncthreads();
+    uint32_t k = before + x - mine;
+    for (uint32_t w = 0; w < wave; ++w) k += wsum[w];
+    for (uint32_t j = 0; j < 4u; ++j) {
+        if (!keep[j]) continue;
+        uint32_t slot = k++;
+        if (slot < dealt) {
+            const uint32_t r = slot % run;
+            slot = slot - r + (r % A.deal) * 8u + r / A.deal;
+        }
+        for (uint32_t i = 0; i < A.tpw; ++i) {
+            const uint32_t p = (g0 + j) * A.tpw + i;
+            A.buf[slot * A.tpw + i] = p < P.n_tiles ? P.tile_order[p] : 0u;
+        }
+    }
+    if (blockIdx.x == gridDim.x - 1u) {
+        const uint32_t end = total * A.tpw, padded = (kept_tiles + 7u) / 8u * 8u;
+        if (end + threadIdx.x < padded) A.buf[end + threadIdx.x] = 0u;
+        if (threadIdx.x == 0) {
+            A.buf[A.off_result] = total;
+            A.buf[A.off_result + 1] = kept_tiles;
+            if (kept_tiles != A.want_tiles) atomicOr(&P.shards[0].error, 2u);
+        }
+    }
+}
+
 __global__ __launch_bounds__(256) void ceres_compact_lit(const float* __restrict__ px, uint32_t n_pix,
                                                          uint4* __restrict__ out, uint32_t* __restrict__ n,
                                                          uint32_t cap) {
@@ -1618,7 +1730,8 @@
     if (s->d_refit_stage) { (void)hipFree(s->d_refit_stage); s->d_refit_stage = nullptr; }
     for (auto& o : s->orders) dfree(o.d);
     for (auto& d : s->retired) dfree(d);
-    s->orders.clear(); s->retired.clear(); s->retired_bytes = 0;
+    for (auto& c : s->compact) dfree(c.d);
+    s->orders.clear(); s->retired.clear(); s->retired_bytes = 0; s->compact.clear();
     dfree(s->d_pairs); dfree(s->d_nodes4); dfree(s->d_qnodes4); dfree(s->d_tris); dfree(s->d_orig); dfree(s->d_norms);
     dfree(s->d_shards); dfree(s->d_counters); dfree(s->d_wave_log); dfree(s->d_pixels); dfree(s->d_rgb8);
     for (auto e : s->ev_pool) (void)hipEventDestroy(e);
@@ -1664,48 +1777,70 @@
     return CERES_OK;
 }
 
+int retire_buffer(ceres_scene* s, uint32_t* d, size_t words) {
+    s->retired.push_back(d);
+    s->retired_bytes += (words * sizeof(uint32_t) + kAllocGranule - 1) / kAllocGranule * kAllocGranule;
+    if (s->retired_bytes > ceres::kRetiredBytes || s->retired.size() >= ceres::kMaxRetired) {
+        HIP_TRY(hipDeviceSynchronize());
+        for (auto& r : s->retired) dfree(r);
+        s->retired.clear();
+        s->retired_bytes = 0;
+    }
+    return CERES_OK;
+}
+
+static void prepare_host_count(ceres_scene::TileOrder& o, const std::vector<uint32_t>& ids, uint32_t bx, uint32_t by, uint32_t tpw);
+
 int upload_tile_order(ceres_scene* s, size_t W, size_t H, const ceres_tiling& t, uint32_t frames, uint32_t tile,
-                      std::vector<uint32_t>& order, hipStream_t stream, const uint32_t** out, bool packed,
-                      uint32_t bx, uint32_t by) {
+                      std::vector<uint32_t>& order, hipStream_t stream, const ceres_scene::TileOrder** out, bool packed,
+                      uint32_t bx, uint32_t by, bool keep_curve, std::vector<uint32_t>* curve = nullptr, uint32_t deal = 0) {
     const size_t n = order.size();
+    ceres_scene::TileOrder o;
+    if (keep_curve) {
+        prepare_host_count(o, curve ? *curve : order, bx, by, tile >> 16);
+        keep_curve = o.countable;
+    }
     if (packed) {
         const uint32_t per_frame = bx * by;
-        for (auto& id : order) {
-            const uint32_t f = id / per_frame, rem = id - f * per_frame, y = rem / bx;
-            id = pack_tile(f, y, rem - y * bx);
-        }
-    }
-    ceres_scene::TileOrder o;
+        auto pack = [&](std::vector<uint32_t>& v) {
+            for (auto& id : v) {
+                const uint32_t f = id / per_frame, rem = id - f * per_frame, y = rem / bx;
+                id = pack_tile(f, y, rem - y * bx);
+            }
+        };
+        pack(order);
+        if (keep_curve && curve) pack(*curve);
+    }
     if (s->orders.size() >= ceres::kMaxTileOrders) {
         auto lru = std::min_element(s->orders.begin(), s->orders.end(),
                                     [](const auto& a, const auto& b) { return a.used < b.used; });
-        s->retired.push_back(lru->d);
-        s->retired_bytes += (lru->cap * sizeof(uint32_t) + kAllocGranule - 1) / kAllocGranule * kAllocGranule;
+        uint32_t* const d = lru->d;
+        const size_t cap = lru->cap;
         s->orders.erase(lru);
-        if (s->retired_bytes > ceres::kRetiredBytes || s->retired.size() >= ceres::kMaxRetired) {
-            HIP_TRY(hipDeviceSynchronize());
-            for (auto& d : s->retired) dfree(d);
-            s->retired.clear();
-            s->retired_bytes = 0;
-        }
+        if (int rc = retire_buffer(s, d, cap)) return rc;
     }
     o.W = W; o.H = H; o.row_block = t.row_block; o.rank = t.rank; o.world = t.world; o.frames = frames; o.tile = tile;
     o.bands = t.bands;
     o.packed = packed;
     const size_t padded = (n + 7) / 8 * 8;
-    if (!o.d) {
-        HIP_TRY(hipMalloc(&o.d, padded * sizeof(uint32_t)));
-        o.cap = padded;
-    }
+    const bool own_curve = keep_curve && curve;
+    o.cap = padded + (own_curve ? n : 0);
+    HIP_TRY(hipMalloc(&o.d, o.cap * sizeof(uint32_t)));
     if ((padded > n && hipMemsetAsync(o.d + n, 0, (padded - n) * sizeof(uint32_t), stream) != hipSuccess) ||
         hipMemcpyAsync(o.d, order.data(), n * sizeof(uint32_t), hipMemcpyHostToDevice, stream) != hipSuccess ||
+        (own_curve && hipMemcpyAsync(o.d + padded, curve->data(), n * sizeof(uint32_t), hipMemcpyHostToDevice, stream) != hipSuccess) ||
         hipStreamSynchronize(stream) != hipSuccess) {
         dfree(o.d);
         return set_error(CERES_EHIP, "tile order upload failed");
     }
+    o.n = uint32_t(n);
+    if (keep_curve) {
+        o.d_curve = own_curve ? o.d + padded : o.d;
+        o.deal = own_curve ? deal : 0u;
+    }
     o.used = ++s->order_clock;
-    s->orders.push_back(o);
-    *out = o.d;
+    s->orders.push_back(std::move(o));
+    *out = &s->orders.back();
     return CERES_OK;
 }
 
@@ -1732,17 +1867,35 @@
     }
 }
 
+void build_tile_order(size_t scene_bytes, size_t W, size_t H, const ceres_tiling& t, size_t rows, uint32_t frames, uint32_t bx,
+                      uint32_t by, uint32_t tile, uint32_t tpw, bool want_curve, std::vector<uint32_t>& order,
+                      std::vector<uint32_t>& curve, uint32_t& deal);
+
 int ensure_tile_order(ceres_scene* s, size_t W, size_t H, const ceres_tiling& t, size_t rows, uint32_t frames,
-                      uint32_t bx, uint32_t by, uint32_t tile, hipStream_t stream, const uint32_t** out, bool packed,
-                      uint32_t tpw) {
+                      uint32_t bx, uint32_t by, uint32_t tile, hipStream_t stream, const ceres_scene::TileOrder** out,
+                      bool packed, uint32_t tpw) {
     const uint32_t tile_key = tile | tpw << 16;
     for (auto& o : s->orders)
         if (o.W == W && o.H == H && o.row_block == t.row_block && o.rank == t.rank && o.world == t.world && o.bands == t.bands &&
             o.frames == frames && o.tile == tile_key && o.packed == packed) {
             o.used = ++s->order_clock;
-            *out = o.d;
+            *out = &o;
             return CERES_OK;
         }
+    const bool keep_curve = frames > 1 && t.world == 1 && !(s->flags & CERES_SCENE_STATS);
+    const size_t scene_bytes = s->n_pairs * sizeof(SiblingPair) + s->n_nodes4 * sizeof(Node4) +
+                               s->n_tri * (sizeof(Tri48) + 4 + 36);
+    std::vector<uint32_t> order, curve;
+    uint32_t deal = 0;
+    build_tile_order(scene_bytes, W, H, t, rows, frames, bx, by, tile, tpw, keep_curve, order, curve, deal);
+    return upload_tile_order(s, W, H, t, frames, tile_key, order, stream, out, packed, bx, by, keep_curve,
+                             deal ? &curve : nullptr, deal);
+}
+
+void build_tile_order(size_t scene_bytes, size_t W, size_t H, const ceres_tiling& t, size_t rows, uint32_t frames, uint32_t bx,
+                      uint32_t by, uint32_t tile, uint32_t tpw, bool want_curve, std::vector<uint32_t>& order,
+                      std::vector<uint32_t>& curve, uint32_t& deal) {
+    deal = 0;
     const size_t n = size_t(bx) * by * frames;
     const double cx = 0.5 * double(W), cy = 0.5 * double(H);
     std::vector<std::pair<double, uint32_t>> k(n);
@@ -1764,10 +1917,8 @@
         if (frame_major && a.second / per_frame != b.second / per_frame) return a.second < b.second;
         return a.first < b.first;
     });
-    std::vector<uint32_t> order(n);
+    order.resize(n);
     for (size_t q = 0; q < n; ++q) order[q] = k[q].second;
-    const size_t scene_bytes = s->n_pairs * sizeof(SiblingPair) + s->n_nodes4 * sizeof(Node4) +
-                               s->n_tri * (sizeof(Tri48) + 4 + 36);
     const size_t lchunk = !CERES_LOCAL_ORDER || !frame_major ? 0
                           : frames > 1 ? size_t(CERES_LOCAL_CHUNK_BATCH)
                           : scene_bytes >= kDramSceneBytes ? size_t(CERES_LOCAL_CHUNK_SOLO) : 0;
@@ -1793,7 +1944,12 @@
             }
             order[p] = mk[src].second;
         }
-        return upload_tile_order(s, W, H, t, frames, tile_key, order, stream, out, packed, bx, by);
+        if (want_curve) {
+            curve.resize(n);
+            for (size_t p = 0; p < n; ++p) curve[p] = mk[p].second;
+        }
+        deal = uint32_t(cw);
+        return;
     }
     uint64_t st = 0x9e3779b97f4a7c15ull;
     for (size_t b0 = 0; b0 < n; b0 += dev::kTileShuffleWindow) {
@@ -1804,7 +1960,6 @@
         }
     }
     if (CERES_XCD_GROUP_TILES && frames > 1) xcd_group_rows(order, bx, per_frame, tpw);
-    return upload_tile_order(s, W, H, t, frames, tile_key, order, stream, out, packed, bx, by);
 }
 
 int quantize_nodes4(const std::vector<Node4>& in, std::vector<QNode4>& out) {
@@ -1927,6 +2082,118 @@
     return false;
 }
 
+static void prepare_host_count(ceres_scene::TileOrder& o, const std::vector<uint32_t>& ids, uint32_t bx, uint32_t by, uint32_t tpw) {
+    const size_t n = ids.size(), pf = size_t(bx) * by;
+    o.shapes.clear(); o.h_curve.clear(); o.countable = false;
+    bool same = tpw <= 4 && pf % tpw == 0;
+    for (size_t p = 0; same && p < n; ++p) same = ids[p % pf] < pf && ids[p] == ids[p % pf] + (p / pf) * pf;
+    std::vector<ceres_scene::TileOrder::SubsetBoxes> shapes;
+    const size_t stride = size_t(bx) + 1;
+    for (size_t g = 0; same && g < pf / tpw; ++g)
+        for (uint32_t mask = 1; same && mask < (1u << tpw); ++mask) {
+            uint32_t x0 = ~0u, x1 = 0, y0 = ~0u, y1 = 0;
+            for (uint32_t i = 0; i < tpw; ++i)
+                if (mask >> i & 1u) {
+                    const uint32_t id = ids[g * tpw + i], y = id / bx, x = id - y * bx;
+                    x0 = std::min(x0, x); x1 = std::max(x1, x); y0 = std::min(y0, y); y1 = std::max(y1, y);
+                }
+            auto it = std::find_if(shapes.begin(), shapes.end(), [&](const auto& b) { return b.w == x1 - x0 && b.h == y1 - y0; });
+            if (it == shapes.end()) {
+                if (shapes.size() == ceres::kCountShapes) { same = false; break; }
+                shapes.emplace_back();
+                it = shapes.end() - 1;
+                it->w = x1 - x0; it->h = y1 - y0;
+                it->sum.assign((size_t(by) + 1) * stride, 0);
+            }
+            it->sum[(size_t(y0) + 1) * stride + x0 + 1] += (__builtin_popcount(mask) & 1) ? 1 : -1;
+        }
+    if (same) {
+        for (auto& b : shapes)
+            for (size_t y = 1; y <= by; ++y)
+                for (size_t x = 1; x <= bx; ++x)
+                    b.sum[y * stride + x] += b.sum[(y - 1) * stride + x] + b.sum[y * stride + x - 1] - b.sum[(y - 1) * stride + x - 1];
+        o.shapes = std::move(shapes);
+        o.countable = true;
+    } else if (n <= ceres::kCountWalkTiles) {
+        o.h_curve = ids;
+        o.countable = true;
+    }
+}
+
+static uint32_t count_kept_tiles(const KParams& P, const ceres_scene::TileOrder& o, uint32_t tpw) {
+    const uint32_t tiles_x = P.tiles_x, tile_rows = P.row_blocks_per_frame, per_frame = tiles_x * tile_rows;
+    std::vector<uint32_t> c0(P.frames, 1u), c1(P.frames, 0u), r0(P.frames, 1u), r1(P.frames, 0u);
+    for (uint32_t f = 0; f < P.frames; ++f) {
+        const CullRect& r = P.cull_rect[f];
+        bool any = false;
+        for (uint32_t bx = 0; bx < tiles_x; ++bx)
+            if (dev::cull_cols_hit(r, P.W, bx)) { if (!any) c0[f] = bx; c1[f] = bx; any = true; }
+        any = false;
+        for (uint32_t by = 0; by < tile_rows; ++by) {
+            const uint32_t lo = 8u * by, hi = std::min(lo + 7u, P.local_rows - 1u);
+            if (std::max<uint32_t>(lo, r.j0) <= std::min<uint32_t>(hi, r.j1)) { if (!any) r0[f] = by; r1[f] = by; any = true; }
+        }
+    }
+    if (!o.shapes.empty()) {
+        const size_t stride = size_t(tiles_x) + 1;
+        int64_t kept = 0;
+        for (uint32_t f = 0; f < P.frames; ++f)
+            for (const auto& b : o.shapes) {
+                if (c0[f] + b.w > c1[f] || r0[f] + b.h > r1[f]) continue;
+                const size_t xa = c0[f], xb = size_t(c1[f]) - b.w + 1, ya = r0[f], yb = size_t(r1[f]) - b.h + 1;
+                kept += int64_t(b.sum[yb * stride + xb]) - b.sum[ya * stride + xb] - b.sum[yb * stride + xa] + b.sum[ya * stride + xa];
+            }
+        return uint32_t(kept) * tpw;
+    }
+    const uint32_t n = o.n, groups = (n + tpw - 1) / tpw;
+    const uint32_t* e = o.h_curve.data();
+    uint32_t kept = 0;
+    bool last = false;
+    for (uint32_t g = 0; g < groups; ++g) {
+        bool keep = false;
+        for (uint32_t p = g * tpw; p < std::min(n, (g + 1) * tpw) && !keep; ++p) {
+            const uint32_t f = e[p] / per_frame, rem = e[p] - f * per_frame, by = rem / tiles_x, bx = rem - by * tiles_x;
+            keep = by >= r0[f] && by <= r1[f] && bx >= c0[f] && bx <= c1[f];
+        }
+        kept += keep;
+        last = keep;
+    }
+    return kept * tpw - (last && n % tpw ? tpw - n % tpw : 0u);
+}
+
+static int compact_buffer(ceres_scene* s, hipStream_t stream, size_t words, ceres_scene::CompactBuf** out) {
+    ceres_scene::CompactBuf* b = nullptr;
+    for (auto& c : s->compact)
+        if (c.stream == stream) b = &c;
+    if (!b) {
+        if (s->compact.size() >= ceres::kMaxCompactBufs) {
+            auto lru = std::min_element(s->compact.begin(), s->compact.end(),
+                                        [](const auto& x, const auto& y) { return x.used < y.used; });
+            uint32_t* const d = lru->d;
+            const size_t cap = lru->cap;
+            s->compact.erase(lru);
+            if (d)
+                if (int rc = retire_buffer(s, d, cap)) return rc;
+        }
+        s->compact.emplace_back();
+        b = &s->compact.back();
+        b->stream = stream;
+    }
+    if (b->cap < words) {
+        if (b->d) {
+            uint32_t* const d = b->d;
+            const size_t cap = b->cap;
+            b->d = nullptr; b->cap = 0;
+            if (int rc = retire_buffer(s, d, cap)) return rc;
+        }
+        HIP_TRY(hipMalloc(&b->d, words * sizeof(uint32_t)));
+        b->cap = words;
+    }
+    b->used = ++s->order_clock;
+    *out = b;
+    return CERES_OK;
+}
+
 static int stack_width(size_t n_pairs, size_t n_nodes4) {
     const size_t nmax = std::max(n_pairs, n_nodes4);
     return CERES_STACK16 && nmax < (1u << 16) ? 2 : CERES_STACK24 && nmax < (1u << 24) ? 3 : 4;
@@ -2033,7 +2300,7 @@
     }
     constexpr uint32_t ftile = 8;
     const uint32_t fbx = uint32_t((W + ftile - 1) / ftile), fby = uint32_t((rows + ftile - 1) / ftile);
-    const uint32_t* tile_order = nullptr;
+    const ceres_scene::TileOrder* tile_order = nullptr;
     const bool packed = frames <= (1u << (32 - kTileXBits - kTileYBits)) &&
                         fbx <= (1u << kTileXBits) && fby <= (1u << kTileYBits);
     const uint32_t tpw = (!stats && (frames > 1 || t.bands)) ? batch_tiles_per_wave(size_t(W) * rows, stack_width(s->n_pairs, s->n_nodes4), qbvh)
@@ -2061,11 +2328,40 @@
                     const long k = std::strtol(g, nullptr, 10);
                     if (k > 0 && uint32_t(k) < P.stack_entries) P.stack_entries = uint32_t(k);
                 }
-            P.tile_order = tile_order;
+            P.tile_order = tile_order->d;
             P.tile_packed = packed ? 1u : 0u;
             P.tiles_x = fbx;
             P.row_blocks_per_frame = fby;
-            const uint32_t n_tiles = fbx * fby * frames;
+            uint32_t n_tiles = fbx * fby * frames;
+            bool compacted = false;
+            if (CERES_COMPACT && P.cull && fill_tasks && tile_order->d_curve && tpw > 1 && P.packets) {
+                const uint32_t kept = count_kept_tiles(P, *tile_order, tpw);
+                if (kept < n_tiles) {
+                    const uint32_t groups = (n_tiles + tpw - 1) / tpw, nb = (groups + dev::kCompactBlock - 1) / dev::kCompactBlock;
+                    ceres::CompactArgs A{};
+                    A.tpw = tpw; A.deal = tile_order->deal; A.want_tiles = kept;
+                    A.off_result = (groups * tpw + 8u + 3u) / 4u * 4u;
+                    A.off_counts = A.off_result + 4u;
+                    A.off_rows = A.off_counts + nb;
+                    ceres_scene::CompactBuf* cb = nullptr;
+                    if (int rc = compact_buffer(s, stream, size_t(A.off_rows) + size_t(frames) * fby, &cb)) return rc;
+                    A.buf = cb->d;
+                    KParams Q = P;
+                    Q.tile_order = tile_order->d_curve;
+                    Q.n_tiles = n_tiles;
+                    hipLaunchKernelGGL(dev::ceres_cull_rows, dim3((frames * fby + 3u) / 4u), dim3(256), 0, stream, Q, A);
+                    hipLaunchKernelGGL(dev::ceres_order_count, dim3(nb), dim3(256), 0, stream, Q, A);
+                    hipLaunchKernelGGL(dev::ceres_order_compact, dim3(nb), dim3(256), 0, stream, Q, A);
+                    HIP_TRY(hipGetLastError());
+                    cb->src = tile_order->d_curve; cb->n = n_tiles; cb->host_tiles = kept; cb->tpw = tpw;
+                    cb->deal = A.deal; cb->off_result = A.off_result;
+                    P.tile_order = cb->d;
+                    n_tiles = kept;
+                    compacted = true;
+                }
+            }
+            if (!stats && frames > 1) { s->last_fused_stream = stream; s->last_fused_compacted = compacted; }
+            P.n_tiles = n_tiles;
             const uint32_t tile_groups = (n_tiles + tpw - 1) / tpw;
             dim3 fgrid(tile_groups + fill_tasks), fblock(dev::kFusedB);
             if (CERES_FILL_SPREAD > (steal ? 1 : 0) && fill_tasks) {
@@ -2218,8 +2514,11 @@
 }
 int frame_tile_order(ceres_scene* s, size_t W, size_t H, uint32_t tile, hipStream_t stream, const uint32_t** out) {
     const ceres_tiling t{uint32_t(H), 0, 1};
-    return ensure_tile_order(s, W, H, t, H, 1, uint32_t((W + tile - 1) / tile), uint32_t((H + tile - 1) / tile), tile,
-                             stream, out, false, 1u);
+    const ceres_scene::TileOrder* o = nullptr;
+    if (int rc = ensure_tile_order(s, W, H, t, H, 1, uint32_t((W + tile - 1) / tile), uint32_t((H + tile - 1) / tile), tile,
+                                   stream, &o, false, 1u)) return rc;
+    *out = o->d;
+    return CERES_OK;
 }
 }
 
@@ -2237,7 +2536,7 @@
     return n;
 }
 const char* ceres_kernel_names(void) {
-    return "ceres_fused,ceres_primary,ceres_finalize,ceres_assemble,ceres_trace_rays_k,ceres_trace_rays64_k,ceres_shade_rays_k,ceres_shade_rays64_k";
+    return "ceres_fused,ceres_primary,ceres_finalize,ceres_assemble,ceres_cull_rows,ceres_order_count,ceres_order_compact,ceres_trace_rays_k,ceres_trace_rays64_k,ceres_shade_rays_k,ceres_shade_rays64_k";
 }
 
 size_t ceres_tiling_local_rows(size_t height, const ceres_tiling* t) {
@@ -2941,6 +3240,66 @@
     return CERES_OK;
 }
 
+int ceres_debug_compact_order(ceres_scene* s, uint32_t info[8], uint32_t* order, uint32_t* source, size_t cap) {
+    if (!s || !info) return set_error(CERES_EINVAL, "ceres_debug_compact_order: null argument");
+    for (int k = 0; k < 8; ++k) info[k] = 0;
+    if (!s->last_fused_compacted) return CERES_OK;
+    const ceres_scene::CompactBuf* b = nullptr;
+    for (const auto& c : s->compact)
+        if (c.stream == s->last_fused_stream) b = &c;
+    if (!b || !b->d) return set_error(CERES_EINVAL, "ceres_debug_compact_order: the launch's buffer is gone");
+    HIP_TRY(hipSetDevice(s->device));
+    HIP_TRY(hipStreamSynchronize(b->stream));
+    uint32_t res[2] = {0, 0};
+    HIP_TRY(hipMemcpy(res, b->d + b->off_result, sizeof res, hipMemcpyDeviceToHost));
+    info[0] = 1; info[1] = b->host_tiles; info[2] = res[1]; info[3] = res[0]; info[4] = b->tpw; info[5] = b->deal; info[6] = b->n;
+    const size_t padded = std::min<size_t>((size_t(res[1]) + 7) / 8 * 8, b->off_result);
+    if (order) {
+        if (cap < padded) return set_error(CERES_EINVAL, "ceres_debug_compact_order: %zu words needed", padded);
+        HIP_TRY(hipMemcpy(order, b->d, padded * sizeof(uint32_t), hipMemcpyDeviceToHost));
+    }
+    if (source) {
+        if (cap < b->n) return set_error(CERES_EINVAL, "ceres_debug_compact_order: %u words needed", b->n);
+        HIP_TRY(hipMemcpy(source, b->src, size_t(b->n) * sizeof(uint32_t), hipMemcpyDeviceToHost));
+    }
+    return CERES_OK;
+}
+
+int ceres_debug_kept_tiles(size_t W, size_t H, uint32_t frames, uint32_t tpw, const uint16_t* rects, uint32_t info[4],
+                           uint32_t* source, size_t cap) {
+    if (!rects || !info) return set_error(CERES_EINVAL, "ceres_debug_kept_tiles: null argument");
+    if (frames < 2 || frames > uint32_t(kFramesPerLaunch) || W == 0 || H == 0 || W > 0xffffu || H > 0xffffu ||
+        (tpw != 2 && tpw != 4 && tpw != 8))
+        return set_error(CERES_EINVAL, "ceres_debug_kept_tiles: 2..%d frames of at most 65535 x 65535 pixels, 2, 4 or 8 tiles per wave",
+                         kFramesPerLaunch);
+    const ceres_tiling t{uint32_t(H), 0, 1};
+    const uint32_t bx = uint32_t((W + 7) / 8), by = uint32_t((H + 7) / 8);
+    const bool packed = frames <= (1u << (32 - kTileXBits - kTileYBits)) && bx <= (1u << kTileXBits) && by <= (1u << kTileYBits);
+    std::vector<uint32_t> order, curve;
+    uint32_t deal = 0;
+    build_tile_order(0, W, H, t, H, frames, bx, by, 8, tpw, true, order, curve, deal);
+    ceres_scene::TileOrder o;
+    std::vector<uint32_t>& src = deal ? curve : order;
+    o.n = uint32_t(src.size());
+    prepare_host_count(o, src, bx, by, tpw);
+    if (packed)
+        for (auto& id : src) {
+            const uint32_t f = id / (bx * by), rem = id - f * (bx * by), y = rem / bx;
+            id = pack_tile(f, y, rem - y * bx);
+        }
+    KParams P{};
+    P.frames = frames; P.W = uint32_t(W); P.H = uint32_t(H); P.local_rows = uint32_t(H); P.row_block = uint32_t(H); P.world = 1;
+    P.tiles_x = bx; P.row_blocks_per_frame = by; P.tile_packed = packed ? 1u : 0u;
+    for (uint32_t f = 0; f < frames; ++f) P.cull_rect[f] = CullRect{rects[4 * f], rects[4 * f + 1], rects[4 * f + 2], rects[4 * f + 3]};
+    info[0] = o.countable ? count_kept_tiles(P, o, tpw) : o.n;
+    info[1] = o.n; info[2] = deal; info[3] = (packed ? 1u : 0u) | (!o.countable ? 0u : o.shapes.empty() ? 2u : 4u);
+    if (source) {
+        if (cap < o.n) return set_error(CERES_EINVAL, "ceres_debug_kept_tiles: %u words needed", o.n);
+        std::memcpy(source, src.data(), size_t(o.n) * sizeof(uint32_t));
+    }
+    return CERES_OK;
+}
+
 int ceres_fetch_counters(int device, uint64_t out[8], int reset) {
     if (!out) return set_error(CERES_EINVAL, "ceres_fetch_counters: null argument");
 #if CERES_COUNTING
diff --git a/ceres-raytracer_amd/csrc/scene_internal.hpp b/ceres-raytracer_amd/csrc/scene_internal.hpp
--- a/ceres-raytracer_amd/csrc/scene_internal.hpp
+++ b/ceres-raytracer_amd/csrc/scene_internal.hpp
@@ -30,7 +30,27 @@
         uint32_t* d = nullptr;
         size_t cap = 0;
         uint64_t used = 0;
+        const uint32_t* d_curve = nullptr;
+        uint32_t n = 0, deal = 0;
+        struct SubsetBoxes {
+            uint32_t w = 0, h = 0;
+            std::vector<int32_t> sum;
+        };
+        std::vector<SubsetBoxes> shapes;
+        std::vector<uint32_t> h_curve;
+        bool countable = false;
     };
+    struct CompactBuf {
+        hipStream_t stream = nullptr;
+        uint32_t* d = nullptr;
+        size_t cap = 0;
+        uint64_t used = 0;
+        const uint32_t* src = nullptr;
+        uint32_t n = 0, host_tiles = 0, tpw = 0, deal = 0, off_result = 0;
+    };
+    std::vector<CompactBuf> compact;
+    hipStream_t last_fused_stream = nullptr;
+    bool last_fused_compacted = false;
     std::vector<TileOrder> orders;
     std::vector<uint32_t*> retired;
     size_t retired_bytes = 0;
@@ -83,6 +103,9 @@
 int scene_after_refit(ceres_scene* s, const float root[6], const SiblingPair& p0);
 int frame_tile_order(ceres_scene* s, size_t W, size_t H, uint32_t tile, hipStream_t stream, const uint32_t** out);
 constexpr size_t kMaxTileOrders = 16;
+constexpr size_t kCountWalkTiles = size_t(1) << 16;
+constexpr size_t kCountShapes = 32;
+constexpr size_t kMaxCompactBufs = 16;
 constexpr size_t kDramSceneBytes = size_t(64) << 20;
 #ifndef CERES_RETIRED_BYTES
 #define CERES_RETIRED_BYTES (64u << 20)
diff --git a/include/ceres_render.h b/include/ceres_render.h
--- a/include/ceres_render.h
+++ b/include/ceres_render.h
@@ -187,6 +187,10 @@
 
 int ceres_scene_wave_log(ceres_scene* scene, uint64_t* out, size_t max_waves, size_t* n_waves);
 
+int ceres_debug_compact_order(ceres_scene* scene, uint32_t info[8], uint32_t* order, uint32_t* source, size_t cap);
+int ceres_debug_kept_tiles(size_t width, size_t height, uint32_t frames, uint32_t tiles_per_wave, const uint16_t* rects,
+                           uint32_t info[4], uint32_t* source, size_t cap);
+
 int ceres_fetch_counters(int device, uint64_t out[8], int reset);
 
 typedef struct ceres_cpu_scene ceres_cpu_scene;
```

After: 52940 Mrays/s, median of 6. +5.9%, better.
